# 07350100647/nvbio-gpl

Hardware: AMD Instinct MI355X
Metric: aligned reads/sec (150 bp single-end, 3 Gbp ref); GCUPS of the banded extend pass in `extend` (higher is better)
Workload: dtype u32 (FM-index coordinates) / i16x2 (band-31 DP, two alignments per 32-bit lane: 16-bit integer scores, held in binary16 lanes where every score is an integer of magnitude <= 2040 -- exact -- and in int16 lanes otherwise; bound-checked on the host)

## Files before the change

include/nvbio_amd.h:

```cpp
#ifndef NVBIO_AMD_H
#define NVBIO_AMD_H

#include <stdint.h>

#ifdef __cplusplus
extern "C" {
#endif

#define NVBIO_AMD_VERSION 100

typedef enum
{
    NVBIO_OK              = 0,
    NVBIO_ERR_INVALID     = 1,
    NVBIO_ERR_HIP         = 2,
    NVBIO_ERR_NOMEM       = 3,
    NVBIO_ERR_UNSUPPORTED = 4,
    NVBIO_ERR_NO_DEVICE   = 5
} nvbio_status;

int         nvbio_amd_version(void);
const char* nvbio_amd_last_error(void);
nvbio_status nvbio_amd_device_count(int* count);
nvbio_status nvbio_amd_device_arch(int device, char* name, uint32_t name_len);
// ... 125 lines not shown
                                           nvbio_uint2* hits_dev, void* stream);

nvbio_status nvbio_fm_filter_locate_diagonals(nvbio_fm_index_t index, const nvbio_uint2* ranges_dev, const uint64_t* slots_dev,
                                              const uint8_t* direct_dev, uint32_t n_queries, uint64_t begin, uint64_t end,
                                              uint32_t seeds_per_read, uint32_t seed_interval, uint32_t seed_len, uint32_t read_len,
                                              uint32_t strand, const uint32_t* query_ids_dev, uint64_t* keys_dev, void* stream);

enum { NVBIO_BACKTRACK_REFERENCE_QUIRKS = 1 };
nvbio_status nvbio_fm_hamming_backtrack(nvbio_fm_index_t index, const nvbio_string_set* queries, uint32_t seed_len, uint32_t mismatches, uint32_t flags,
                                        uint32_t* counts_dev, uint32_t* n_ranges_dev, nvbio_uint2* ranges_dev, uint32_t max_ranges, void* stream);

nvbio_status nvbio_fm_match_seed_diagonals_temp_bytes(const nvbio_string_set* seeds, uint64_t* bytes);
nvbio_status nvbio_fm_match_seed_diagonals(nvbio_fm_index_t index, const nvbio_string_set* seeds, uint32_t flags, uint32_t read_len,
                                           uint32_t strand, uint64_t* keys_dev, nvbio_uint2* residual_ranges_dev, uint32_t* residual_ids_dev,
                                           uint32_t* counts_dev, void* temp_dev, uint64_t temp_bytes, void* stream);

#define NVBIO_FM_INLINE_HITS(h) (((uint32_t)(h) & 15u) << 8)
#define NVBIO_FM_DEFER_HEAVY 64u
#define NVBIO_FM_NO_SEED_LOCUS 128u
#define NVBIO_FM_COUNT_LOCUS 4096u
#define NVBIO_FM_NO_FAST_RESOLVE 8192u
#define NVBIO_FM_COUNT_RESOLVE 16384u
nvbio_status nvbio_fm_match_seed_diagonals_both_temp_bytes(const nvbio_string_set* seeds, uint64_t* bytes);
nvbio_status nvbio_fm_match_seed_diagonals_both_keys_capacity(const nvbio_string_set* seeds, uint64_t* n_keys);
nvbio_status nvbio_fm_match_seed_diagonals_both(nvbio_fm_index_t index, const nvbio_string_set* seeds, uint32_t flags, uint32_t read_len,
                                                uint64_t* keys_dev, nvbio_uint2* residual_ranges_dev, uint32_t* residual_ids_dev,
                                                uint32_t residual_capacity, uint32_t* counts_dev, void* temp_dev, uint64_t temp_bytes,
                                                void* stream);
nvbio_status nvbio_fm_seed_tiles(const nvbio_string_set* seeds, uint32_t* reads_per_tile, uint32_t* n_tiles);
nvbio_status nvbio_fm_match_seed_diagonals_both_tiled(nvbio_fm_index_t index, const nvbio_string_set* seeds, uint32_t flags, uint32_t read_len,
                                                      uint64_t* keys_dev, nvbio_uint2* residual_ranges_dev, uint32_t* residual_ids_dev,
                                                      uint32_t residual_capacity, uint32_t* counts_dev, uint32_t* tile_offsets_dev,
                                                      void* temp_dev, uint64_t temp_bytes, void* stream);
int nvbio_fm_index_is_canonical(nvbio_fm_index_t index);

nvbio_status nvbio_fm_locate_init(nvbio_fm_index_t index, const uint32_t* rows_dev, uint32_t n,
                                  nvbio_uint2* jt_dev, void* stream);
nvbio_status nvbio_fm_locate_lookup(nvbio_fm_index_t index, const nvbio_uint2* jt_dev, uint32_t n,
                                    uint32_t* pos_dev, void* stream);

nvbio_status nvbio_fm_filter_rank(nvbio_fm_index_t index, const nvbio_string_set* queries, uint32_t flags,
                                  nvbio_uint2* ranges_dev, uint64_t* slots_dev, uint64_t* n_hits, void* stream);
nvbio_status nvbio_fm_filter_scan(nvbio_fm_index_t index, const nvbio_uint2* ranges_dev, uint32_t n_queries,
                                  uint64_t* slots_dev, uint64_t* n_hits, void* stream);
nvbio_status nvbio_fm_filter_locate(nvbio_fm_index_t index, const nvbio_uint2* ranges_dev, const uint64_t* slots_dev,
                                    uint32_t n_queries, uint64_t begin, uint64_t end,
                                    nvbio_uint2* hits_dev, void* stream);


typedef struct { uint32_t x, y, string_id, span; } nvbio_mem_range;
typedef struct { uint32_t pos, string_id, span_begin, span_end; } nvbio_mem_hit;
typedef struct { uint32_t min_intv, max_intv, min_span, split_len, split_width; } nvbio_mem_params;

nvbio_status nvbio_mem_filter_temp_bytes(const nvbio_string_set* reads, const nvbio_mem_params* params, uint64_t* bytes, void* stream);
nvbio_status nvbio_mem_filter_rank(nvbio_fm_index_t f_index, nvbio_fm_index_t r_index, const nvbio_string_set* reads,
                                   const nvbio_mem_params* params, nvbio_mem_range* ranges_dev, uint32_t max_ranges,
                                   uint32_t* first_range_dev, uint64_t* slots_dev, void* temp_dev, uint64_t temp_bytes,
                                   uint32_t* n_ranges, uint64_t* n_mems, uint64_t* records, void* stream);
nvbio_status nvbio_mem_filter_locate(nvbio_fm_index_t f_index, const nvbio_mem_range* ranges_dev, const uint64_t* slots_dev,
                                     uint32_t n_ranges, uint64_t begin, uint64_t end, nvbio_mem_hit* hits_dev, void* stream);

typedef struct nvbio_qgram_index_s* nvbio_qgram_index_t;

typedef struct
{
    uint32_t        q, symbol_size, qlut;
// ... 317 lines not shown
    const void*     text_dev;
    uint32_t        text_bits;
    const uint32_t* win_begin_dev;
    const uint32_t* win_end_dev;
    uint32_t        n;
    uint32_t        max_read_len;
    uint32_t        algo_flags;
    const void*     text_planes_dev;
} nvbio_alignment_batch;


enum
{
    NVBIO_ALN_NO_UNGAPPED_SCORE     = 1,
    NVBIO_ALN_NO_THIRD_CHANCE       = 2,
    NVBIO_ALN_NO_PACKED_DP          = 4,
    NVBIO_ALN_FORCE_PACKED_DP       = 8,
    NVBIO_ALN_NO_UNGAPPED_TRACEBACK = 16,
    NVBIO_ALN_PK_THREE_WAVES        = 32,
    NVBIO_ALN_NO_SECOND_CHANCE      = 128,
    NVBIO_ALN_NO_NARROW_SCORE       = 512,
    NVBIO_ALN_NO_BAND_ROUTE         = 1024,
    NVBIO_ALN_PK_STRIPE8            = 256,
    NVBIO_ALN_RAGGED_READS          = 4096,
    NVBIO_ALN_NO_LENGTH_SORT        = 8192,
    NVBIO_ALN_NO_QUALITY_SHORTCUT   = 2048,
    NVBIO_ALN_NO_GAP_CHANCE         = 65536,
    NVBIO_ALN_NO_COOPERATIVE_DP     = 32768,
    NVBIO_ALN_NO_F16_DP             = 16384,
    NVBIO_ALN_SPLIT_CHANCES         = 131072,
    NVBIO_ALN_NO_PAIRED_GAP_CHANCE  = 262144,
    NVBIO_ALN_NO_NARROW_DP          = 524288,
    NVBIO_ALN_NO_TEXT_PLANES        = 1048576,
    NVBIO_ALN_NO_NARROW_TRACEBACK   = 64
};

enum { NVBIO_READ_REVERSE = 1, NVBIO_READ_COMPLEMENT = 2 };

nvbio_status nvbio_best_candidate_reduce(int device, const uint64_t* keys_dev, const int32_t* scores_dev, const nvbio_uint2* sinks_dev,
                                         const uint32_t* win_begin_dev, uint64_t n, uint64_t* best_dev, void* stream);

nvbio_status nvbio_best_candidate_unpack(int device, const uint64_t* best_dev, uint32_t n_reads, int32_t* scores_dev,
                                         int64_t* end_pos_dev, uint8_t* rc_dev, void* stream);

nvbio_status nvbio_best_candidate_windows(int device, const uint64_t* keys_dev, const int32_t* scores_dev, const nvbio_uint2* sinks_dev,
                                          const uint32_t* win_begin_dev, uint64_t n, const uint64_t* best_dev, int64_t* best_wb_dev,
                                          int64_t* best_locus_dev, void* stream);

nvbio_status nvbio_traceback_best_batch(int device, const uint64_t* best_dev, const int64_t* best_wb_dev, uint32_t n_reads, uint32_t read_len,
                                        uint32_t band, uint32_t genome_len, int32_t min_score, uint8_t* flags_dev, uint32_t* win_begin_dev,
                                        uint32_t* win_end_dev, int32_t* scores_dev, nvbio_uint2* sinks_dev, void* stream);

nvbio_status nvbio_second_candidate_reduce(int device, const uint64_t* keys_dev, const int32_t* scores_dev, const nvbio_uint2* sinks_dev,
                                           const uint32_t* win_begin_dev, uint64_t n, const uint64_t* best_dev,
                                           uint32_t distinct_dist, int32_t worst_score, uint64_t* second_dev, void* stream);

typedef struct
{
    int32_t version;
    int32_t monotone;
    int32_t perfect_score;
    int32_t min_score;
} nvbio_mapq_params;
nvbio_status nvbio_mapq(int device, const uint64_t* best_dev, const uint64_t* second_dev, uint32_t n_reads,
                        const nvbio_mapq_params* params, int32_t* second_scores_dev, uint8_t* mapq_dev, void* stream);

nvbio_status nvbio_finish_reads_tiles_per_group(uint32_t reads_per_tile, uint32_t* tiles_per_group);
nvbio_status nvbio_finish_reads(int device, const uint64_t* keys_dev, const int32_t* scores_dev, const nvbio_uint2* sinks_dev,
                                const uint32_t* win_begin_dev, uint64_t n, const uint32_t* tile_offsets_dev, uint32_t n_tiles,
                                uint32_t reads_per_tile, uint32_t n_reads, uint32_t distinct_dist, int32_t worst_score,
                                const nvbio_mapq_params* params, int32_t match, const uint32_t* read_offsets_dev, const int32_t* min_scores_dev,
                                uint64_t* best_dev, uint64_t* second_dev, int32_t* scores_out_dev, int64_t* end_pos_dev, uint8_t* rc_dev,
                                uint8_t* mapq_dev, int32_t* second_scores_dev, uint32_t* status_dev, void* stream);

enum { NVBIO_PE_POLICY_FF = 0, NVBIO_PE_POLICY_FR = 1, NVBIO_PE_POLICY_RF = 2, NVBIO_PE_POLICY_RR = 3 };
nvbio_status nvbio_opposite_mate_windows(int device, const uint32_t* g_pos_dev, const uint8_t* anchor_rc_dev, uint32_t n,
                                         uint32_t anchor_len, uint32_t opposite_gapped_len, uint32_t anchor, uint32_t policy,
                                         uint32_t min_frag_len, uint32_t max_frag_len, uint32_t overlap, uint32_t genome_len,
                                         uint32_t* win_begin_dev, uint32_t* win_end_dev, uint8_t* flags_dev, uint8_t* valid_dev,
                                         void* stream);

#define NVBIO_GAP_PAIR_MAX_SHIFT 5
nvbio_status nvbio_banded_gap_pairs(int device, const nvbio_alignment_batch* batch, uint32_t* partner_dev, void* stream);

nvbio_status nvbio_banded_gotoh_score(int device, uint32_t band, nvbio_alignment_type type,
                                      const nvbio_gotoh_scheme* scheme, const nvbio_alignment_batch* batch,
                                      int32_t* scores_dev, nvbio_uint2* sinks_dev, void* stream);

nvbio_status nvbio_banded_gotoh_score_routes(int device, uint32_t band, nvbio_alignment_type type,
                                             const nvbio_gotoh_scheme* scheme, const nvbio_alignment_batch* batch,
                                             int32_t* scores_dev, nvbio_uint2* sinks_dev, uint8_t* routes_dev, void* stream);

nvbio_status nvbio_banded_gotoh_score_staged(int device, uint32_t band, nvbio_alignment_type type,
                                             const nvbio_gotoh_scheme* scheme, const nvbio_alignment_batch* batch,
                                             const int32_t* min_scores_dev, int32_t min_score,
                                             int32_t* scores_dev, nvbio_uint2* sinks_dev, void* stream);

enum { NVBIO_TRACEBACK_SINKS_GIVEN = 1 };
nvbio_status nvbio_banded_gotoh_traceback_temp_bytes(const nvbio_alignment_batch* batch_host_sizes, uint32_t band, uint64_t* bytes);
nvbio_status nvbio_banded_gotoh_traceback(int device, uint32_t band, nvbio_alignment_type type,
                                          const nvbio_gotoh_scheme* scheme, const nvbio_alignment_batch* batch,
                                          int32_t* scores_dev, nvbio_uint2* sources_dev, nvbio_uint2* sinks_dev,
                                          uint16_t* cigars_dev, uint32_t cigar_stride, uint32_t* cigar_lens_dev,
                                          uint32_t flags, void* temp_dev, uint64_t temp_bytes, void* stream);

nvbio_status nvbio_banded_gotoh_traceback_routes(int device, uint32_t band, nvbio_alignment_type type,
                                                 const nvbio_gotoh_scheme* scheme, const nvbio_alignment_batch* batch,
                                                 int32_t* scores_dev, nvbio_uint2* sources_dev, nvbio_uint2* sinks_dev,
                                                 uint16_t* cigars_dev, uint32_t cigar_stride, uint32_t* cigar_lens_dev,
                                                 uint32_t flags, void* temp_dev, uint64_t temp_bytes,
                                                 uint8_t* routes_dev, uint8_t* band_off_dev, void* stream);

nvbio_status nvbio_banded_sw_traceback(int device, uint32_t band, nvbio_alignment_type type,
                                       const nvbio_sw_scheme* scheme, const nvbio_alignment_batch* batch,
                                       int32_t* scores_dev, nvbio_uint2* sources_dev, nvbio_uint2* sinks_dev,
                                       uint16_t* cigars_dev, uint32_t cigar_stride, uint32_t* cigar_lens_dev,
                                       uint32_t flags, void* temp_dev, uint64_t temp_bytes, void* stream);

nvbio_status nvbio_full_gotoh_traceback_temp_bytes(const nvbio_alignment_batch* batch_host_sizes, uint32_t max_pattern_len,
                                                   uint32_t max_text_len, uint64_t* bytes);
nvbio_status nvbio_full_gotoh_traceback(int device, nvbio_alignment_type type, const nvbio_gotoh_scheme* scheme,
                                        const nvbio_alignment_batch* batch, uint32_t max_pattern_len, uint32_t max_text_len,
                                        const int32_t* min_scores_dev,
                                        int32_t* scores_dev, nvbio_uint2* sources_dev, nvbio_uint2* sinks_dev,
// ... 231 lines not shown
```

nvbio-gpl_amd/__init__.py:

```python
import ctypes
import os

import numpy as np

from .abi import bind

_HERE = os.path.dirname(os.path.abspath(__file__))
LIB_PATH = os.path.join(_HERE, "lib", "libnvbio_amd.so")
HEADER_PATH = os.path.join(os.path.dirname(_HERE), "include", "nvbio_amd.h")
HOST_HEADER_PATH = os.path.join(os.path.dirname(_HERE), "include", "nvbio_amd_host.h")

GLOBAL, LOCAL, SEMI_GLOBAL = 0, 1, 2
SCORE_MIN = -(1 << 30)
FM_SCAN_FORWARD, FM_COMPLEMENT, FM_NO_KMER_TABLE, FM_NO_VERIFY, FM_COUNT_SECTORS, FM_NO_PIPELINE, FM_DEFER_HEAVY = 1, 2, 4, 8, 16, 32, 64
FM_TABLE_NO_DIRECT, FM_TABLE_NO_CONTEXT, FM_TABLE_NO_GROUPS, FM_TABLE_CANONICAL, FM_TABLE_CANONICAL_WIDE = 1, 2, 4, 8, 16
FM_TABLE_NO_TEXT_PLANES = 32
FM_TABLE_NO_SEED_LOCUS = 64
FM_NO_SEED_LOCUS, FM_COUNT_LOCUS = 128, 4096
FM_NO_FAST_RESOLVE, FM_COUNT_RESOLVE = 8192, 16384
READ_REVERSE, READ_COMPLEMENT = 1, 2
MAX_SEED_OFFSET = 1024
TRACEBACK_SINKS_GIVEN = 1
ALN_NO_UNGAPPED_SCORE, ALN_NO_THIRD_CHANCE, ALN_NO_PACKED_DP, ALN_FORCE_PACKED_DP, ALN_NO_UNGAPPED_TRACEBACK, ALN_PK_THREE_WAVES = 1, 2, 4, 8, 16, 32
ALN_NO_NARROW_TRACEBACK, ALN_NO_SECOND_CHANCE, ALN_PK_STRIPE8, ALN_NO_NARROW_SCORE, ALN_NO_BAND_ROUTE = 64, 128, 256, 512, 1024
ALN_NO_QUALITY_SHORTCUT, ALN_RAGGED_READS, ALN_NO_LENGTH_SORT, ALN_NO_F16_DP, ALN_NO_COOPERATIVE_DP, ALN_NO_GAP_CHANCE = 2048, 4096, 8192, 16384, 32768, 65536
ALN_SPLIT_CHANCES, ALN_NO_PAIRED_GAP_CHANCE = 131072, 262144
ALN_NO_NARROW_DP = 524288
ALN_NO_TEXT_PLANES = 1048576
SEED_NO_LOCUS = 2097152
SEED_NO_FAST_RESOLVE = 4194304
ROUTE_SETTLED, ROUTE_FULL_BAND, ROUTE_CLASS_A, ROUTE_CLASS_B, ROUTE_REDONE = 0, 1, 2, 3, 8
DEFAULT_ALGO_FLAGS = 0
BACKTRACK_REFERENCE_QUIRKS = 1

_STATUS = {0: "OK", 1: "INVALID", 2: "HIP", 3: "NOMEM", 4: "UNSUPPORTED", 5: "NO_DEVICE"}


class NvbioError(RuntimeError):
    def __init__(self, status, msg):
        super().__init__("nvbio_amd: %s: %s" % (_STATUS.get(status, status), msg))
        self.status = status


class _View(ctypes.Structure):
    _fields_ = [("length", ctypes.c_uint32), ("primary", ctypes.c_uint32), ("L2", ctypes.c_uint32 * 5),
                ("bwt_occ_dev", ctypes.c_void_p), ("bwt_occ_words", ctypes.c_uint64),
                ("ssa_dev", ctypes.c_void_p), ("ssa_words", ctypes.c_uint64), ("sa_int", ctypes.c_uint32)]


class _BuildOptions(ctypes.Structure):
    _fields_ = [("kmer_len", ctypes.c_uint32), ("sa_int", ctypes.c_uint32), ("max_lcp", ctypes.c_uint32),
                ("verify", ctypes.c_uint32), ("table_flags", ctypes.c_uint32), ("bucket_symbols", ctypes.c_uint32)]


class _StringSet(ctypes.Structure):
    _fields_ = [("symbols_dev", ctypes.c_void_p), ("symbol_bits", ctypes.c_uint32),
                ("offsets_dev", ctypes.c_void_p), ("offsets_are_ranges", ctypes.c_uint32),
                ("fixed_len", ctypes.c_uint32), ("stride", ctypes.c_uint32), ("n", ctypes.c_uint32),
                ("seeds_per_string", ctypes.c_uint32), ("seed_interval", ctypes.c_uint32),
                ("seed_intervals_dev", ctypes.c_void_p)]


class _Scheme(ctypes.Structure):
    _fields_ = [("match", ctypes.c_int32), ("mm_min", ctypes.c_int32), ("mm_max", ctypes.c_int32),
# ... 292 lines not shown
        _check(lib().nvbio_fm_hamming_backtrack(self._h, ctypes.byref(qs), seed_len, mismatches, BACKTRACK_REFERENCE_QUIRKS if quirks else 0,
                                                _ptr(counts), _ptr(nr), _ptr(rg), max_ranges, _stream_ptr(self.device)))
        return counts, nr, rg

    def match_seed_diagonals(self, seeds, flags, read_len, strand, buffers=None, grid_blocks=0):
        torch = _torch()
        n = seeds.n
        if buffers is None:
            buffers = {}
        qs = seeds.c_struct()
        if buffers.get("n") != n or buffers.get("spr") != seeds.seeds_per_string:
            buffers["n"], buffers["spr"] = n, seeds.seeds_per_string
            buffers["keys"] = torch.empty(n, dtype=torch.int64, device=self.device)
            buffers["ranges"] = torch.empty((n, 2), dtype=torch.int32, device=self.device)
            buffers["ids"] = torch.empty(n, dtype=torch.int32, device=self.device)
            buffers["counts"] = torch.empty(4, dtype=torch.int32, device=self.device)
            nb = ctypes.c_uint64(0)
            _check(lib().nvbio_fm_match_seed_diagonals_temp_bytes(ctypes.byref(qs), ctypes.byref(nb)))
            buffers["temp"] = torch.empty(nb.value, dtype=torch.uint8, device=self.device)
        assert grid_blocks % 64 == 0 and grid_blocks < (1 << 22)
        _check(lib().nvbio_fm_match_seed_diagonals(self._h, ctypes.byref(qs), flags | ((grid_blocks // 64) << 16), read_len, strand,
                                                   _ptr(buffers["keys"]), _ptr(buffers["ranges"]), _ptr(buffers["ids"]), _ptr(buffers["counts"]),
                                                   _ptr(buffers["temp"]), buffers["temp"].numel(), _stream_ptr(self.device)))
        return buffers

    @property
    def canonical_kmer(self):
        return lib().nvbio_fm_index_is_canonical(self._h)

    @property
    def canonical(self):
        return self.canonical_kmer != 0

    def match_seed_diagonals_both(self, seeds, read_len, buffers=None, flags=0, grid_blocks=0, inline_hits=0, defer_heavy=False):
        torch = _torch()
        n = seeds.n
        if buffers is None:
            buffers = {}
        qs = seeds.c_struct()
        if buffers.get("n") != n or buffers.get("spr") != seeds.seeds_per_string:
            buffers["n"], buffers["spr"] = n, seeds.seeds_per_string
            cap = ctypes.c_uint64(0)
            _check(lib().nvbio_fm_match_seed_diagonals_both_keys_capacity(ctypes.byref(qs), ctypes.byref(cap)))
            buffers["keys"] = torch.empty(max(int(cap.value), 1), dtype=torch.int64, device=self.device)
            buffers["ranges"] = torch.empty((2 * n, 2), dtype=torch.int32, device=self.device)
            buffers["ids"] = torch.empty(2 * n, dtype=torch.int32, device=self.device)
            buffers["counts"] = torch.zeros(12, dtype=torch.int32, device=self.device)
            nb = ctypes.c_uint64(0)
            _check(lib().nvbio_fm_match_seed_diagonals_both_temp_bytes(ctypes.byref(qs), ctypes.byref(nb)))
            buffers["temp"] = torch.empty(nb.value, dtype=torch.uint8, device=self.device)
            rpt, nt = ctypes.c_uint32(0), ctypes.c_uint32(0)
            _check(lib().nvbio_fm_seed_tiles(ctypes.byref(qs), ctypes.byref(rpt), ctypes.byref(nt)))
            buffers["reads_per_tile"], buffers["n_tiles"] = int(rpt.value), int(nt.value)
            buffers["tile_offsets"] = torch.zeros(int(nt.value) + 1, dtype=torch.int32, device=self.device)
        assert grid_blocks % 64 == 0 and grid_blocks < (1 << 22)
        _check(lib().nvbio_fm_match_seed_diagonals_both_tiled(
            self._h, ctypes.byref(qs), flags | (FM_DEFER_HEAVY if defer_heavy else 0) | ((int(inline_hits) & 15) << 8) | ((grid_blocks // 64) << 16),
            read_len, _ptr(buffers["keys"]), _ptr(buffers["ranges"]), _ptr(buffers["ids"]), n, _ptr(buffers["counts"]), _ptr(buffers["tile_offsets"]),
            _ptr(buffers["temp"]), buffers["temp"].numel(), _stream_ptr(self.device)))
        return buffers

    def residual_diagonals(self, ranges, ids, cap, seeds_per_read, seed_interval, seed_len, read_len, read_offsets=None, seed_intervals=None):
        torch = _torch()
        n = int(ids.numel())
        keys = torch.empty(max(n * int(cap), 1), dtype=torch.int64, device=self.device)
        n_keys = torch.zeros(1, dtype=torch.int32, device=self.device)
        _check(lib().nvbio_fm_residual_diagonals(
            self._h, _ptr(ranges), _ptr(ids), n, int(cap), seeds_per_read, seed_interval, seed_len, read_len, _ptr(read_offsets),
            _ptr(seed_intervals), _ptr(keys), _ptr(n_keys), _stream_ptr(self.device)))
        return keys, n_keys

    def rank(self, rows, syms):
        torch = _torch()
        rows = _dev_tensor(rows, torch.int32, self.device)
        syms = _dev_tensor(syms, torch.uint8, self.device)
        out = torch.empty(rows.numel(), dtype=torch.int32, device=self.device)
        _check(lib().nvbio_fm_rank(self._h, _ptr(rows), _ptr(syms), rows.numel(), _ptr(out), _stream_ptr(self.device)))
        return out

    def rank4(self, rows):
        torch = _torch()
        rows = _dev_tensor(rows, torch.int32, self.device)
        out = torch.empty((rows.numel(), 4), dtype=torch.int32, device=self.device)
        _check(lib().nvbio_fm_rank4(self._h, _ptr(rows), rows.numel(), _ptr(out), _stream_ptr(self.device)))
        return out

    def basic_inv_psi(self, rows):
        torch = _torch()
        rows = _dev_tensor(rows, torch.int32, self.device)
        out = torch.empty(rows.numel(), dtype=torch.int32, device=self.device)
        _check(lib().nvbio_fm_basic_inv_psi(self._h, _ptr(rows), rows.numel(), _ptr(out), _stream_ptr(self.device)))
        return out
# ... 513 lines not shown
        self.c = _SWScheme(match, mismatch, deletion, insertion)


class SmithWatermanAligner:

    def __init__(self, type, scheme):
        self.type, self.sw = type, scheme
        c = scheme.c
        self.scheme = (GotohScheme(c.match, -c.mismatch, -c.mismatch, c.deletion, c.deletion, c.deletion, c.deletion)
                       if c.deletion == c.insertion else None)


def make_smith_waterman_aligner(type, scheme):
    return SmithWatermanAligner(type, scheme)


def make_edit_distance_aligner(type):
    return SmithWatermanAligner(type, SimpleSmithWatermanScheme(0, -1, -1, -1))


class GotohAligner:

    def __init__(self, type, scheme):
        self.type, self.scheme = type, scheme


def make_gotoh_aligner(type, scheme):
    return GotohAligner(type, scheme)


class AlignmentBatch:

    def __init__(self, reads, read_bits, read_offsets, text, text_bits, win_begin, win_end, quals=None, read_id=None,
                 flags=None, device="cuda:0", max_read_len=0, algo_flags=None, text_planes=None):
        torch = _torch()
        self.device = device
        self.text_planes = text_planes
        self.algo_flags = DEFAULT_ALGO_FLAGS if algo_flags is None else int(algo_flags)
        self.read_bits, self.text_bits = int(read_bits), int(text_bits)
        self.reads = _dev_tensor(reads, torch.uint8 if read_bits == 8 else torch.int32, device)
        self.read_offsets = _dev_tensor(read_offsets, torch.int32, device)
        self.text = _dev_tensor(text, torch.uint8 if text_bits == 8 else torch.int32, device)
        self.win_begin = _dev_tensor(win_begin, torch.int32, device)
        self.win_end = _dev_tensor(win_end, torch.int32, device)
        self.quals = _dev_tensor(quals, torch.uint8, device)
        self.read_id = _dev_tensor(read_id, torch.int32, device)
        self.flags = _dev_tensor(flags, torch.uint8, device)
        self.n = int(self.win_begin.numel())
        self.max_read_len = int(max_read_len)

    def size(self):
        return self.n

    def c_struct(self):
        return _Batch(_ptr(self.reads), self.read_bits, _ptr(self.read_offsets), _ptr(self.quals), _ptr(self.read_id),
                      _ptr(self.flags), _ptr(self.text), self.text_bits, _ptr(self.win_begin), _ptr(self.win_end),
                      self.n, self.max_read_len, self.algo_flags,
                      ctypes.c_void_p(self.text_planes.data_ptr() if hasattr(self.text_planes, "data_ptr") else self.text_planes))


def seed_locus_bytes(length):
    b = ctypes.c_uint64()
    _check(lib().nvbio_seed_locus_bytes(length, ctypes.byref(b)))
    return b.value


def text_planes_bytes(length):
    b = ctypes.c_uint64()
    _check(lib().nvbio_text_planes_bytes(length, ctypes.byref(b)))
    return b.value
# ... 13 lines not shown


class BatchedBandedAlignmentScore:

    def __init__(self, band_len, aligner, scheduler=DEVICE_THREAD_SCHEDULER):
        self.band_len, self.aligner, self.scheduler = int(band_len), aligner, scheduler
        if scheduler not in (DEVICE_THREAD_SCHEDULER, DEVICE_STAGED_THREAD_SCHEDULER):
            raise NvbioError(1, "unknown scheduler %r" % (scheduler,))

    def min_temp_storage(self, max_pattern_len, max_text_len, stream_size):
        return 0

    max_temp_storage = min_temp_storage

    def enact(self, batch, scores=None, sinks=None, min_scores=None):
        torch = _torch()
        if scores is None:
            scores = torch.empty(batch.n, dtype=torch.int32, device=batch.device)
        if sinks is None:
            sinks = torch.empty((batch.n, 2), dtype=torch.int32, device=batch.device)
        bs = batch.c_struct()
        sw = getattr(self.aligner, "sw", None)
        if self.scheduler == DEVICE_STAGED_THREAD_SCHEDULER:
            if sw is not None:
                raise NvbioError(4, "the staged scheduler is instantiated for Gotoh aligners")
            per_job = min_scores is not None and not isinstance(min_scores, int)
            if per_job and (min_scores.dtype != torch.int32 or min_scores.numel() != batch.n):
                raise NvbioError(1, "min_scores: int32 per job")
            _check(lib().nvbio_banded_gotoh_score_staged(
                FMIndex._dev_index(batch.device), self.band_len, self.aligner.type, ctypes.byref(self.aligner.scheme.c), ctypes.byref(bs),
                _ptr(min_scores) if per_job else None, SCORE_MIN if min_scores is None else (0 if per_job else int(min_scores)), _ptr(scores),
                _ptr(sinks), _stream_ptr(batch.device)))
            return scores, sinks
        fn = lib().nvbio_banded_sw_score if sw is not None else lib().nvbio_banded_gotoh_score
        _check(fn(FMIndex._dev_index(batch.device), self.band_len, self.aligner.type, ctypes.byref(sw.c if sw is not None else self.aligner.scheme.c),
                  ctypes.byref(bs), _ptr(scores), _ptr(sinks), _stream_ptr(batch.device)))
        return scores, sinks


def batch_banded_alignment_score(band_len, aligner, batch):
    return BatchedBandedAlignmentScore(band_len, aligner).enact(batch)


def banded_gotoh_score_routes(band_len, aligner, batch):
    torch = _torch()
    scores = torch.empty(batch.n, dtype=torch.int32, device=batch.device)
    sinks = torch.empty((batch.n, 2), dtype=torch.int32, device=batch.device)
    routes = torch.empty(batch.n, dtype=torch.uint8, device=batch.device)
    bs = batch.c_struct()
    _check(lib().nvbio_banded_gotoh_score_routes(FMIndex._dev_index(batch.device), int(band_len), aligner.type, ctypes.byref(aligner.scheme.c),
                                                 ctypes.byref(bs), _ptr(scores), _ptr(sinks), _ptr(routes), _stream_ptr(batch.device)))
    return scores, sinks, routes


TB_ROUTE_SETTLED, TB_ROUTE_FULL_BAND, TB_ROUTE_BAND15, TB_ROUTE_BAND7 = 0, 1, 2, 3


def banded_gotoh_traceback_routes(band_len, aligner, batch, cigar_stride=64, temp=None, scores=None, sinks=None):
    torch = _torch()
    n, dev = batch.n, batch.device
    given = scores is not None and sinks is not None
    if not given:
        scores = torch.empty(n, dtype=torch.int32, device=dev)
        sinks = torch.empty((n, 2), dtype=torch.int32, device=dev)
    sources = torch.empty((n, 2), dtype=torch.int32, device=dev)
    cigars = torch.zeros((n, cigar_stride), dtype=torch.int16, device=dev)
    lens = torch.empty(n, dtype=torch.int32, device=dev)
    routes = torch.empty(n, dtype=torch.uint8, device=dev)
    band_off = torch.empty(n, dtype=torch.uint8, device=dev)
    bs = batch.c_struct()
    _check(lib().nvbio_banded_gotoh_traceback_routes(
        FMIndex._dev_index(dev), int(band_len), aligner.type, ctypes.byref(aligner.scheme.c), ctypes.byref(bs), _ptr(scores), _ptr(sources),
        _ptr(sinks), _ptr(cigars), cigar_stride, _ptr(lens), TRACEBACK_SINKS_GIVEN if given else 0, _ptr(temp),
        0 if temp is None else temp.numel() * temp.element_size(), _ptr(routes), _ptr(band_off), _stream_ptr(dev)))
    return scores, sources, sinks, cigars, lens, routes, band_off


FULL_TB_ROUTE_SETTLED, FULL_TB_ROUTE_ALL_ROWS, FULL_TB_ROUTE_RESTRICTED, FULL_TB_ROUTE_BAND15 = 0, 1, 2, 3


def full_gotoh_traceback_routes(aligner, batch, max_pattern_len, max_text_len, min_scores=None, cigar_stride=64, temp=None, scores=None, sinks=None):
    torch = _torch()
# ... 1227 lines not shown
```

nvbio-gpl_amd/csrc/band31_first_pass.hip:

```cpp
#include "band31_ungapped_inl.h"

namespace nvbio_amd {

template <int RBITS, int MODE, bool QUAL = false>
__global__ void __launch_bounds__(256) __attribute__((amdgpu_waves_per_eu((MODE == 0 && !QUAL) ? 7 : 1)))
ungapped_e2e31_kernel(const BatchDev b, const int32_t P, const int32_t G, const int32_t gap_open, const int32_t gap_ext,
                      int32_t* __restrict__ scores, uint2* __restrict__ sinks, uint8_t* __restrict__ need_dp,
                      const uint32_t* __restrict__ job_list, const uint32_t* __restrict__ job_count,
                      const SchemeDev sc, const JobLists out, const uint32_t third_mask, const NarrowRule nr)
{
    constexpr bool LIST = MODE != 0;
    constexpr int  NL   = LIST ? 1 : 6;
    __shared__ int32_t s_pen[QUAL ? 64 : 1];
    __shared__ typename JobAppend<NL>::Lds s_lists;
    const uint32_t n    = LIST ? *job_count : b.n;
    const uint32_t slot0 = blockIdx.x * (256u * JOB_LIST_CHUNKS);
    if (slot0 >= n) return;
    if (QUAL)
    {
        if (threadIdx.x < 64) s_pen[threadIdx.x] = -mismatch_score( sc, threadIdx.x );
        __syncthreads();
    }
    JobAppend<NL> app;
    auto job_of = [&](const int k) -> uint32_t { const uint32_t slot = slot0 + 256u * k + threadIdx.x; return LIST ? job_list[slot] : slot; };
    const bool pairing = ((third_mask >> 4) & 1u) && !(b.algo & (NVBIO_ALN_NO_PAIRED_GAP_CHANCE | NVBIO_ALN_RAGGED_READS));
    #pragma unroll 1
    for (int k = 0; k < JOB_LIST_CHUNKS; ++k)
    {
        int which = -1;
        uint32_t flag = 0;
        if (slot0 + 256u * k + threadIdx.x < n)
        {
            const uint32_t job  = job_of( k );
            flag = ungapped_e2e31_job<RBITS,MODE,QUAL>( b, P, G, gap_open, gap_ext, scores, sinks, job, s_pen, nr );
            const uint32_t cls = flag >> 8;
            flag &= 255u;
            need_dp[job] = (uint8_t)flag;
            if (flag) which = LIST ? JOB_DP : (flag == 3u ? JOB_SECOND : (((third_mask >> flag) & 1u) ? JOB_THIRD : (cls ? JOB_CLASS_B - 1 + (int)cls : JOB_DP)));
        }
        if (MODE == 0 && !QUAL && pairing && __any( flag == 4u ))
        {
            const uint32_t slot = slot0 + 256u * k + threadIdx.x;
            const int role = gap_pair_role( b, slot, slot < n );
            const uint32_t flag_up = __shfl_down( flag, 1 ), flag_dn = __shfl_up( flag, 1 );
            if (role > 0 && flag == 4u && flag_up == 4u) which = JOB_PAIRS;
            if (role < 0 && flag == 4u && flag_dn == 4u) which = -1;
        }
        app.note( s_lists, k, which );
    }
    app.flush( s_lists, out, job_of );
}

nvbio_status launch_ungapped_e2e31(const uint32_t rbits, const int mode, const bool by_quality, const BatchDev& b, const SchemeDev& sc, const int32_t P,
                                   const int32_t G, int32_t* scores, uint2* sinks, uint8_t* need_dp, const JobLists& out, const uint32_t third_mask,
                                   const NarrowRule nr, hipStream_t s)
{
    const dim3 grid( job_list_grid( b.n ) ), block( 256 );
    const uint32_t* job_list  = mode == 1 ? out.second : (mode == 2 ? out.third : nullptr);
    const uint32_t* job_count = mode == 1 ? out.count( JOB_SECOND ) : (mode == 2 ? out.count( JOB_THIRD ) : nullptr);
    auto miss = [&] { set_error( "band-31 first pass: read_bits %u, mode %d not instantiated", rbits, mode ); return NVBIO_ERR_UNSUPPORTED; };
    return with_value( ReadBits31(), (int)rbits, [&](auto RB)
    {
        if (by_quality && mode == 0)
            return NVB_LAUNCH( (ungapped_e2e31_kernel<RB,0,true>), grid, block, s, b, P, G, sc.pat_go, sc.pat_ge, scores, sinks, need_dp, job_list, job_count,
                               sc, out, third_mask, nr );
        return with_value( Values<0, 1, 2>(), by_quality ? -1 : mode, [&](auto MODE)
        {
            return NVB_LAUNCH( (ungapped_e2e31_kernel<RB,MODE>), grid, block, s, b, P, G, sc.pat_go, sc.pat_ge, scores, sinks, need_dp, job_list, job_count,
                               MODE == 0 ? sc : SchemeDev{}, out, MODE == 0 ? third_mask : 0u, MODE == 0 ? nr : NarrowRule{ 1, 1, 0u } );
        }, miss );
    }, miss );
}

}
```

nvbio-gpl_amd/csrc/band31_jobs.h:

```cpp
#pragma once
#include "gotoh_common.h"
#include "bitplanes.h"

namespace nvbio_amd {

constexpr int GAP_CHANCE_GA = 5;
__host__ __device__ __forceinline__ int32_t gap_chance_unknown_cost(const int32_t P, const int32_t go, const int32_t ge)
{
    auto cg = [&](const int g) -> int32_t { return -(go + (g - 1) * ge); };
    int32_t c = cg( 1 ) + 3 * P;
    const int32_t others[] = { cg( GAP_CHANCE_GA + 1 ), 3 * cg( 1 ), 2 * cg( 1 ) + P, cg( 1 ) + cg( 3 ), 2 * cg( 2 ) };
    #pragma unroll
    for (int k = 0; k < 5; ++k) c = others[k] < c ? others[k] : c;
    return c;
}
struct GapLadder { int32_t c_unk_u, c_unk_n; };
constexpr int NARROW_A_HALF = 6, NARROW_B_HALF = 8;
struct NarrowJobs { const uint32_t *list_b, *count_b, *list_a, *count_a; uint32_t *redo, *redo_count; };
struct NarrowRule { int32_t thr_a, thr_b; uint32_t cnt_max; };
__device__ __forceinline__ uint32_t narrow_class(const NarrowRule nr, const int64_t U, const uint32_t best_d, const int32_t gap_ext)
{
    const int64_t o = best_d > 15u ? best_d - 15u : 15u - best_d;
    if (o <= NARROW_A_HALF && U >= (int64_t)nr.thr_a - o * gap_ext) return 2u;
    if (o <= NARROW_B_HALF && U >= (int64_t)nr.thr_b - o * gap_ext) return 1u;
    return 0u;
}

enum JobList : uint32_t
{
    JOB_DP,
    JOB_SECOND,
    JOB_THIRD,
    JOB_PAIRS,
    JOB_CLASS_B, JOB_CLASS_A,
    JOB_REDO,
    JOB_LIST_COUNT
};
static_assert( JOB_CLASS_A == JOB_CLASS_B + 1, "narrow_class() 1, 2 = class B, class A, in this order" );
constexpr uint32_t JOB_COUNT_STRIDE = 32u;
#ifndef NVB_JOB_LIST_CHUNKS
#define NVB_JOB_LIST_CHUNKS 1
#endif
constexpr int JOB_LIST_CHUNKS = NVB_JOB_LIST_CHUNKS;
static inline uint32_t job_list_grid(const uint32_t n) { return (n + 256u * JOB_LIST_CHUNKS - 1u) / (256u * JOB_LIST_CHUNKS); }

struct JobLists
{
    uint32_t *dp, *second, *third, *pairs; uint32_t* counts; uint32_t *class_b, *class_a, *redo;
    static __host__ __device__ constexpr uint32_t count_at(const uint32_t list) { return JOB_COUNT_STRIDE * list; }
    __host__ __device__ __forceinline__ uint32_t* count(const uint32_t list) const { return counts + count_at( list ); }
};

template <int NL>
struct JobAppend
{
    static_assert( NL >= 1 && NL <= 6 && JOB_LIST_CHUNKS >= 1 && JOB_LIST_CHUNKS <= 4, "JobAppend: up to 6 lists, up to 4 chunks" );
    struct Lds { uint32_t cnt[NL][4 * JOB_LIST_CHUNKS]; uint32_t base[NL]; };
    static constexpr int SLOT = NL <= 3 ? 8 : 16;
    typedef typename std::conditional<NL <= 3, uint32_t, uint64_t>::type Mine;
    Mine mine = 0;
    __device__ __forceinline__ void note(Lds& lds, const int k, const int which)
    {
        const uint32_t lane = threadIdx.x & 63u, wave = threadIdx.x >> 6;
        #pragma unroll
        for (int l = 0; l < NL; ++l)
        {
            const uint64_t m = __ballot( which == l );
            if (lane == 0) lds.cnt[l][4 * k + wave] = (uint32_t)__popcll( m );
            if (which == l) mine |= (Mine)(((uint32_t)(l + 1) << 6) | (uint32_t)__popcll( m & ((1ull << lane) - 1ull) )) << (SLOT * k);
        }
    }
    template <typename JobOf>
    __device__ __forceinline__ void flush(Lds& lds, const JobLists& out, JobOf job_of)
    {
        __syncthreads();
        if (threadIdx.x < (uint32_t)NL)
        {
            uint32_t tot = 0;
            for (int i = 0; i < 4 * JOB_LIST_CHUNKS; ++i) { const uint32_t c = lds.cnt[threadIdx.x][i]; lds.cnt[threadIdx.x][i] = tot; tot += c; }
            lds.base[threadIdx.x] = tot ? atomicAdd( out.count( threadIdx.x ), (unsigned int)tot ) : 0u;
        }
        __syncthreads();
        const uint32_t wave = threadIdx.x >> 6;
        #pragma unroll
        for (int k = 0; k < JOB_LIST_CHUNKS; ++k)
        {
            const uint32_t e = (uint32_t)(mine >> (SLOT * k)) & ((1u << SLOT) - 1u);
            if (e)
            {
                const uint32_t l = (e >> 6) - 1u;
                uint32_t* const list = l == JOB_DP ? out.dp : (l == JOB_SECOND ? out.second : (l == JOB_THIRD ? out.third : (l == JOB_PAIRS ? out.pairs : (l == JOB_CLASS_B ? out.class_b : out.class_a))));
                list[lds.base[l] + lds.cnt[l][4 * k + wave] + (e & 63u)] = job_of( k );
            }
        }
    }
};

struct JobAppendTwo
{
    struct Lds { uint32_t cnt[2 * 4 * JOB_LIST_CHUNKS]; uint32_t base; };
    uint64_t mine = 0;
    __device__ __forceinline__ void note(Lds& lds, const int k, const bool first, const bool second)
    {
        const uint32_t lane = threadIdx.x & 63u, wave = threadIdx.x >> 6;
        #pragma unroll
        for (int r = 0; r < 2; ++r)
        {
            const bool on = r ? second : first;
            const uint64_t m = __ballot( on );
            if (lane == 0) lds.cnt[4 * (2 * k + r) + wave] = (uint32_t)__popcll( m );
            if (on) mine |= (uint64_t)(64u | (uint32_t)__popcll( m & ((1ull << lane) - 1ull) )) << (16 * k + 8 * r);
        }
    }
    template <typename JobOf>
    __device__ __forceinline__ void flush(Lds& lds, const JobLists& out, JobOf job_of)
    {
        __syncthreads();
        if (threadIdx.x == 0)
        {
            uint32_t tot = 0;
            for (int i = 0; i < 2 * 4 * JOB_LIST_CHUNKS; ++i) { const uint32_t c = lds.cnt[i]; lds.cnt[i] = tot; tot += c; }
            lds.base = tot ? atomicAdd( out.count( JOB_DP ), (unsigned int)tot ) : 0u;
        }
        __syncthreads();
        const uint32_t wave = threadIdx.x >> 6;
        #pragma unroll
        for (int k = 0; k < JOB_LIST_CHUNKS; ++k)
            #pragma unroll
            for (int r = 0; r < 2; ++r)
            {
                const uint32_t e = (uint32_t)(mine >> (16 * k + 8 * r)) & 255u;
                if (e) out.dp[lds.base + lds.cnt[4 * (2 * k + r) + wave] + (e & 63u)] = job_of( k, r );
            }
    }
};

constexpr uint32_t PAIR_MAX_SHIFT = NVBIO_GAP_PAIR_MAX_SHIFT;

__device__ __forceinline__ int gap_pair_role(const BatchDev& b, const uint32_t job, const bool live)
{
    uint32_t rid = 0, fl = 0, tb = 0, whole = 0;
    if (live)
    {
        rid = b.read_id ? b.read_id[job] : job;
        const uint32_t M = b.read_offsets[rid + 1] - b.read_offsets[rid];
        fl = b.flags ? b.flags[job] : 0u;
        tb = b.win_begin[job];
        whole = (M >= 1u && M <= PLANE_MAX_READ && b.win_end[job] - tb == M + 31u) ? 1u : 0u;
    }
    const uint32_t lane = threadIdx.x & 63u;
    const uint32_t rid_n = __shfl_down( rid, 1 ), fl_n = __shfl_down( fl, 1 ), tb_n = __shfl_down( tb, 1 ), whole_n = __shfl_down( whole, 1 );
    const uint32_t shift = tb_n > tb ? tb_n - tb : tb - tb_n;
    const bool link = lane < 63u && whole && whole_n && rid_n == rid && fl_n == fl && shift >= 1u && shift <= PAIR_MAX_SHIFT;
    const uint64_t links = __ballot( link );
    const uint32_t run = lane ? (uint32_t)__clzll( (long long)~(links << (64u - lane)) ) : 0u;
    const bool lower = link && !(run & 1u);
    const uint64_t lowers = __ballot( lower );
    if (lower) return 1;
    return (lane && ((lowers >> (lane - 1u)) & 1ull)) ? -1 : 0;
}

bool packed_ok(const int type, const SchemeDev& sc, const uint32_t max_read_len);
bool pk_binary16_ok(const int type, const BatchDev& b, const SchemeDev& sc);
nvbio_status launch_pk_kernel(const int type, const uint32_t rbits, const BatchDev& b, const SchemeDev& sc, const uint32_t pairs, int32_t* scores, uint2* sinks,
                              const uint32_t* job_list, const uint32_t* job_count, hipStream_t s, const NarrowJobs* narrow = nullptr);
nvbio_status launch_ungapped_e2e31(const uint32_t rbits, const int mode, const bool by_quality, const BatchDev& b, const SchemeDev& sc, const int32_t P,
                                   const int32_t G, int32_t* scores, uint2* sinks, uint8_t* need_dp, const JobLists& out, const uint32_t third_mask,
                                   const NarrowRule nr, hipStream_t s);
nvbio_status launch_gap_chance_e2e31(const uint32_t rbits, const bool with_second, const BatchDev& b, const SchemeDev& sc, const int32_t P, const int32_t G,
                                     const GapLadder lad, int32_t* scores, uint2* sinks, uint8_t* need_dp, const JobLists& out, hipStream_t s);
nvbio_status launch_gap_pairs(const BatchDev& b, uint32_t* partner, hipStream_t s);
nvbio_status launch_pk(const int type, const uint32_t rbits, const BatchDev& b, const SchemeDev& sc, int32_t* scores, uint2* sinks, hipStream_t s, uint8_t* routes);

using ReadBits31 = Values<2, 4>;

}
```

nvbio-gpl_amd/csrc/band31_stage.hip:

```cpp
#include "band31_jobs.h"
#include <hipcub/hipcub.hpp>

namespace nvbio_amd {

static bool ungapped_ok(const SchemeDev& sc, const BatchDev& b, int32_t* P, bool* by_quality)
{
    if (sc.match != 0) return false;
    if (sc.mm_min < 0 || sc.mm_max < 0) return false;
    if (sc.mm_min == 0) return false;
    *by_quality = b.quals != nullptr && sc.mm_min != sc.mm_max;
    if (*by_quality && (sc.mm_min <= 0 || sc.mm_max < sc.mm_min || (b.algo & NVBIO_ALN_NO_QUALITY_SHORTCUT))) return false;
    if (sc.pat_go >= 0 || sc.txt_go >= 0 || sc.pat_ge > 0 || sc.txt_ge > 0) return false;
    *P = sc.mm_min;
    return true;
}

static NarrowRule narrow_rule(const bool on, const int32_t P, const int32_t go, const int32_t ge)
{
    NarrowRule r = { 1, 1, 0u };
    if (!on || ge >= 0 || P <= 0) return r;
    const int64_t a = (int64_t)go + (int64_t)NARROW_A_HALF * ge + 1, bb = (int64_t)go + (int64_t)NARROW_B_HALF * ge + 1;
    if (bb < -2000) return r;
    r.thr_a = (int32_t)a; r.thr_b = (int32_t)bb;
    r.cnt_max = (uint32_t)((-bb) / P);
// ... 29 lines not shown
    }
}

static nvbio_status sort_jobs_by_length(const BatchDev& b, const uint32_t* job_list, const uint32_t* job_count, const uint32_t** list_out,
                                        const uint32_t** count_out, ScratchBlock* aux, hipStream_t s)
{
    size_t sort_bytes = 0;
    const int bits = 16;
    NVB_HIP( hipcub::DeviceRadixSort::SortPairs( nullptr, sort_bytes, (const uint16_t*)nullptr, (uint16_t*)nullptr, (const uint32_t*)nullptr, (uint32_t*)nullptr,
                                                 (int)b.n, 0, bits, s ) );
    uint16_t *k_in, *k_out; uint32_t *l_all, *l_out, *c_all; void* tmp;
    NVB_CHECK( aux->alloc_layout( "banded_length_sort", s, "banded score: out of device memory for the length-sorted job list", [&](ScratchLayout& c)
    {
        k_in  = c.take<uint16_t>( b.n ); k_out = c.take<uint16_t>( b.n );
        l_all = c.take<uint32_t>( b.n ); l_out = c.take<uint32_t>( b.n );
        c_all = c.take<uint32_t>( 1 );
        tmp   = c.take<uint8_t>( sort_bytes );
    } ) );
    NVB_CHECK( NVB_LAUNCH( job_length_keys_kernel, dim3( (b.n + 255u) / 256u < 65536u ? (b.n + 255u) / 256u : 65536u ), dim3( 256 ), s, b, job_list, job_count, k_in, l_all, c_all ) );
    const hipError_t e = hipcub::DeviceRadixSort::SortPairs( tmp, sort_bytes, (const uint16_t*)k_in, k_out, job_list ? job_list : (const uint32_t*)l_all, l_out, (int)b.n, 0, bits, s );
    if (e != hipSuccess) { set_error( "job sort failed: %s", hipGetErrorString( e ) ); return NVBIO_ERR_HIP; }
    *list_out = l_out; *count_out = job_list ? job_count : c_all;
    return NVBIO_OK;
}

template <bool REDO>
__global__ void __launch_bounds__(256)
job_routes_kernel(const JobLists l, const uint32_t n, const bool classes, uint8_t* __restrict__ routes)
{
    const uint32_t n_dp = REDO ? 0u : *l.count( JOB_DP ), n_b = (REDO || !classes) ? 0u : *l.count( JOB_CLASS_B ), n_a = (REDO || !classes) ? 0u : *l.count( JOB_CLASS_A );
    const uint32_t n_r = (REDO && classes) ? *l.count( JOB_REDO ) : 0u;
    for (uint32_t i = blockIdx.x * blockDim.x + threadIdx.x; i < n; i += gridDim.x * blockDim.x)
    {
        if (i < n_dp) routes[l.dp[i]] = 1u;
        if (i < n_b)  routes[l.class_b[i]] = 3u;
        if (i < n_a)  routes[l.class_a[i]] = 2u;
        if (i < n_r)  routes[l.redo[i]] |= 8u;
    }
}

nvbio_status launch_pk(const int type, const uint32_t rbits, const BatchDev& b, const SchemeDev& sc, int32_t* scores, uint2* sinks, hipStream_t s, uint8_t* routes)
{
    const uint32_t pairs = (b.n + 1u) / 2u;
    int32_t P = 0; bool by_quality = false;
    const bool sorted_lengths = type == NVBIO_SEMI_GLOBAL && sc.match == 0 && (b.algo & NVBIO_ALN_RAGGED_READS) && !(b.algo & NVBIO_ALN_NO_LENGTH_SORT);
    if (type == NVBIO_SEMI_GLOBAL && ungapped_ok( sc, b, &P, &by_quality ) && !(b.algo & NVBIO_ALN_NO_UNGAPPED_SCORE))
    {
        const int32_t G = sc.pat_go > sc.txt_go ? sc.pat_go : sc.txt_go;
        const bool third = !(b.algo & NVBIO_ALN_NO_THIRD_CHANCE);
        uint8_t* need_dp; JobLists out;
        const NarrowRule nr = narrow_rule( b.quals == nullptr && !(b.algo & (NVBIO_ALN_NO_NARROW_DP | NVBIO_ALN_RAGGED_READS)) && pk_binary16_ok( type, b, sc ),
                                           P, sc.pat_go, sc.pat_ge );
        const bool classes = nr.thr_b != 1;
        ScratchBlock aux;
        NVB_CHECK( aux.alloc_layout( "banded_job_list", s, "banded score: out of device memory for the job list", [&](ScratchLayout& c)
        {
            need_dp     = c.take<uint8_t>( b.n );
            out.dp      = c.take<uint32_t>( b.n );
            out.second  = c.take<uint32_t>( b.n );
            out.third   = c.take<uint32_t>( b.n );
            out.pairs   = c.take<uint32_t>( (b.n + 1u) / 2u );
            out.counts  = c.take<uint32_t>( JobLists::count_at( JOB_LIST_COUNT ) );
            out.class_b = c.take<uint32_t>( classes ? b.n : 1u );
            out.class_a = c.take<uint32_t>( classes ? b.n : 1u );
            out.redo    = c.take<uint32_t>( classes ? b.n : 1u );
        } ) );
        const bool gapc = !by_quality && !(b.algo & NVBIO_ALN_NO_GAP_CHANCE);
        const uint32_t third_mask = gapc ? ((third ? 1u << 2 : 0u) | 1u << 4) : (third ? 1u << 2 : 0u);
        const bool fused = gapc && third && !(b.algo & (NVBIO_ALN_NO_SECOND_CHANCE | NVBIO_ALN_SPLIT_CHANCES));
        const GapLadder lad = gap_ladder( P, G, sc.pat_go, sc.pat_ge );
        NVB_HIP( hipMemsetAsync( out.counts, 0, JobLists::count_at( JOB_LIST_COUNT ) * sizeof(uint32_t), s ) );
        NVB_CHECK( launch_ungapped_e2e31( rbits, 0, by_quality, b, sc, P, G, scores, sinks, need_dp, out, third_mask, nr, s ) );
        if (!fused)     NVB_CHECK( launch_ungapped_e2e31( rbits, 1, false, b, sc, P, G, scores, sinks, need_dp, out, 0u, nr, s ) );
        if (gapc)       NVB_CHECK( launch_gap_chance_e2e31( rbits, fused, b, sc, P, G, lad, scores, sinks, need_dp, out, s ) );
        else if (third) NVB_CHECK( launch_ungapped_e2e31( rbits, 2, false, b, sc, P, G, scores, sinks, need_dp, out, 0u, nr, s ) );
        const uint32_t* jl = out.dp; const uint32_t* jc = out.count( JOB_DP ); ScratchBlock sorted;
        if (sorted_lengths) NVB_CHECK( sort_jobs_by_length( b, out.dp, out.count( JOB_DP ), &jl, &jc, &sorted, s ) );
        if (classes)
        {
            const NarrowJobs nj = { out.class_b, out.count( JOB_CLASS_B ), out.class_a, out.count( JOB_CLASS_A ), out.redo, out.count( JOB_REDO ) };
            NVB_CHECK( launch_pk_kernel( type, rbits, b, sc, pairs, scores, sinks, jl, jc, s, &nj ) );
            NVB_CHECK( launch_pk_kernel( type, rbits, b, sc, pairs, scores, sinks, out.redo, out.count( JOB_REDO ), s ) );
        }
        else
            NVB_CHECK( launch_pk_kernel( type, rbits, b, sc, pairs, scores, sinks, jl, jc, s ) );
        if (routes)
        {
            const dim3 rgrid( (b.n + 255u) / 256u < 4096u ? (b.n + 255u) / 256u : 4096u ), block( 256 );
            NVB_HIP( hipMemsetAsync( routes, 0, b.n, s ) );
            NVB_CHECK( NVB_LAUNCH( job_routes_kernel<false>, rgrid, block, s, out, b.n, classes, routes ) );
            NVB_CHECK( NVB_LAUNCH( job_routes_kernel<true>,  rgrid, block, s, out, b.n, classes, routes ) );
        }
        return NVBIO_OK;
    }
    if (sorted_lengths && b.n > 1u)
    {
        const uint32_t* jl = nullptr; const uint32_t* jc = nullptr; ScratchBlock sorted;
        NVB_CHECK( sort_jobs_by_length( b, nullptr, nullptr, &jl, &jc, &sorted, s ) );
        return launch_pk_kernel( type, rbits, b, sc, pairs, scores, sinks, jl, jc, s );
    }
    return launch_pk_kernel( type, rbits, b, sc, pairs, scores, sinks, nullptr, nullptr, s );
}

}
```

nvbio-gpl_amd/csrc/band31_ungapped_inl.h:

```cpp
#pragma once
#include "band31_jobs.h"

namespace nvbio_amd {


struct PlaneWords
{
    uint32_t pl[6], ph[6], pn[6], pm[6], ql[7], qh[7];

    __device__ __forceinline__ void set(const uint64_t (&rlo)[3], const uint64_t (&rhi)[3], const uint64_t (&rn)[3],
                                        const uint64_t (&tlo)[4], const uint64_t (&thi)[4], const uint32_t M)
    {
        #pragma unroll
        for (int k = 0; k < 3; ++k)
        {
            pattern_plane_words( k, rlo, rhi, rn, M, pl, ph, pn, pm );
            ql[2*k] = (uint32_t)tlo[k]; ql[2*k+1] = (uint32_t)(tlo[k] >> 32);
            qh[2*k] = (uint32_t)thi[k]; qh[2*k+1] = (uint32_t)(thi[k] >> 32);
        }
        ql[6] = (uint32_t)tlo[3]; qh[6] = (uint32_t)thi[3];
    }
    __device__ __forceinline__ uint32_t mmw(const int k, const uint32_t x) const
    {
        const uint32_t tl = __builtin_amdgcn_alignbit( ql[k + 1], ql[k], x ), th = __builtin_amdgcn_alignbit( qh[k + 1], qh[k], x );
        return (((pl[k] ^ tl) | (ph[k] ^ th)) & pm[k]) | pn[k];
    }
};

template <int RBITS, int MODE, bool QUAL>
__device__ __forceinline__ uint32_t
ungapped_e2e31_job(const BatchDev& b, const int32_t P, const int32_t G, const int32_t gap_open, const int32_t gap_ext,
                   int32_t* __restrict__ scores, uint2* __restrict__ sinks, const uint32_t job, const int32_t* s_pen,
                   const NarrowRule nr = NarrowRule{ 1, 1, 0u })
{
    constexpr bool LIST = MODE != 0;
    const AlnJob   J = load_job( b, job );
    const uint32_t first = J.first, M = J.M, tb = J.tb, N = scored_text_len( b, J );
    const bool     rev = J.rev, comp = J.comp;

    if (N < M)
    {
        scores[job] = NVBIO_SCORE_MIN; sinks[job] = make_uint2( 0xFFFFFFFFu, 0xFFFFFFFFu );
        return 0u;
    }
    if (M == 0u || M > 161u) return 1u;

    uint64_t rlo[3], rhi[3], rn[3], tlo[4], thi[4];
    {
        ReadWords<RBITS> rw; TextUnits<4> tu;
        load_read_words<RBITS>( b.reads, first, M, rw );
        if (b.text_planes) load_text_units<4,0,3>( b.text_planes, tb, tu );
        else               load_text_words<13>( b.text, tb, N < 192u ? N : 192u, tu );
        read_planes192<RBITS>( rw, first, M, rev, comp, rlo, rhi, rn );
        if (b.text_planes)
        {
            load_text_units<4,3,4>( b.text_planes, tb, tu );
            text_planes_units<4>( tu, tb, tlo, thi );
        }
        else text_planes_words<13>( tu, tb, tlo, thi );
    }
    const uint32_t mb = M + 30u;
    const uint32_t m  = (mb < N ? mb : N) - (M - 1u);
    PlaneWords pw;
    pw.set( rlo, rhi, rn, tlo, thi, M );
    const uint32_t (&pl)[6] = pw.pl, (&ph)[6] = pw.ph, (&pn)[6] = pw.pn, (&pm)[6] = pw.pm, (&ql0)[7] = pw.ql, (&qh0)[7] = pw.qh;
    uint32_t ql[7], qh[7];

    uint32_t best_cnt = 0xFFFFFFFFu, best_d = 0;
    int64_t U = 0;
    if (LIST)
    {
        U      = scores[job];
        best_d = sinks[job].x - M;
    }
    else
    {
        const int64_t floor_u = 3 * (int64_t)(G < gap_open ? G : gap_open) - P;
        const uint32_t cap = P > 0 ? (uint32_t)((-floor_u - 1) / (int64_t)P) : 0xFFFFFFFEu;
        const uint32_t cap_x = (!QUAL && nr.cnt_max > cap && N >= M + 30u) ? nr.cnt_max : cap;
        uint32_t cnt_d[QUAL ? 31 : 1];
        #pragma unroll
        for (uint32_t d = 0; d < 31u; ++d)
        {
            const bool on = (d == 0u || d < m);
            uint32_t cnt = (uint32_t)__popc( pw.mmw( 0, d ) );
            const uint32_t thr = QUAL ? cap : (best_cnt < cap_x ? best_cnt : cap_x);
            if (__any( on && cnt <= thr ))
            {
                #pragma unroll
                for (int k = 1; k < 6; ++k) cnt += (uint32_t)__popc( pw.mmw( k, d ) );
            }
            else cnt = 0xFFFFFFFFu;
            if (QUAL) cnt_d[d] = on ? cnt : 0xFFFFFFFFu;
            if (on && cnt <= best_cnt) { best_cnt = cnt; best_d = d; }
        }
        if (best_cnt > cap)
        {
            if (!QUAL && best_cnt <= cap_x)
            {
                const uint32_t cls = narrow_class( nr, -(int64_t)P * (int64_t)best_cnt, best_d, gap_ext );
                if (cls) { scores[job] = -P * (int32_t)best_cnt; sinks[job] = make_uint2( M + best_d, M ); return 1u | (cls << 8); }
            }
            const bool gap_chance = !QUAL && P > 0 && N >= M + 30u && gap_ext < 0 && gap_open <= gap_ext && !(b.algo & NVBIO_ALN_NO_GAP_CHANCE);
            return gap_chance ? 4u : 1u;
        }
        U = -(int64_t)P * (int64_t)best_cnt;
        if (QUAL)
        {
            if (U <= 3 * (int64_t)G - P) return 1u;
            const uint32_t pmax  = (uint32_t)s_pen[63];
            const uint64_t bound = (uint64_t)pmax * best_cnt;
            uint32_t cand = 0;
            #pragma unroll
            for (uint32_t d = 0; d < 31u; ++d)
                if (cnt_d[d] != 0xFFFFFFFFu && (uint64_t)(uint32_t)P * cnt_d[d] <= bound) cand |= 1u << d;
            uint32_t best_w = 0xFFFFFFFFu;
            while (cand)
            {
                const uint32_t d = (uint32_t)__builtin_ctz( cand );
                cand &= cand - 1u;
                uint32_t w = 0;
                #pragma unroll
                for (int k = 0; k < 6; ++k)
                {
                    uint32_t mm = pw.mmw( k, d );
                    while (mm)
                    {
                        const uint32_t row = 32u * k + (uint32_t)__builtin_ctz( mm );
                        mm &= mm - 1u;
                        const uint32_t qq = b.quals[rev ? first + M - 1u - row : first + row];
                        w += (uint32_t)s_pen[qq < 63u ? qq : 63u];
                    }
                }
                if (w <= best_w) { best_w = w; best_d = d; }
            }
            U = -(int64_t)best_w;
        }
    }
    bool settled = U > (int64_t)G;
    auto stash = [&]() { scores[job] = (int32_t)U; sinks[job] = make_uint2( M + best_d, M ); };
    const bool second_applies = !settled && (int64_t)G - P < U && 2 * (int64_t)G < U && N >= M + 30u && !(b.algo & NVBIO_ALN_NO_SECOND_CHANCE);
    if (MODE == 0 && second_applies)
    {
        int32_t gmax = 0;
        while (gmax < 5 && (int64_t)gap_open + (int64_t)gmax * gap_ext >= U) ++gmax;
        if (gmax >= 1 && gmax <= 4) { stash(); return 3u; }
    }
    if (MODE == 1 && second_applies)
    {
        int32_t gmax = 0;
        while (gmax < 5 && (int64_t)gap_open + (int64_t)gmax * gap_ext >= U) ++gmax;
        if (gmax >= 1 && gmax <= 4)
        {
            #pragma unroll
            for (int k = 0; k < 7; ++k) { ql[k] = ql0[k]; qh[k] = qh0[k]; }
            uint32_t lead_prev[4] = { 0, 0, 0, 0 }, tail_prev[4] = { 0, 0, 0, 0 };
            bool gapped = false;
            for (uint32_t d = 0; d < 31u && !gapped; ++d)
            {
                uint32_t first = M, last = 0xFFFFFFFFu;
                #pragma unroll
                for (int k = 0; k < 6; ++k)
                    if (first == M)
                    {
                        const uint32_t mm = (((pl[k] ^ ql[k]) | (ph[k] ^ qh[k])) & pm[k]) | pn[k];
                        if (mm) first = 32u * k + (uint32_t)__builtin_ctz( mm );
                    }
                #pragma unroll
                for (int k = 5; k >= 0; --k)
                    if (last == 0xFFFFFFFFu)
                    {
                        const uint32_t mm = (((pl[k] ^ ql[k]) | (ph[k] ^ qh[k])) & pm[k]) | pn[k];
                        if (mm) last = 32u * k + 31u - (uint32_t)__builtin_clz( mm );
                    }
                const uint32_t lead = first;
                const uint32_t tail = (last == 0xFFFFFFFFu) ? M : M - 1u - last;
                #pragma unroll
                for (int g = 1; g <= 4; ++g)
                    if (g <= gmax && d >= (uint32_t)g)
                    {
                        if (lead_prev[g - 1] + tail >= M) gapped = true;
                        if (lead + tail_prev[g - 1] + (uint32_t)g >= M) gapped = true;
                    }
                #pragma unroll
                for (int k = 3; k > 0; --k) { lead_prev[k] = lead_prev[k - 1]; tail_prev[k] = tail_prev[k - 1]; }
                lead_prev[0] = lead; tail_prev[0] = tail;
                #pragma unroll
                for (int k = 0; k < 6; ++k)
                {
                    ql[k] = __builtin_amdgcn_alignbit( ql[k + 1], ql[k], 1u );
                    qh[k] = __builtin_amdgcn_alignbit( qh[k + 1], qh[k], 1u );
                }
                ql[6] >>= 1; qh[6] >>= 1;
            }
            settled = !gapped;
        }
    }
    const int64_t go = gap_open, ge = gap_ext;
    int32_t gmax0 = 0, gmax1 = 0;
    while (gmax0 < 5 && go + (int64_t)gmax0 * ge >= U) ++gmax0;
    while (gmax1 < 5 && go + (int64_t)gmax1 * ge - P >= U) ++gmax1;
    const bool two11  = 2 * go >= U;
    const bool beyond = gmax0 > 4 || gmax1 > 4 || go - 2 * (int64_t)P >= U || 2 * go + ge >= U || 2 * go - P >= U || 3 * go >= U || ge < go;
    const bool third_applies = !settled && N >= M + 30u && !beyond && gmax0 >= 1 && (gmax1 >= 1 || two11);
    if (MODE == 0 && third_applies)
    {
        stash();
        return 2u;
    }
    if (MODE != 0 && third_applies)
    {
        #pragma unroll
        for (int k = 0; k < 7; ++k) { ql[k] = ql0[k]; qh[k] = qh0[k]; }
        uint32_t lead0_p[4] = { 0, 0, 0, 0 }, lead1_p[4] = { 0, 0, 0, 0 }, tail0_p[4] = { 0, 0, 0, 0 }, tail1_p[4] = { 0, 0, 0, 0 };
        bool gapped = false;
        uint32_t mwp[6] = { 0, 0, 0, 0, 0, 0 };
        for (uint32_t d = 0; d <= 31u && !gapped; ++d)
        {
            const bool have = d < 31u;
            uint32_t first = M, second = M, last = 0xFFFFFFFFu, last2 = 0xFFFFFFFFu;
            #pragma unroll
            for (int k = 0; k < 6; ++k)
                if (have && __any( second == M ))
                {
                    uint32_t w = (second == M) ? ((((pl[k] ^ ql[k]) | (ph[k] ^ qh[k])) & pm[k]) | pn[k]) : 0u;
                    if (first == M && w) { first = 32u * k + (uint32_t)__builtin_ctz( w ); w &= w - 1u; }
                    if (first != M && second == M && w) second = 32u * k + (uint32_t)__builtin_ctz( w );
                }
            #pragma unroll
            for (int k = 5; k >= 0; --k)
                if (have && __any( last2 == 0xFFFFFFFFu ))
                {
                    uint32_t w = (last2 == 0xFFFFFFFFu) ? ((((pl[k] ^ ql[k]) | (ph[k] ^ qh[k])) & pm[k]) | pn[k]) : 0u;
                    if (last == 0xFFFFFFFFu && w) { const uint32_t t = 31u - (uint32_t)__builtin_clz( w ); last = 32u * k + t; w &= ~(1u << t); }
                    if (last != 0xFFFFFFFFu && last2 == 0xFFFFFFFFu && w) last2 = 32u * k + 31u - (uint32_t)__builtin_clz( w );
                }
            const uint32_t lead0 = first, lead1 = second;
            const uint32_t tail0 = (last  == 0xFFFFFFFFu) ? M : M - 1u - last;
            const uint32_t tail1 = (last2 == 0xFFFFFFFFu) ? M : M - 1u - last2;
            if (have)
            {
                #pragma unroll
// ... 51 lines not shown
                                {
                                    const uint32_t hi_m = (a1 >= 32) ? 0xFFFFFFFFu : ((1u << a1) - 1u);
                                    const uint32_t lo_m = (1u << a0) - 1u;
                                    any = any || ((mwp[k] & hi_m & ~lo_m) != 0u);
                                }
                            }
                        }
                        if (!any) gapped = true;
                    }
            }
            #pragma unroll
            for (int k = 3; k > 0; --k) { lead0_p[k] = lead0_p[k - 1]; lead1_p[k] = lead1_p[k - 1]; tail0_p[k] = tail0_p[k - 1]; tail1_p[k] = tail1_p[k - 1]; }
            lead0_p[0] = lead0; lead1_p[0] = lead1; tail0_p[0] = tail0; tail1_p[0] = tail1;
            if (two11 && have)
            {
                #pragma unroll
                for (int k = 0; k < 6; ++k) mwp[k] = (((pl[k] ^ ql[k]) | (ph[k] ^ qh[k])) & pm[k]) | pn[k];
            }
            #pragma unroll
            for (int k = 0; k < 6; ++k)
            {
                ql[k] = __builtin_amdgcn_alignbit( ql[k + 1], ql[k], 1u );
                qh[k] = __builtin_amdgcn_alignbit( qh[k + 1], qh[k], 1u );
            }
            ql[6] >>= 1; qh[6] >>= 1;
        }
        settled = !gapped;
    }
    if (settled)
    {
        scores[job] = (int32_t)U; sinks[job] = make_uint2( M + best_d, M );
        return 0u;
    }
    if (MODE == 0 && !QUAL && N >= M + 30u)
    {
        const uint32_t cls = narrow_class( nr, U, best_d, gap_ext );
        if (cls) { stash(); return 1u | (cls << 8); }
    }
    return 1u;
}

}
```

nvbio-gpl_amd/csrc/bitplanes.h:

```cpp
#pragma once
#include "common.h"

namespace nvbio_amd {

constexpr uint32_t PLANE_MAX_READ = 161u;

template <int RBITS> struct ReadWords { static constexpr int N = (161 + 15) * RBITS / 32 + 2; uint32_t w[N]; };

template <int RBITS>
__device__ __forceinline__ void load_read_words(const void* reads, const uint32_t first, const uint32_t M, ReadWords<RBITS>& out)
{
    constexpr uint32_t RPW = 32u / RBITS;
    const uint32_t* __restrict__ rwords = (const uint32_t*)reads;
    const uint32_t rw0 = (first & ~(RPW - 1u)) / RPW, rw_last = (first + M - 1u) / RPW;
    #pragma unroll
    for (int j = 0; j < ReadWords<RBITS>::N; ++j) { const uint32_t widx = rw0 + (uint32_t)j; out.w[j] = rwords[widx < rw_last ? widx : rw_last]; }
}

template <int WORDS, typename W>
__device__ __forceinline__ void load_text_words(const void* text, const uint32_t tb, const uint32_t T, W& out)
{
    const uint32_t* __restrict__ twords = (const uint32_t*)text;
    const uint32_t tw0 = (tb & ~15u) >> 4, tw_last = (tb + T - 1u) >> 4;
    #pragma unroll
// ... 138 lines not shown
    #pragma unroll
    for (int k = 0; k < 4; ++k)
    {
        tlo[k] = (uint64_t)__builtin_amdgcn_alignbit( a[2*k+1], a[2*k], s ) | ((uint64_t)__builtin_amdgcn_alignbit( a[2*k+2], a[2*k+1], s ) << 32);
        thi[k] = (uint64_t)__builtin_amdgcn_alignbit( c[2*k+1], c[2*k], s ) | ((uint64_t)__builtin_amdgcn_alignbit( c[2*k+2], c[2*k+1], s ) << 32);
    }
}

constexpr uint32_t SEED_LOCUS_LINE_BYTES = 128u;
constexpr uint32_t SEED_LOCUS_UNITS      = 5u;
constexpr uint32_t SEED_LOCUS_MAX_READ   = 193u;
inline __host__ __device__ uint64_t seed_locus_lines(const uint32_t n) { return ((uint64_t)n >> 7) + 1u; }

struct LocusWords { uint32_t lo0, lo1, hi0, hi1, u; };

__device__ __forceinline__ void load_locus_words(const void* __restrict__ lines, const uint32_t base, const uint32_t x, LocusWords& out)
{
    static_assert( 127u + SEED_LOCUS_MAX_READ - 1u <= 64u * SEED_LOCUS_UNITS - 1u, "the last symbol of a read lies in the line its first symbol lies in" );
    static_assert( 24u * SEED_LOCUS_UNITS <= SEED_LOCUS_LINE_BYTES, "a line holds its units" );
    const uint32_t line = base >> 7, off = x - (line << 7), unit = off >> 6, w = (off >> 5) & 1u;
    const uint32_t* __restrict__ p = (const uint32_t*)lines + ((size_t)line * 32u + 6u * unit);
    const uint32_t w1 = w ? (unit + 1u < SEED_LOCUS_UNITS ? 6u : 0u) : 1u;
    out.lo0 = p[w]; out.lo1 = p[w1]; out.hi0 = p[2u + w]; out.hi1 = p[2u + w1]; out.u = p[4u + w];
}

__device__ __forceinline__ bool locus_answers(const LocusWords& lw, const uint32_t x, const uint32_t len, const uint32_t tlo, const uint32_t thi)
{
    const uint32_t s = x & 31u;
    const uint32_t lo = __builtin_amdgcn_alignbit( lw.lo1, lw.lo0, s ), hi = __builtin_amdgcn_alignbit( lw.hi1, lw.hi0, s );
    const uint32_t mask = len >= 32u ? 0xFFFFFFFFu : (1u << len) - 1u;
    return ((((lo ^ tlo) | (hi ^ thi)) & mask) == 0u) && ((lw.u >> s) & 1u);
}

}
```

nvbio-gpl_amd/csrc/fm_canon_inl.h:

```cpp
constexpr uint32_t CTAB_FLANK    = 7u;
constexpr uint32_t CTAB_ROWS_MAX = 8u;
constexpr uint32_t CTAB_INLINE   = 4u;

__device__ __forceinline__ uint64_t canon_revcomp(const uint64_t key, const uint32_t k)
{
    return reverse_symbols( key, k ) ^ ((1ull << (2u * k)) - 1ull);
}
__device__ __forceinline__ uint64_t canon_index(const uint64_t ckey, const uint32_t k)
{
    return ((ckey >> (k + 1u)) << k) | (ckey & ((1ull << k) - 1ull));
}
__device__ __forceinline__ uint64_t canon_key(const uint64_t idx, const uint32_t k)
{
    return ((idx >> k) << (k + 1u)) | (idx & ((1ull << k) - 1ull));
}
__device__ __forceinline__ uint32_t text_symbol(const uint32_t* __restrict__ text, const uint32_t i)
{
    return (text[i >> 4] >> (30u - 2u * (i & 15u))) & 3u;
}

__device__ __forceinline__ uint2 canon_range(const DevIndex& f, const uint64_t key)
{
    const uint2 r = f.ktab[key >> 2];
    uint32_t x = r.x, y = r.y, nb = 0;
// ... 212 lines not shown
seed_locus_kernel(const DevIndex f, const uint32_t len, const uint32_t wide, const uint64_t n_units, const uint64_t n_lines, uint64_t* __restrict__ lines)
{
    const uint32_t lane = threadIdx.x & 63u, n = f.length;
    for (uint64_t unit = (uint64_t)blockIdx.x * 4u + (threadIdx.x >> 6); unit < n_units; unit += (uint64_t)gridDim.x * 4u)
    {
        const uint64_t x64 = unit * 64u + lane;
        const uint32_t sym = x64 < n ? text_symbol( f.text, (uint32_t)x64 ) : 0u;
        bool uq = false;
        if (x64 + len <= n)
        {
            const uint32_t x = (uint32_t)x64;
            uint64_t V; uint32_t qo; CanonHits h;
            (void)seed_bits_from_words<2>( load_seed_words<2>( f.text, x, len ), x, len, false, false, V );
            uint4 e = canon_entry( f, V, len, wide != 0u, qo );
            uq = canon_lookup( f, V, len, qo, e, h ) && h.nf == 1u && h.nr == 0u && h.vf == x;
            if (uq)
            {
                const uint64_t R = canon_revcomp( V, len );
                e  = canon_entry( f, R, len, wide != 0u, qo );
                uq = canon_lookup( f, R, len, qo, e, h ) && h.nf == 0u && h.nr == 1u && h.vr == x;
            }
        }
        const uint64_t ub = __ballot( uq ), lo = __ballot( (sym & 1u) != 0u ), hi = __ballot( (sym & 2u) != 0u );
        if (lane < 3u && (unit >> 1) >= lane)
        {
            const uint64_t L = (unit >> 1) - lane, slot = unit - 2u * L;
            if (L < n_lines && slot < SEED_LOCUS_UNITS) { uint64_t* p = lines + L * 16u + 3u * slot; p[0] = lo; p[1] = hi; p[2] = ub; }
        }
    }
}

enum : uint32_t { LS_SEED = 1u, LS_OK = 2u, LS_ASKED = 4u, LS_USABLE = 8u, LS_STRAND = 16u,
                  LS_SETTLED = 32u,
                  LS_BEGIN = 256u };
template <int BITS, bool COUNT, bool WIDE, bool RAGGED, typename Geom, typename Entry, typename Resolve>
__device__ __forceinline__ void fm_seed_locus_loop(const DevIndex& f, const StringSetDev& q, const SeedTiles& tl, const uint32_t read_len, const void* __restrict__ locus,
                                                   unsigned long long* __restrict__ sectors_out, unsigned int* __restrict__ routes, const uint32_t tile0,
                                                   const uint32_t lane, const uint32_t lr, const uint32_t j, const bool lane_ok,
                                                   const Geom& seed_geom, const Entry& entry_of, const Resolve& resolve_tile)
{
    const uint32_t n_waves = gridDim.x * 4u;
    const uint32_t k = f.ckmer, len = q.fixed_len, n = f.length;
    const uint32_t anchor = lane - j;
    const bool     first = j == 0u;
    const uint32_t u_pfw = j * q.interval;
    const uint4 none = make_uint4( 1u, 0u, 0u, 0u );
    auto qo_of = [&](const uint64_t V) -> uint32_t { return (uint32_t)(V >> (2u * (len - k) + k)) & 1u; };
    auto pfw_of  = [&](const uint32_t v) -> uint32_t { return RAGGED ? v : u_pfw; };
    auto rlen_of = [&](const uint32_t v) -> uint32_t { return RAGGED ? v : read_len; };
    auto add = [&](unsigned int* word, const bool on) {
        const uint32_t c = (uint32_t)__popcll( __ballot( on ) );
        if (lane == 0 && c) atomicAdd( word, c );
    };
    SeedWords W = { 0, 0, 0, 0, 0 }; uint32_t w_pfw = 0, w_rlen = 0, w_fl = 0;
    uint64_t aV = 0; uint4 ae = none; uint32_t a_fl = 0, a_pfw = 0, a_rlen = 0;
    uint64_t lV = 0; uint32_t l_fl = 0, l_pfw = 0, l_rlen = 0;
    uint32_t l_x = 0; LocusWords LW = { none.x, none.y, none.z, none.w, 0 };
    uint64_t cV = 0; uint4 ce = none; uint32_t c_fl = 0, c_pfw = 0, c_rlen = 0;
    for (uint32_t step = 0; ; ++step)
    {
        const uint64_t t4 = (uint64_t)tile0 + (uint64_t)step * n_waves;
        if (step >= 4u && t4 - 4ull * n_waves >= tl.n_tiles) break;
        uint32_t settled = 0;
        if (l_fl & LS_ASKED)
        {
            const uint32_t strand = (l_fl / LS_STRAND) & 1u;
            const uint32_t vl = (uint32_t)lV, vh = (uint32_t)(lV >> 32);
            uint32_t plo = squeeze2( vl ) | (squeeze2( vh ) << 16), phi = squeeze2( vl >> 1 ) | (squeeze2( vh >> 1 ) << 16);
            if (strand) { plo = ~(__brev( plo ) >> (32u - len)); phi = ~(__brev( phi ) >> (32u - len)); }
            if (locus_answers( LW, l_x, len, plo, phi )) settled = 1u + strand;
        }
        if (COUNT && routes)
        {
            add( routes + 1, settled != 0u );
            add( routes + 2, (l_fl & LS_SEED) && !first && (l_fl & LS_USABLE) && !settled );
            add( routes + 3, (l_fl & LS_SEED) && !first && !(l_fl & LS_USABLE) );
        }
        uint32_t a_hit = 0xFFFFFFFFu, a_strand = 0;
        if (first && (a_fl & LS_OK))
        {
            CanonHits h;
            if (canon_lookup( f, aV, len, qo_of( aV ), ae, h ) && h.nf + h.nr == 1u) { a_strand = h.nr; a_hit = h.nr ? h.vr : h.vf; }
        }
        const uint32_t r_hit = (uint32_t)__shfl( (int)a_hit, (int)anchor ), r_strand = (uint32_t)__shfl( (int)a_strand, (int)anchor );
        const bool usable = r_hit != 0xFFFFFFFFu;
        bool ask = false; uint32_t x = 0, base = 0;
        if (usable && !first && (a_fl & LS_OK) && rlen_of( a_rlen ) <= SEED_LOCUS_MAX_READ)
        {
            const uint32_t p = pfw_of( a_pfw );
            if (r_strand == 0u) { base = r_hit; x = r_hit + p; ask = (uint64_t)r_hit + p + len <= n; }
            else
            {
                const uint32_t span = rlen_of( a_rlen ) - len;
                base = r_hit >= span ? r_hit - span : 0u; x = r_hit - p; ask = r_hit >= p;
            }
        }
        if (COUNT)
        {
            if (routes) add( routes, first && usable );
            const uint64_t asked = __ballot( ask );
            const uint64_t mine = (q.spr >= 64u ? ~0ull : ((1ull << q.spr) - 1ull)) << anchor;
            const uint32_t c = (uint32_t)__popcll( __ballot( first && (asked & mine) != 0ull ) );
            if (lane == 0 && c) atomicAdd( sectors_out, (unsigned long long)c );
        }
        uint64_t nV = 0; uint32_t n_fl = w_fl;
        if (w_fl & LS_SEED) n_fl |= seed_bits_from_words<BITS>( W, (w_fl / LS_BEGIN) & 15u, len, false, false, nV ) ? LS_OK : 0u;
        const uint32_t n_pfw = w_pfw, n_rlen = w_rlen;
        const bool c_ok = (c_fl & LS_OK) != 0u;
        const bool is_one   = c_ok && ce.y >= DTAB_MARK && ce.x < DTAB_MARK;
        const bool is_group = c_ok && ce.y >= DTAB_MARK && ce.x >= DTAB_MARK;
        const bool is_heavy = c_ok && ce.y < DTAB_MARK && ce.x <= ce.y;
        uint4 q0 = make_uint4( 0, 0, 0, 0 ), q1 = q0, q2 = q0, q3 = q0;
        if (is_group)
        {
            const uint4* g4 = (const uint4*)(f.cside + 4ull * (ce.x - DTAB_MARK));
            q0 = g4[0]; q1 = g4[1];
            if (ce.y - DTAB_MARK > 4u) { q2 = g4[2]; q3 = g4[3]; }
        }
        uint4 got = none;
        if (first ? (n_fl & LS_OK) != 0u : ((l_fl & LS_OK) && !settled)) { uint32_t qo; got = entry_of( first ? nV : lV, qo ); }
        const uint4 fe = first ? make_uint4( LW.lo0, LW.lo1, LW.hi0, LW.hi1 ) : got;
        LocusWords nLW = { ae.x, ae.y, ae.z, ae.w, 0 };
        if (ask) load_locus_words( locus, base, x, nLW );
        {
            const uint64_t rid4 = t4 * tl.rpt + lr;
            uint32_t w_begin = 0;
            bool ws = t4 < tl.n_tiles && lane_ok && rid4 < tl.reads;
            if (RAGGED) { if (ws) ws = seed_geom( (uint32_t)rid4, w_begin, w_pfw, w_rlen ); }
            else if (ws) w_begin = (q.offsets ? q.offsets[rid4] : (uint32_t)rid4 * q.stride) + u_pfw;
            if (ws) W = load_seed_words<BITS>( q.symbols, w_begin, len );
            w_fl = ws ? LS_SEED | ((w_begin & 15u) * LS_BEGIN) : 0u;
        }
        if (step >= 4u)
        {
            const uint32_t tile = (uint32_t)(t4 - 4ull * n_waves), rid = tile * tl.rpt + lr;
            resolve_tile( tile, rid, (c_fl & LS_SEED) != 0u, cV, ce, c_ok, qo_of( cV ), pfw_of( c_pfw ), rlen_of( c_rlen ), is_one, is_group, is_heavy,
                          q0, q1, q2, q3, (c_fl / LS_SETTLED) & 3u, (uint32_t)cV );
        }
        cV = settled ? (uint64_t)l_x : lV; ce = fe; c_fl = l_fl | (settled * LS_SETTLED); c_pfw = l_pfw; c_rlen = l_rlen;
        lV = aV; l_pfw = a_pfw; l_rlen = a_rlen; l_x = x; LW = nLW;
        l_fl = (a_fl & (LS_SEED | LS_OK)) | (ask ? LS_ASKED : 0u) | (usable ? LS_USABLE : 0u) | (r_strand ? LS_STRAND : 0u);
        aV = nV; ae = got; a_fl = n_fl; a_pfw = n_pfw; a_rlen = n_rlen;
    }
}

constexpr uint32_t SEED_RESOLVE_GENERAL = 16u;
template <int BITS, bool COUNT, bool WIDE, bool DEFER, bool LOCUS, bool RAGGED = false>
__global__ void __launch_bounds__(256)
fm_seed_both_kernel(const DevIndex f, const StringSetDev q, const SeedTiles tl, const uint32_t read_len, const uint32_t resolve_opts,
                    uint64_t* __restrict__ tile_keys, uint32_t* __restrict__ tile_counts, uint2* __restrict__ res_ranges,
                    uint32_t* __restrict__ res_ids, const uint32_t res_cap, unsigned int* __restrict__ counts, unsigned long long* __restrict__ sectors_out,
                    uint32_t* __restrict__ tile_defer, uint32_t* __restrict__ defer_counts, const void* __restrict__ locus, unsigned int* __restrict__ routes,
                    unsigned int* __restrict__ paths)
{
    const uint32_t lane = threadIdx.x & 63u;
    const uint32_t inline_max = resolve_opts & 15u;
    constexpr bool FAST_FORM = BITS == 4 && WIDE && (COUNT || DEFER);
    const bool fast_ok = FAST_FORM && !(resolve_opts & SEED_RESOLVE_GENERAL) && inline_max >= 1u && f.length >= q.fixed_len;
    const uint32_t n_waves = gridDim.x * 4u;
    const uint32_t k = f.ckmer, len = q.fixed_len, r = len - k;
    const uint32_t lr = lane / q.spr, j = lane - lr * q.spr;
    const bool lane_ok = lr < tl.rpt;
    const bool ragged = LOCUS ? RAGGED : (q.intervals != nullptr);
    const uint32_t rmask = (1u << (2u * r)) - 1u;
    const uint32_t fshift = 2u * (CTAB_FLANK - r);
    DevIndex fplain = f; fplain.dtab = nullptr; fplain.dkmer = 0;

    auto seed_geom = [&](const uint32_t rid, uint32_t& begin, uint32_t& p_fw, uint32_t& rlen) -> bool {
        const uint32_t base = q.offsets ? q.offsets[rid] : rid * q.stride;
        p_fw  = j * (ragged ? q.intervals[rid] : q.interval);
        rlen  = ragged ? q.offsets[rid + 1] - base : read_len;
        begin = base + p_fw;
        return !ragged || p_fw + len <= rlen;
    };
    auto entry_of = [&](const uint64_t V, uint32_t& qo) -> uint4 {
        const uint64_t key = V >> (2u * r);
        qo = (uint32_t)(key >> k) & 1u;
        const uint64_t idx = canon_index( qo ? canon_revcomp( key, k ) : key, k );
        if (WIDE)
        {
            typedef unsigned int u4v __attribute__((ext_vector_type(4)));
            const u4v v = __builtin_nontemporal_load( (const u4v*)f.ctab + idx );
            return make_uint4( v.x, v.y, v.z, v.w );
        }
        const uint2 e = load_table_entry( f.ctab, idx, true );
        return make_uint4( e.x, e.y, 0u, 0u );
    };

    auto resolve_tile = [&](const uint32_t tile, const uint32_t rid, const bool valid, const uint64_t V, const uint4 e, const bool e_valid, const uint32_t qo,
                            const uint32_t c_pfw, const uint32_t c_rlen, const bool is_one, const bool is_group, const bool is_heavy,
                            const uint4 q0, const uint4 q1, const uint4 q2, const uint4 q3, const uint32_t settled, const uint32_t settled_x)
    {
        const uint32_t m = e.y - DTAB_MARK;
        const uint32_t rest = (uint32_t)V & rmask;
        const uint32_t want = qo ? (~rest & rmask) : rest;
        const uint32_t i = rid * q.spr + j;
        uint32_t sectors = (e_valid && !(LOCUS && settled)) ? (is_group ? 2u : 1u) : 0u;
        bool common = false;
        if (fast_ok)
        {
            const uint32_t fsel = (qo ? 0u : 14u) + fshift;
            const uint32_t plim = f.length - len + 1u;
            uint32_t cnt = 0, hit_rev = 0, hit_p = 0;
            auto crow = [&](const bool on, const uint32_t P, const uint32_t C) {
                const uint32_t rev = ((C >> 28) ^ qo) & 1u;
                const bool fits = rev ? P < plim : P >= r;
                const bool hit = on & (__builtin_amdgcn_ubfe( C, fsel, 2u * r ) == want) & fits;
                cnt += hit ? 1u : 0u; hit_rev = hit ? rev : hit_rev; hit_p = hit ? P : hit_p;
            };
            crow( is_one, e.x, e.y );
            if (WIDE) crow( is_one & (e.w >= DTAB_MARK), e.z, e.w );
            if (__ballot( is_group ))
            {
                const uint32_t gm = is_group ? m : 0u;
                crow( 0u < gm, q0.x, q0.y ); crow( 1u < gm, q0.z, q0.w ); crow( 2u < gm, q1.x, q1.y ); crow( 3u < gm, q1.z, q1.w );
                if (__ballot( gm > 4u ))
                {
                    crow( 4u < gm, q2.x, q2.y ); crow( 5u < gm, q2.z, q2.w ); crow( 6u < gm, q3.x, q3.y ); crow( 7u < gm, q3.z, q3.w );
                }
            }
            uint32_t v = hit_rev ? hit_p : hit_p - r;
            if (LOCUS && settled) { cnt = 1u; hit_rev = settled - 1u; v = settled_x; }
            const bool live = valid && e_valid;
            common = __ballot( live && (is_heavy || cnt > 1u) ) == 0ull;
            if (common)
            {
                const bool     has = live && cnt == 1u;
                const uint32_t s = hit_rev;
                const uint32_t p = s ? c_rlen - c_pfw - len : c_pfw;
                const uint64_t diag = (uint64_t)v + 1024u - p;
                const uint64_t key = ((uint64_t)rid << 34) | ((uint64_t)s << 33) | diag;
                const uint64_t below = (1ull << lane) - 1ull;
                const uint64_t m0 = __ballot( has && s == 0u ), m1 = __ballot( has && s != 0u );
                const uint64_t prev_mask = (s ? m1 : m0) & below;
                const int      prev_lane = prev_mask ? 63 - __clzll( (long long)prev_mask ) : 0;
                const uint32_t prev_diag = (uint32_t)__shfl( (int)(uint32_t)diag, prev_lane );
                const bool     dup = prev_mask != 0ull && (uint32_t)prev_lane >= lane - j && prev_diag == (uint32_t)diag;
                const bool     keep = has && !dup;
                const uint64_t k0 = __ballot( keep && s == 0u ), k1 = __ballot( keep && s != 0u );
                const uint32_t n0 = (uint32_t)__popcll( k0 ), n1 = (uint32_t)__popcll( k1 );
                if (keep) tile_keys[(uint64_t)tile * 128u + (s ? n0 + (uint32_t)__popcll( k1 & below ) : (uint32_t)__popcll( k0 & below ))] = key;
                if (lane == 0) { tile_counts[tile] = n0 + n1; if (DEFER) defer_counts[tile] = 0u; }
            }
        }
        if (COUNT && paths && lane == 0) atomicAdd( paths + (common ? 0 : 1), 1u );
        if (!common)
        {
        uint32_t hits[2] = { 0, 0 }, pos[2][CTAB_INLINE] = { { 0, 0, 0, 0 }, { 0, 0, 0, 0 } };
        auto row = [&](const uint32_t P, const uint32_t C) {
            bool rev; uint32_t v;
            if (!canon_row_hit( P, C, qo, want, fshift, r, len, f.length, rev, v )) return;
            #pragma unroll
            for (int s = 0; s < 2; ++s)
                if ((s == 1) == rev)
                {
                    #pragma unroll
                    for (uint32_t t = 0; t < CTAB_INLINE; ++t) pos[s][t] = (hits[s] == t) ? v : pos[s][t];
                    ++hits[s];
                }
        };
        if (is_one) { row( e.x, e.y ); if (WIDE && e.w >= DTAB_MARK) row( e.z, e.w ); }
        else if (is_group)
        {
#define NVB_CROW(jj, P, C) if ((jj) < m) row( (P), (C) );
            NVB_CROW( 0u, q0.x, q0.y ) NVB_CROW( 1u, q0.z, q0.w ) NVB_CROW( 2u, q1.x, q1.y ) NVB_CROW( 3u, q1.z, q1.w )
            NVB_CROW( 4u, q2.x, q2.y ) NVB_CROW( 5u, q2.z, q2.w ) NVB_CROW( 6u, q3.x, q3.y ) NVB_CROW( 7u, q3.z, q3.w )
#undef NVB_CROW
        }
        if (LOCUS && settled)
        {
            hits[0] = settled == 1u; hits[1] = settled == 2u;
            pos[0][0] = pos[1][0] = settled_x;
        }
        uint32_t tile_fill = 0;
        uint32_t defer_fill = 0;
        #pragma unroll
        for (int s = 0; s < 2; ++s)
        {
            uint32_t cnt = (valid && e_valid && !is_heavy && hits[s] <= inline_max) ? hits[s] : 0u;
            uint32_t rx = 1u, ry = 0u;
            bool searched = false, deferred = false;
            const uint32_t sflags = s ? (NVBIO_FM_SCAN_FORWARD | NVBIO_FM_COMPLEMENT) : 0u;
            auto plain_search = [&]() -> bool {
                uint32_t nblk, sec = 0; bool single = false;
                match_one<BITS,false,true,true>( fplain, q, sflags, f.ktab != nullptr, false, i, rx, ry, nblk, single, &sec );
                sectors += sec; searched = true;
                return single;
            };
            if (valid && e_valid && (is_heavy || hits[s] > inline_max))
            {
                cnt = 0u;
                if (DEFER) deferred = true;
                else if (plain_search()) { pos[s][0] = rx; cnt = 1u; }
                else if (rx <= ry && ry - rx < inline_max)
                {
                    cnt = ry - rx + 1u;
                    #pragma unroll
                    for (uint32_t t = 0; t < CTAB_INLINE; ++t)
                        if (t < cnt) { const uint32_t sv = f.ssa[rx + t]; pos[s][t] = (sv == 0xFFFFFFFFu) ? f.length : sv; }
                    sectors += cnt;
                }
            }
            if (__ballot( cnt >= 2u ))
            {
                uint32_t total = (uint32_t)__popcll( __ballot( cnt == 1u ) );
                #pragma unroll
// ... 7 lines not shown
            }
            uint64_t* slots = tile_keys + (uint64_t)tile * 128u + tile_fill;
            uint32_t n_out = 0; uint64_t last = ~0ull;
            const uint32_t x1 = cnt == 1u ? pos[s][0] : (cnt == 0u ? rx : 1u), y1 = cnt == 1u ? pos[s][0] : (cnt == 0u ? ry : 0u);
            emit_seed_results( c_pfw, len, c_rlen, (uint32_t)s, lane, valid, cnt == 1u, x1, y1, rid, i, slots, n_out, last,
                               res_ranges + (s ? res_cap : 0u), res_ids + (s ? res_cap : 0u), counts + s );
            if (__ballot( cnt >= 2u ))
            {
                uint32_t pq = c_pfw;
                if (s) pq = c_rlen - pq - len;
                #pragma unroll
                for (uint32_t t = 0; t < CTAB_INLINE; ++t)
                {
                    const bool on = cnt >= 2u && t < cnt;
                    const uint64_t mk = __ballot( on );
                    if (on) slots[n_out + (uint32_t)__popcll( mk & ((1ull << lane) - 1ull) )] =
                                ((uint64_t)rid << 34) | ((uint64_t)s << 33) | ((uint64_t)pos[s][t] + 1024u - pq);
                    n_out += (uint32_t)__popcll( mk );
                }
            }
            tile_fill += n_out;
            if (DEFER)
            {
                const uint64_t md = __ballot( deferred );
                if (md)
                {
                    if (deferred) tile_defer[(uint64_t)tile * 128u + defer_fill + (uint32_t)__popcll( md & ((1ull << lane) - 1ull) )] = i | ((uint32_t)s << 31);
                    defer_fill += (uint32_t)__popcll( md );
                }
            }
        }
        if (lane == 0) { tile_counts[tile] = tile_fill; if (DEFER) defer_counts[tile] = defer_fill; }
        }
        if (COUNT)
        {
            uint32_t tot = valid ? sectors : 0u;
            #pragma unroll
            for (int d = 32; d > 0; d >>= 1) tot += (uint32_t)__shfl_xor( (int)tot, d );
            if (lane == 0 && tot) atomicAdd( sectors_out, (unsigned long long)tot );
        }
    };

    uint32_t tile = blockIdx.x * 4u + (threadIdx.x >> 6);
    if (tile >= tl.n_tiles) return;
    if constexpr (LOCUS)
    {
        tile = (uint32_t)__builtin_amdgcn_readfirstlane( (int)tile );
        fm_seed_locus_loop<BITS,COUNT,WIDE,RAGGED>( f, q, tl, read_len, locus, sectors_out, routes, tile, lane, lr, j, lane_ok, seed_geom, entry_of, resolve_tile );
        return;
    }
    SeedWords W = { 0, 0, 0, 0, 0 }; uint32_t w_begin = 0, w_pfw = 0, w_rlen = 0; bool w_valid = false;
    uint64_t V = 0; uint4 e = make_uint4( 1u, 0u, 0u, 0u ); bool e_valid = false; uint32_t qo = 0, c_pfw = 0, c_rlen = 0; bool c_seed = false;
    {
        const uint32_t rid = tile * tl.rpt + lr;
        if (lane_ok && rid < tl.reads)
        {
            uint32_t b0;
            c_seed = seed_geom( rid, b0, c_pfw, c_rlen );
            if (c_seed)
            {
                const SeedWords W0 = load_seed_words<BITS>( q.symbols, b0, len );
                e_valid = seed_bits_from_words<BITS>( W0, b0, len, false, false, V );
                if (e_valid) e = entry_of( V, qo );
            }
        }
        const uint32_t t1 = tile + n_waves, rid1 = t1 * tl.rpt + lr;
        if (t1 < tl.n_tiles && lane_ok && rid1 < tl.reads)
        {
            w_valid = seed_geom( rid1, w_begin, w_pfw, w_rlen );
            if (w_valid) W = load_seed_words<BITS>( q.symbols, w_begin, len );
        }
    }
    for (; tile < tl.n_tiles; tile += n_waves)
    {
        const uint32_t rid = tile * tl.rpt + lr;
        const bool valid = lane_ok && rid < tl.reads && c_seed;
        const bool is_one   = e_valid && e.y >= DTAB_MARK && e.x < DTAB_MARK;
        const bool is_group = e_valid && e.y >= DTAB_MARK && e.x >= DTAB_MARK;
        const bool is_heavy = e_valid && e.y < DTAB_MARK && e.x <= e.y;
        uint4 q0 = make_uint4( 0, 0, 0, 0 ), q1 = q0, q2 = q0, q3 = q0;
        const uint32_t m = e.y - DTAB_MARK;
        if (is_group)
        {
            const uint4* g4 = (const uint4*)(f.cside + 4ull * (e.x - DTAB_MARK));
            q0 = g4[0]; q1 = g4[1];
            if (m > 4u) { q2 = g4[2]; q3 = g4[3]; }
        }
        uint64_t Vn = 0; uint4 en = make_uint4( 1u, 0u, 0u, 0u ); bool en_valid = false; uint32_t qon = 0;
        const uint32_t n_pfw = w_pfw, n_rlen = w_rlen; const bool n_seed = w_valid;
        if (w_valid)
        {
            en_valid = seed_bits_from_words<BITS>( W, w_begin, len, false, false, Vn );
            if (en_valid) en = entry_of( Vn, qon );
        }
        {
            const uint32_t t2 = tile + 2u * n_waves, rid2 = t2 * tl.rpt + lr;
            w_valid = t2 < tl.n_tiles && lane_ok && rid2 < tl.reads;
            if (w_valid) w_valid = seed_geom( rid2, w_begin, w_pfw, w_rlen );
            if (w_valid) W = load_seed_words<BITS>( q.symbols, w_begin, len );
        }
        resolve_tile( tile, rid, valid, V, e, e_valid, qo, c_pfw, c_rlen, is_one, is_group, is_heavy, q0, q1, q2, q3, 0u, 0u );
        V = Vn; e = en; e_valid = en_valid; qo = qon; c_pfw = n_pfw; c_rlen = n_rlen; c_seed = n_seed;
    }
}

constexpr uint32_t HEAVY_PER_LANE = 4u;
template <int BITS>
__global__ void __launch_bounds__(256)
fm_seed_heavy_kernel(const DevIndex f, const StringSetDev q, const uint32_t read_len, const uint32_t* __restrict__ list, const uint32_t* __restrict__ n_list,
                     uint64_t* __restrict__ keys_out, uint2* __restrict__ res_ranges, uint32_t* __restrict__ res_ids, const uint32_t res_cap,
                     unsigned int* __restrict__ counts)
{
    __shared__ uint32_t s_cnt[4][3], s_base[3];
    const uint32_t n = *n_list;
    const uint32_t lane = threadIdx.x & 63u, wave = threadIdx.x >> 6;
    const uint32_t len = q.fixed_len;
    const bool ragged = q.intervals != nullptr;
    DevIndex fplain = f; fplain.dtab = nullptr; fplain.dkmer = 0;
    const uint32_t chunk = 256u * HEAVY_PER_LANE;
    for (uint32_t c0 = blockIdx.x * chunk; c0 < n; c0 += gridDim.x * chunk)
    {
        uint32_t kind[HEAVY_PER_LANE], vx[HEAVY_PER_LANE], vy[HEAVY_PER_LANE], ent[HEAVY_PER_LANE];
        uint32_t nk = 0, nr0 = 0, nr1 = 0;
        #pragma unroll
        for (uint32_t u = 0; u < HEAVY_PER_LANE; ++u)
        {
            const uint32_t t = c0 + u * 256u + threadIdx.x;
            kind[u] = 0u; vx[u] = 1u; vy[u] = 0u; ent[u] = 0u;
            if (t < n)
            {
                ent[u] = list[t];
                const uint32_t i = ent[u] & 0x7FFFFFFFu, s = ent[u] >> 31;
                uint32_t rx, ry, nblk; bool single;
                match_one<BITS,false,true,true>( fplain, q, s ? (NVBIO_FM_SCAN_FORWARD | NVBIO_FM_COMPLEMENT) : 0u, f.ktab != nullptr, false, i, rx, ry, nblk, single );
// ... 54 lines not shown
```

nvbio-gpl_amd/csrc/fm_index.hip:

```cpp
#include "fm_device.h"
#include "fm_seed_device.h"
#include "seed_hits_device.h"
#include "bitplanes.h"
#include <hipcub/hipcub.hpp>
#include <new>
#include <stdlib.h>

namespace nvbio_amd {

struct FMIndexImpl
{
    int                  device;
    nvbio_fm_index_view  view;
    uint2*               ktab;
    uint32_t             kmer;
    uint2*               dtab;
    uint32_t             dkmer;
    uint2*               side;
    uint32_t             dmark, dctx;
    uint2*               ctab;
    uint2*               cside;
    uint32_t             ckmer;
    uint32_t             cwide;
    uint32_t             table_flags;
    bool                 owns_arrays;
    uint64_t             owned_bytes;
    uint32_t*            isa;
    uint32_t*            text;
    void*                planes;
    void*                locus;
    uint32_t             locus_len;

    DevIndex dev() const
    {
        DevIndex d;
        d.length = view.length; d.primary = view.primary;
// ... 1576 lines not shown
{
    return index != nullptr && ((FMIndexImpl*)index)->ctab != nullptr ? (int)((FMIndexImpl*)index)->ckmer : 0;
}

nvbio_status nvbio_fm_match_seed_diagonals_both_temp_bytes(const nvbio_string_set* seeds, uint64_t* bytes)
{
    NVB_REQUIRE( bytes != nullptr, "bytes is NULL" );
    SeedScratch L; NVB_CHECK( seed_scratch_layout( seeds, true, &L ) );
    ScratchLayout c( nullptr, scratch_check_enabled() ); L.carve( c ); *bytes = c.bytes();
    return NVBIO_OK;
}

nvbio_status nvbio_fm_match_seed_diagonals_both_keys_capacity(const nvbio_string_set* seeds, uint64_t* n_keys)
{
    NVB_REQUIRE( n_keys != nullptr, "n_keys is NULL" );
    SeedScratch L; NVB_CHECK( seed_scratch_layout( seeds, true, &L ) );
    *n_keys = 256ull * L.tl.n_tiles;
    return NVBIO_OK;
}

nvbio_status nvbio_fm_seed_tiles(const nvbio_string_set* seeds, uint32_t* reads_per_tile, uint32_t* n_tiles)
{
    NVB_REQUIRE( reads_per_tile && n_tiles, "NULL output pointer" );
    SeedScratch L; NVB_CHECK( seed_scratch_layout( seeds, true, &L ) );
    *reads_per_tile = L.tl.rpt; *n_tiles = L.tl.n_tiles;
    return NVBIO_OK;
}

nvbio_status nvbio_fm_match_seed_diagonals_both(nvbio_fm_index_t index, const nvbio_string_set* seeds, uint32_t flags, uint32_t read_len,
                                                uint64_t* keys_dev, nvbio_uint2* residual_ranges_dev, uint32_t* residual_ids_dev,
                                                uint32_t residual_capacity, uint32_t* counts_dev, void* temp_dev, uint64_t temp_bytes,
                                                void* stream)
{
    return nvbio_fm_match_seed_diagonals_both_tiled( index, seeds, flags, read_len, keys_dev, residual_ranges_dev, residual_ids_dev, residual_capacity,
                                                     counts_dev, nullptr, temp_dev, temp_bytes, stream );
}

nvbio_status nvbio_fm_match_seed_diagonals_both_tiled(nvbio_fm_index_t index, const nvbio_string_set* seeds, uint32_t flags, uint32_t read_len,
                                                      uint64_t* keys_dev, nvbio_uint2* residual_ranges_dev, uint32_t* residual_ids_dev,
                                                      uint32_t residual_capacity, uint32_t* counts_dev, uint32_t* tile_offsets_dev,
                                                      void* temp_dev, uint64_t temp_bytes, void* stream)
{
    NVB_REQUIRE( index != nullptr, "index is NULL" );
    FMIndexImpl* idx = (FMIndexImpl*)index;
    StringSetDev q; NVB_CHECK( make_set( seeds, &q ) );
    NVB_REQUIRE( counts_dev != nullptr, "counts_dev is NULL" );
    if (idx->ctab == nullptr)
    {
        set_error( "nvbio_fm_match_seed_diagonals_both needs the canonical table: build the index with NVBIO_FM_TABLE_CANONICAL" );
        return NVBIO_ERR_UNSUPPORTED;
    }
    NVB_REQUIRE( q.spr > 0 && q.spr <= 64u, "the string set must enumerate 1..64 seeds per read (seeds_per_string)" );
    NVB_REQUIRE( seeds->symbol_bits == 2 || seeds->symbol_bits == 4, "packed seeds (2 or 4 bits per symbol)" );
    NVB_REQUIRE( q.fixed_len >= idx->ckmer && q.fixed_len - idx->ckmer <= CTAB_FLANK, "seed length outside [kmer_len, kmer_len + 7]" );
    NVB_REQUIRE( q.intervals != nullptr || (uint64_t)(q.spr - 1u) * q.interval + q.fixed_len <= read_len, "seeds do not fit the read" );
    NVB_REQUIRE( q.intervals != nullptr || read_len - q.fixed_len <= NVBIO_MAX_SEED_OFFSET, NVB_SEED_OFFSET_MSG );
    NVB_REQUIRE( residual_capacity >= q.n, "residual_capacity must be at least the number of seeds" );
    NVB_REQUIRE( q.n < (1u << 31), "at most 2^31 - 1 seeds per call (bit 31 of a seed id carries the strand)" );
    DeviceGuard g( idx->device ); if (!g.ok) return NVBIO_ERR_NO_DEVICE;
    hipStream_t s = (hipStream_t)stream;
    const bool count = (flags & NVBIO_FM_COUNT_SECTORS) != 0;
    const bool defer = (flags & NVBIO_FM_DEFER_HEAVY) != 0 && !count;
    const bool routes = (flags & NVBIO_FM_COUNT_LOCUS) != 0;
    NVB_REQUIRE( !routes || count, "NVBIO_FM_COUNT_LOCUS goes with NVBIO_FM_COUNT_SECTORS" );
    const bool paths = (flags & NVBIO_FM_COUNT_RESOLVE) != 0;
    NVB_REQUIRE( !paths || routes, "NVBIO_FM_COUNT_RESOLVE goes with NVBIO_FM_COUNT_LOCUS" );
    NVB_REQUIRE( !count || ((uintptr_t)counts_dev & 7u) == 0, "counts_dev must be 8-byte aligned with NVBIO_FM_COUNT_SECTORS" );
    NVB_HIP( hipMemsetAsync( counts_dev, 0, (paths ? 12 : (routes ? 10 : (count ? 6 : 4))) * sizeof(uint32_t), s ) );
    const bool use_locus = idx->locus && idx->locus_len == q.fixed_len && !(flags & NVBIO_FM_NO_SEED_LOCUS) &&
                           (q.intervals != nullptr || read_len <= SEED_LOCUS_MAX_READ);
    if (q.n == 0) return NVBIO_OK;
    NVB_REQUIRE( keys_dev && residual_ranges_dev && residual_ids_dev, "NULL device pointer" );
    SeedScratch L; NVB_CHECK( seed_scratch_layout( seeds, true, &L ) );
    ScratchBlock temp;
    NVB_CHECK( temp.alloc_layout( "fm_seed_pass_both", s, "seed pass: out of device memory for %llu bytes of scratch", [&](ScratchLayout& c) { L.carve( c ); },
                                  temp_dev, temp_bytes, "nvbio_fm_match_seed_diagonals_both_temp_bytes" ) );
    uint64_t* tile_keys = L.tile_keys; uint32_t* tile_counts = L.tile_counts; uint32_t* tile_defer = L.tile_defer; uint32_t* defer_counts = L.defer_counts;
    uint32_t* tile_offsets = tile_offsets_dev ? tile_offsets_dev : L.tile_offsets;
    const DevIndex f = idx->dev();
    unsigned blocks = (L.tl.n_tiles + 3u) / 4u;
    const unsigned cap = (flags >> 16) ? (flags >> 16) * 64u : 256u * 64u;
    if (blocks > cap) blocks = cap;
    const dim3 grid( blocks ), block( 256 );
    uint32_t inline_max = (flags >> 8) & 15u;
    inline_max = inline_max < 1u ? 1u : (inline_max > CTAB_INLINE ? CTAB_INLINE : inline_max);
    const uint32_t resolve_opts = inline_max | (((flags & NVBIO_FM_NO_FAST_RESOLVE) || !(flags & NVBIO_FM_DEFER_HEAVY)) ? SEED_RESOLVE_GENERAL : 0u);
    NVB_CHECK( with_value( Values<2, 4>(), seeds->symbol_bits, [&](auto BITS)
    {
        const auto launch = [&](auto CNT, auto W, auto D, auto LC)
        {
            const auto form = [&](auto RG)
            {
                return NVB_LAUNCH( (fm_seed_both_kernel<BITS,CNT,W,D,LC,RG>), grid, block, s, f, q, L.tl, read_len, resolve_opts, tile_keys, tile_counts,
                                   (uint2*)residual_ranges_dev, residual_ids_dev, residual_capacity, (unsigned int*)counts_dev,
                                   CNT ? (unsigned long long*)(counts_dev + 4) : (unsigned long long*)nullptr, tile_defer, defer_counts,
                                   (const void*)(LC ? idx->locus : nullptr), routes ? (unsigned int*)counts_dev + 6 : (unsigned int*)nullptr,
                                   paths ? (unsigned int*)counts_dev + 10 : (unsigned int*)nullptr );
            };
            if constexpr (LC) { if (q.intervals != nullptr) return form( std::true_type() ); }
            return form( std::false_type() );
        };
        const auto kind = [&](auto W, auto LC)
        {
            if (count) return launch( std::true_type(),  W, std::false_type(), LC );
            if (defer) return launch( std::false_type(), W, std::true_type(),  LC );
            return            launch( std::false_type(), W, std::false_type(), LC );
        };
        const auto wide = [&](auto W) { return use_locus ? kind( W, std::true_type() ) : kind( W, std::false_type() ); };
        return idx->cwide ? wide( std::true_type() ) : wide( std::false_type() );
    }, bad_symbol_bits ) );
    size_t scan_bytes = L.scan_bytes;
    hipError_t e = hipcub::DeviceScan::ExclusiveSum( L.scan_temp, scan_bytes, (const uint32_t*)tile_counts, tile_offsets, (int)L.tl.n_tiles, s );
    if (e == hipSuccess)
        NVB_CHECK( NVB_LAUNCH( fm_seed_compact_kernel, dim3( grid_for( 4ull * L.tl.n_tiles ) ), block, s, (const uint64_t*)tile_keys, (const uint32_t*)tile_counts,
                               (const uint32_t*)tile_offsets, L.tl.n_tiles, 128u, keys_dev, (unsigned int*)counts_dev, (unsigned int*)counts_dev + 3,
                               tile_offsets_dev ? tile_offsets_dev + L.tl.n_tiles : (uint32_t*)nullptr ) );
    if (e == hipSuccess && defer)
    {
        scan_bytes = L.scan_bytes;
        e = hipcub::DeviceScan::ExclusiveSum( L.scan_temp, scan_bytes, (const uint32_t*)defer_counts, L.defer_offsets, (int)L.tl.n_tiles, s );
        if (e == hipSuccess)
        {
            NVB_CHECK( NVB_LAUNCH( fm_seed_defer_compact_kernel, dim3( grid_for( L.tl.n_tiles ) ), block, s, (const uint32_t*)tile_defer, (const uint32_t*)defer_counts,
                                   (const uint32_t*)L.defer_offsets, L.tl.n_tiles, L.defer_list, L.defer_n ) );
            const uint64_t max_chunks = (128ull * L.tl.n_tiles + 256u * HEAVY_PER_LANE - 1u) / (256u * HEAVY_PER_LANE);
            const dim3 hgrid( (unsigned)(max_chunks < 4096u ? (max_chunks ? max_chunks : 1u) : 4096u) );
            if (seeds->symbol_bits == 2)
                NVB_CHECK( NVB_LAUNCH( (fm_seed_heavy_kernel<2>), hgrid, block, s, f, q, read_len, (const uint32_t*)L.defer_list, (const uint32_t*)L.defer_n, keys_dev,
                                       (uint2*)residual_ranges_dev, residual_ids_dev, residual_capacity, (unsigned int*)counts_dev ) );
            else
// ... 137 lines not shown
```

nvbio-gpl_amd/csrc/fm_seed_device.h:

```cpp
#pragma once
#include "fm_device.h"

namespace nvbio_amd {

constexpr uint32_t DTAB_MARK      = 0xC0000000u;
constexpr uint32_t DTAB_CTX       = 15u;
constexpr uint32_t DTAB_SIDE_MAX  = 7u;

__device__ __forceinline__ uint32_t left_context(const uint32_t* __restrict__ text, const uint32_t p)
{
    uint32_t ctx = 0;
    const uint32_t nsym = p < DTAB_CTX ? p : DTAB_CTX;
    if (nsym == 0) return 0;
    const uint32_t lo = p - nsym, w0 = lo >> 4, w1 = (p - 1u) >> 4;
    const uint32_t a = text[w0], b = (w1 != w0) ? text[w1] : 0u;
    const uint64_t two = ((uint64_t)a << 32) | b;
    #pragma unroll
    for (uint32_t t = 0; t < DTAB_CTX; ++t)
        if (t < nsym)
        {
            const uint32_t k = (p - 1u - t) - (w0 << 4);
            ctx |= (uint32_t)((two >> (62u - 2u * k)) & 3u) << (2u * (DTAB_CTX - 1u - t));
        }
    return ctx;
// ... 3 lines not shown
{
    x &= 0x3333333333333333ull;
    x = (x | (x >> 2)) & 0x0F0F0F0F0F0F0F0Full;
    x = (x | (x >> 4)) & 0x00FF00FF00FF00FFull;
    x = (x | (x >> 8)) & 0x0000FFFF0000FFFFull;
    x = (x | (x >> 16)) & 0x00000000FFFFFFFFull;
    return x;
}

__device__ __forceinline__ uint64_t reverse_symbols(uint64_t v, const uint32_t len)
{
    v = __brevll( v );
    v = ((v & 0x5555555555555555ull) << 1) | ((v >> 1) & 0x5555555555555555ull);
    return v >> (64u - 2u * len);
}

struct SeedWords { uint32_t w0, w1, w2, w3, w4; };

template <int BITS>
__device__ __forceinline__ SeedWords load_seed_words(const void* __restrict__ symbols, const uint32_t begin, const uint32_t len)
{
    constexpr uint32_t LOG = (BITS == 4) ? 3u : 4u;
    const uint32_t* w = (const uint32_t*)symbols + (begin >> LOG);
    const uint32_t nw = ((begin + len - 1u) >> LOG) - (begin >> LOG) + 1u;
    SeedWords W;
    W.w0 = w[0];
    W.w1 = nw > 1u ? w[1] : 0u;
    W.w2 = nw > 2u ? w[2] : 0u;
    W.w3 = (BITS == 4 && nw > 3u) ? w[3] : 0u;
    W.w4 = (BITS == 4 && nw > 4u) ? w[4] : 0u;
    return W;
}

template <int BITS>
__device__ __forceinline__ bool seed_bits_from_words(const SeedWords& W, const uint32_t begin, const uint32_t len, const bool fwd, const bool comp, uint64_t& V)
{
    uint64_t P; bool clean = true;
    if (BITS == 4)
    {
        const uint32_t sh = (begin & 7u) * 4u;
        const uint64_t A = ((uint64_t)W.w0 << 32) | W.w1, B = ((uint64_t)W.w2 << 32) | W.w3, C = (uint64_t)W.w4 << 32;
        const uint64_t X = sh ? (A << sh) | (B >> (64u - sh)) : A;
        const uint64_t Y = sh ? (B << sh) | (C >> (64u - sh)) : B;
        const uint64_t mx = len >= 16u ? ~0ull : ~0ull << (64u - 4u * len);
        const uint64_t my = len <= 16u ? 0ull : (len >= 32u ? ~0ull : ~0ull << (64u - 4u * (len - 16u)));
        clean = (((X & mx) | (Y & my)) & 0xCCCCCCCCCCCCCCCCull) == 0ull;
        P = ((squeeze_nibbles( X ) << 32) | squeeze_nibbles( Y )) >> (64u - 2u * len);
    }
    else
    {
        const uint32_t sh = (begin & 15u) * 2u;
        const uint64_t A = ((uint64_t)W.w0 << 32) | W.w1, C = (uint64_t)W.w2 << 32;
        P = (sh ? (A << sh) | (C >> (64u - sh)) : A) >> (64u - 2u * len);
    }
    V = fwd ? P : reverse_symbols( P, len );
    if (comp) V ^= (len >= 32u) ? ~0ull : ((1ull << (2u * len)) - 1ull);
    return clean;
}

template <int BITS>
__device__ __forceinline__ bool seed_bits(const void* __restrict__ symbols, const uint32_t begin, const uint32_t len, const bool fwd, const bool comp,
                                          uint64_t& V)
{
    if (BITS == 8)
    {
        uint64_t P = 0; bool clean = true;
// ... 23 lines not shown
```

nvbio-gpl_amd/csrc/gotoh_banded.hip:

```cpp
#include "band31_jobs.h"

namespace nvbio_amd {

template <int BAND, int TYPE, int RBITS, int TBITS, bool BEST2 = false, bool STAGED = false>
__global__ void __launch_bounds__(128)
banded_gotoh_kernel(const BatchDev b, const SchemeDev sc, int32_t* __restrict__ scores, uint2* __restrict__ sinks,
                    const uint32_t distinct_dist, int32_t* __restrict__ scores2, uint2* __restrict__ sinks2,
                    const int32_t* __restrict__ min_scores, const int32_t min_score_all)
{
    __shared__ int32_t s_mm[64];
    fill_mismatch_table( s_mm, sc );

    const uint32_t job = blockIdx.x * blockDim.x + threadIdx.x;
    if (job >= b.n) return;

    const uint32_t rid   = b.read_id ? b.read_id[job] : job;
    const uint32_t first = b.read_offsets[rid];
    const uint32_t M     = b.read_offsets[rid + 1] - first;
    const uint32_t fl    = b.flags ? b.flags[job] : 0u;
    const uint32_t tb    = b.win_begin[job];
    const uint32_t N     = (b.max_read_len && M > b.max_read_len) ? 0u : b.win_end[job] - tb;
    const AlnJob   J{ first, M, tb, N, fl, (fl & NVBIO_READ_REVERSE) != 0, (fl & NVBIO_READ_COMPLEMENT) != 0 };

    int32_t  best   = NVBIO_SCORE_MIN;
// ... 112 lines not shown

        if (TYPE == NVBIO_LOCAL && !BEST2)
        {
            const int32_t h = row_key >> 5;
            if (h >= best) { best = h; best_x = i + (uint32_t)(row_key & 31) + 1u; best_y = i + 1u; }
        }
    }

    if (STAGED && stopped) {  }
    else if (TYPE == NVBIO_GLOBAL)
    {
        if (BEST2) report2( H[BAND - 1], M + BAND - 1, M );
        else if (best <= H[BAND - 1]) { best = H[BAND - 1]; best_x = M + BAND - 1; best_y = M; }
    }
    else if (TYPE == NVBIO_SEMI_GLOBAL)
    {
        const uint32_t mb = M + (uint32_t)(BAND - 1);
        const uint32_t m  = (mb < N ? mb : N) - (M - 1u);
        #pragma unroll
        for (int j = 0; j < BAND; ++j)
            if (j == 0 || (uint32_t)j < m)
            {
                if (BEST2) report2( H[j], M + j, M );
                else if (best <= H[j]) { best = H[j]; best_x = M + j; best_y = M; }
            }
    }
    scores[job] = best;
    sinks[job]  = make_uint2( best_x, best_y );
    if (BEST2) { scores2[job] = sec; sinks2[job] = make_uint2( sec_x, sec_y ); }
}

template <int BAND>
static nvbio_status launch_score(int type, const BatchDev& b, const SchemeDev& sc, uint32_t rbits, uint32_t tbits,
                                 int32_t* scores, uint2* sinks, hipStream_t s, uint8_t* routes)
{
    return with_value( AlnTypes(), type, [&](auto TYPE)
    {
        if (BAND == 31 && plain_gotoh( sc ) && packed_ok( TYPE, sc, b.max_read_len ) && !(b.algo & NVBIO_ALN_NO_PACKED_DP) &&
            tbits == 2 && (rbits == 4 || rbits == 2))
            return launch_pk( TYPE, rbits, b, sc, scores, sinks, s, routes );
        const dim3 grid( (b.n + 127u) / 128u ), block( 128 );
        return with_bits( BitsAll(), rbits, tbits, [&](auto P)
        {
            return NVB_LAUNCH( (banded_gotoh_kernel<BAND,TYPE,P.r,P.t>), grid, block, s, b, sc, scores, sinks, 0u, nullptr, nullptr, nullptr, 0 );
        }, [&] { return invalid_bits( rbits, tbits ); } );
    }, [&] { return invalid_type( type ); } );
}

template <int BAND>
static nvbio_status launch_staged(int type, const BatchDev& b, const SchemeDev& sc, uint32_t rbits, uint32_t tbits,
                                  const int32_t* min_scores, int32_t min_score, int32_t* scores, uint2* sinks, hipStream_t s)
{
    const dim3 grid( (b.n + 127u) / 128u ), block( 128 );
    return with_value( AlnTypes(), type, [&](auto TYPE)
    {
        return with_bits( BitsStaged(), rbits, tbits, [&](auto P)
        {
            return NVB_LAUNCH( (banded_gotoh_kernel<BAND,TYPE,P.r,P.t,false,true>), grid, block, s, b, sc, scores, sinks,
                               0u, (int32_t*)nullptr, (uint2*)nullptr, min_scores, min_score );
        }, [&] { set_error( "staged scoring: read_bits/text_bits %u/%u not instantiated (4/2, 2/2, 8/8)", rbits, tbits ); return NVBIO_ERR_UNSUPPORTED; } );
    }, [&] { return invalid_type( type ); } );
}

nvbio_status make_batch(const nvbio_alignment_batch* in, BatchDev* b)
{
    NVB_REQUIRE( in != nullptr, "batch is NULL" );
    NVB_REQUIRE( in->read_bits == 2 || in->read_bits == 4 || in->read_bits == 8, "read_bits must be 2, 4 or 8" );
    NVB_REQUIRE( in->text_bits == 2 || in->text_bits == 8, "text_bits must be 2 or 8" );
    NVB_REQUIRE( in->n < (1u << 31), "at most 2^31 - 1 jobs per batch (the job lists are compacted with 32-bit signed counts)" );
    if (in->n)
    {
        NVB_REQUIRE( in->reads_dev && in->read_offsets_dev && in->text_dev && in->win_begin_dev && in->win_end_dev,
                     "NULL device pointer in batch" );
// ... 16 lines not shown
                                 int32_t* scores, uint2* sinks, int32_t* scores2, uint2* sinks2, hipStream_t s)
{
    const dim3 grid( (b.n + 127u) / 128u ), block( 128 );
    return with_value( AlnTypes(), type, [&](auto TYPE)
    {
        return with_bits( BitsBest2(), rbits, tbits, [&](auto P)
        {
            return NVB_LAUNCH( (banded_gotoh_kernel<BAND,TYPE,P.r,P.t,true>), grid, block, s, b, sc, scores, sinks, dist, scores2, sinks2, nullptr, 0 );
        }, [&] { set_error( "Best2Sink scoring: read_bits/text_bits %u/%u not instantiated (4/2, 2/2, 8/2, 8/8)", rbits, tbits ); return NVBIO_ERR_UNSUPPORTED; } );
    }, [&] { return invalid_type( type ); } );
}

extern "C" nvbio_status nvbio_banded_gotoh_score_best2(int device, uint32_t band, nvbio_alignment_type type,
                                                       const nvbio_gotoh_scheme* scheme, const nvbio_alignment_batch* batch, uint32_t distinct_dist,
                                                       int32_t* scores_dev, nvbio_uint2* sinks_dev, int32_t* scores2_dev, nvbio_uint2* sinks2_dev,
                                                       void* stream)
{
    NVB_REQUIRE( scheme != nullptr, "scheme is NULL" );
    BatchDev b; NVB_CHECK( make_batch( batch, &b ) );
    NVB_CHECK( check_band( band, NVBIO_ERR_UNSUPPORTED ) );
    if (b.n == 0) return NVBIO_OK;
    NVB_REQUIRE( scores_dev && sinks_dev && scores2_dev && sinks2_dev, "NULL output pointer" );
    DeviceGuard g( device ); if (!g.ok) return NVBIO_ERR_NO_DEVICE;
    const SchemeDev sc = scheme_dev( scheme );
    hipStream_t s = (hipStream_t)stream;
    return with_value( Bands(), band, [&](auto BAND)
    {
        return launch_best2<BAND>( type, b, sc, batch->read_bits, batch->text_bits, distinct_dist, scores_dev, (uint2*)sinks_dev, scores2_dev,
                                   (uint2*)sinks2_dev, s );
    }, [] { return NVBIO_ERR_UNSUPPORTED; } );
}

static nvbio_status banded_score(int device, uint32_t band, int type, const SchemeDev sc, const BatchDev& b, const nvbio_alignment_batch* batch,
                                 int32_t* scores_dev, nvbio_uint2* sinks_dev, void* stream, uint8_t* routes_dev = nullptr)
{
    DeviceGuard g( device ); if (!g.ok) return NVBIO_ERR_NO_DEVICE;
    hipStream_t s = (hipStream_t)stream;
    if (routes_dev) NVB_HIP( hipMemsetAsync( routes_dev, 1, b.n, s ) );
    return with_value( Bands(), band, [&](auto BAND)
    {
        return launch_score<BAND>( type, b, sc, batch->read_bits, batch->text_bits, scores_dev, (uint2*)sinks_dev, s, routes_dev );
    }, [] { return NVBIO_ERR_UNSUPPORTED; } );
}

extern "C" nvbio_status nvbio_banded_gotoh_score_routes(int device, uint32_t band, nvbio_alignment_type type,
                                                        const nvbio_gotoh_scheme* scheme, const nvbio_alignment_batch* batch,
                                                        int32_t* scores_dev, nvbio_uint2* sinks_dev, uint8_t* routes_dev, void* stream)
{
    NVB_REQUIRE( scheme != nullptr, "scheme is NULL" );
    BatchDev b; NVB_CHECK( make_batch( batch, &b ) );
    NVB_CHECK( check_band( band, NVBIO_ERR_UNSUPPORTED ) );
    if (b.n == 0) return NVBIO_OK;
    NVB_REQUIRE( scores_dev && sinks_dev && routes_dev, "NULL output pointer" );
    return banded_score( device, band, type, scheme_dev( scheme ), b, batch, scores_dev, sinks_dev, stream, routes_dev );
}

extern "C" nvbio_status nvbio_banded_gotoh_score(int device, uint32_t band, nvbio_alignment_type type,
                                                 const nvbio_gotoh_scheme* scheme, const nvbio_alignment_batch* batch,
                                                 int32_t* scores_dev, nvbio_uint2* sinks_dev, void* stream)
{
    NVB_REQUIRE( scheme != nullptr, "scheme is NULL" );
    BatchDev b; NVB_CHECK( make_batch( batch, &b ) );
    NVB_CHECK( check_band( band, NVBIO_ERR_UNSUPPORTED ) );
    if (b.n == 0) return NVBIO_OK;
    NVB_REQUIRE( scores_dev && sinks_dev, "NULL output pointer" );
    return banded_score( device, band, type, scheme_dev( scheme ), b, batch, scores_dev, sinks_dev, stream );
}

extern "C" nvbio_status nvbio_banded_gap_pairs(int device, const nvbio_alignment_batch* batch, uint32_t* partner_dev, void* stream)
{
    BatchDev b; NVB_CHECK( make_batch( batch, &b ) );
    if (b.n == 0) return NVBIO_OK;
    NVB_REQUIRE( partner_dev != nullptr, "NULL output pointer" );
    DeviceGuard g( device ); if (!g.ok) return NVBIO_ERR_NO_DEVICE;
    return launch_gap_pairs( b, partner_dev, (hipStream_t)stream );
}

extern "C" nvbio_status nvbio_banded_gotoh_score_staged(int device, uint32_t band, nvbio_alignment_type type,
                                                        const nvbio_gotoh_scheme* scheme, const nvbio_alignment_batch* batch,
                                                        const int32_t* min_scores_dev, int32_t min_score,
                                                        int32_t* scores_dev, nvbio_uint2* sinks_dev, void* stream)
{
    NVB_REQUIRE( scheme != nullptr, "scheme is NULL" );
    BatchDev b; NVB_CHECK( make_batch( batch, &b ) );
    NVB_CHECK( check_band( band, NVBIO_ERR_UNSUPPORTED ) );
    if (b.n == 0) return NVBIO_OK;
    NVB_REQUIRE( scores_dev && sinks_dev, "NULL output pointer" );
// ... 23 lines not shown
```

nvbio-gpl_amd/pipeline.py:

```python
import ctypes
import math
import os

import numpy as np

from .abi import bind
from . import (_MIRRORS, HOST_HEADER_PATH, ALN_RAGGED_READS, FM_COMPLEMENT, FM_NO_FAST_RESOLVE, FM_NO_SEED_LOCUS, FM_SCAN_FORWARD, LOCAL, MAX_SEED_OFFSET, READ_COMPLEMENT, READ_REVERSE, SCORE_MIN, SEMI_GLOBAL, AlignmentBatch,
               BatchedBandedAlignmentScore, FMIndexFilter, GotohAligner, GotohScheme, HitQueues, PackedStringSet, RaggedSeedLayout, SeedHitsParams,
               best_approx_init_ragged, read_queue_begin_ragged, score_reduce_effort, score_reduce_effort_ragged, score_stream_flatten, score_stream_output,
               seed_hits_loc, seed_hits_map, seed_hits_map_ragged, seed_hits_select, SEED_NO_FAST_RESOLVE, SEED_NO_LOCUS)


class SeedExtendParams:
    def __init__(self, seed_len=22, seed_interval=None, band=31, aln_type=LOCAL, scheme=None, min_score=None,
                 max_seed_hits=None):
        self.seed_len = seed_len
        self.seed_interval = seed_interval
        self.band = band
        self.aln_type = aln_type
        self.scheme = scheme or GotohScheme(2, 2, 6, -8, -3, -8, -3)
        self.min_score = min_score
        self.max_seed_hits = max_seed_hits
        self.direct = True
        self.fused_seed_pass = True
        self.mapq = False
        self.mapq_version = 2
        self.merge_strands = True
        self.algo_flags = 0
        self.defer_heavy = True
        self.fused_finish = True

    @classmethod
    def end_to_end(cls, constant_quality=True, **kw):
        scheme = GotohScheme(0, 6, 6, -8, -3, -8, -3) if constant_quality else GotohScheme(0, 2, 6, -8, -3, -8, -3)
        p = cls(aln_type=SEMI_GLOBAL, scheme=scheme, **kw)
        p.e2e = True
        return p

    def interval_for(self, read_len):
        return self.seed_interval or int(1 + 1.15 * math.sqrt(read_len))
# ... 23 lines not shown


def _batch_geometry(torch, fmi, reads, params):
    dev = fmi.device
    R, M, L = reads.n, reads.read_len, params.seed_len
    if M - L > MAX_SEED_OFFSET:
        raise ValueError("read_len - seed_len = %d exceeds %d (NVBIO_MAX_SEED_OFFSET): a diagonal could leave its key's field" % (M - L, MAX_SEED_OFFSET))
    S_int = params.interval_for(M)
    spr = (M - L) // S_int + 1
    ragged = reads.offsets is not None
    intervals = min_scores = None
    if ragged:
        cache = getattr(reads, "_ragged", None)
        if cache is None or cache[0] is not params:
            lens = (reads.offsets[1:] - reads.offsets[:-1]).to(torch.int64)
            itab = params.interval_table(M)
            it = torch.from_numpy(itab).to(dev)
            mt = torch.from_numpy(params.min_score_table(M)).to(dev)
            spr_max = max(((l - L) // int(itab[l]) + 1) if l >= L else 0 for l in range(M + 1))
            cache = reads._ragged = (params, it[lens].contiguous(), mt[lens].contiguous(), int(spr_max))
        _, intervals, min_scores, spr = cache
        qs = PackedStringSet(reads.reads4, 4, R * spr, offsets=reads.offsets, fixed_len=L, stride=0, device=dev, seeds_per_string=spr,
                             seed_intervals=intervals)
        read_off = reads.offsets
    else:
        qs = PackedStringSet(reads.reads4, 4, R * spr, fixed_len=L, stride=M, device=dev, seeds_per_string=spr,
                             seed_interval=S_int)
        read_off = getattr(reads, "_read_off", None)
        if read_off is None:
            read_off = reads._read_off = torch.arange(R + 1, device=dev, dtype=torch.int32) * M
    return dict(S_int=S_int, spr=spr, ragged=ragged, intervals=intervals, min_scores=min_scores, qs=qs, read_off=read_off)


def seed_pass_begin(fmi, reads, params, slot=0, timers=None, stream=None, after=None):
    import torch
    if stream is not None:
        if after is not None:
            stream.wait_event(after)
        with torch.cuda.stream(stream):
            return seed_pass_begin(fmi, reads, params, slot, timers)
    geo = _batch_geometry(torch, fmi, reads, params)
    bufs = getattr(fmi, "_seed_bufs2", None)
    if bufs is None:
        bufs = fmi._seed_bufs2 = {}
    b = bufs.setdefault(slot, {})
    ev_t = None
    if timers is not None:
        a, ev_t = torch.cuda.Event(enable_timing=True), torch.cuda.Event(enable_timing=True)
        timers.setdefault("match_both", []).append((a, ev_t))
        a.record()
    af = params.algo_flags or 0
    fmi.match_seed_diagonals_both(geo["qs"], reads.read_len, b, inline_hits=min(4, params.max_seed_hits or 4), defer_heavy=params.defer_heavy,
                                  grid_blocks=int(getattr(params, "seed_grid_blocks", 0) or 0),
                                  flags=(FM_NO_SEED_LOCUS if af & SEED_NO_LOCUS else 0) | (FM_NO_FAST_RESOLVE if af & SEED_NO_FAST_RESOLVE else 0))
    if ev_t is not None:
        ev_t.record()
    if "host" not in b:
        b["host"] = torch.empty(4, dtype=torch.int32, pin_memory=True)
    b["host"].copy_(b["counts"][:4], non_blocking=True)
    ev = torch.cuda.Event()
    ev.record()
    return dict(b=b, ev=ev, reads=reads)


SCORE_BIAS = 1 << 20


def pack_best_key(torch, scores, rc, pos):
    s = torch.clamp(scores.to(torch.int64) + SCORE_BIAS, min=0)
    return (s << 34) | (rc.to(torch.int64) << 33) | pos.to(torch.int64)


def seed_and_extend(fmi, genome2, genome_len, reads, params, timers=None, return_windows=False, extras=None, pre=None):
    import torch
    from . import (FinishStatus, best_candidate_reduce, best_candidate_unpack, best_candidate_windows, diagonals_to_windows, finish_reads, mapq,
                   second_candidate_reduce)
    dev = fmi.device
    R, M, L = reads.n, reads.read_len, params.seed_len
    geo = _batch_geometry(torch, fmi, reads, params)
    S_int, spr, ragged, intervals, min_scores, qs, read_off = (geo[k] for k in ("S_int", "spr", "ragged", "intervals", "min_scores", "qs", "read_off"))

    def tick(name):
        if timers is None:
            return None
        a, b = torch.cuda.Event(enable_timing=True), torch.cuda.Event(enable_timing=True)
        timers.setdefault(name, []).append((a, b))
        a.record()
        return b

    def tock(b):
        if b is not None:
            b.record()

    ext_flags = (params.algo_flags or 0) | (ALN_RAGGED_READS if ragged else 0)
    text_planes = fmi.text_planes_of(genome2, genome_len)
    aligner = GotohAligner(params.aln_type, params.scheme)
    top = None
    finish = None

    def extend(keys, tag):
        nonlocal top
        if finish is None and top is None:
            top = torch.zeros((R,), dtype=torch.int64, device=dev)
        e = tick("windows" + tag)
        rid, flags, wb, we = diagonals_to_windows(keys, params.band, M, genome_len, read_offsets=read_off if ragged else None)
        tock(e)
        e = tick("extend" + tag)
        batch = AlignmentBatch(reads.reads4, 4, read_off, genome2, 2, wb, we, quals=reads.quals, read_id=rid,
                               flags=flags, device=dev, max_read_len=M, algo_flags=ext_flags or None, text_planes=text_planes)
        scores, sinks = BatchedBandedAlignmentScore(params.band, aligner).enact(batch)
        tock(e)
        if finish is not None:
            scored.append((keys, scores, sinks, wb))
            return None
        e = tick("reduce")
        best_candidate_reduce(keys, scores, sinks, wb, top)
        tock(e)
        if params.mapq or return_windows:
            scored.append((keys, scores, sinks, wb))
        return None

    use_direct = params.direct and fmi.supports_direct()
    results, n_cand, scored = [], 0, []
    fused = use_direct and params.fused_seed_pass

    def residual_keys(ranges, ids, strand):
        if params.max_seed_hits is not None and params.max_seed_hits <= 64 and use_direct and ids.numel() * params.max_seed_hits < 2 ** 31 \
                and getattr(params, "one_call_residuals", True):
            if strand:
                ids = ids ^ -2 ** 31
            rk, nk = fmi.residual_diagonals(ranges.contiguous(), ids.contiguous(), params.max_seed_hits, spr, S_int, L, M,
                                            read_offsets=read_off if ragged else None, seed_intervals=intervals)
            return rk[:int(nk.item())]
        if params.max_seed_hits is not None:
            x = ranges[:, 0].to(torch.int64) & 0xFFFFFFFF
            y = ranges[:, 1].to(torch.int64) & 0xFFFFFFFF
            ycap = torch.minimum(y, x + (params.max_seed_hits - 1))
            ranges = torch.stack([ranges[:, 0], torch.where(ycap >= 2 ** 31, ycap - 2 ** 32, ycap).to(torch.int32)], dim=1).contiguous()
        flt = FMIndexFilter()
        n_hits = flt.rank_ranges(fmi, ranges.contiguous(), None)
        rkeys = flt.locate_diagonals(0, n_hits, spr, S_int, L, M, strand, query_ids=ids.contiguous(),
                                     read_offsets=read_off if ragged else None, seed_intervals=intervals)
        rkeys = torch.unique_consecutive(rkeys)
        if rkeys.numel() > 2 * R:
            rkeys = torch.unique(rkeys)
        return rkeys

    ck = fmi.canonical_kmer if fused else 0
    both = fused and ck and ck <= L <= ck + 7 and spr <= 64 and getattr(params, "two_strand_pass", True)
    if ragged and fused and not both:
        fused = False
    if both:
        if pre is None:
            pre = seed_pass_begin(fmi, reads, params, 0, timers)
        assert pre["reads"] is reads
        b = pre["b"]
        pre["ev"].synchronize()
        FinishStatus.of(dev).check()
        n_keys, n_rf, n_rr = int(b["host"][0]), int(b["host"][1]), int(b["host"][2])
        if params.mapq and getattr(params, "fused_finish", True) and n_keys and n_rf == 0 and n_rr == 0 and int(b["host"][3]) == n_keys:
            finish = (b["tile_offsets"], b["reads_per_tile"])
        parts = [b["keys"][:n_keys]]
        if n_rf or n_rr:
            e = tick("locate")
            parts.append(residual_keys(torch.cat([b["ranges"][:n_rf], b["ranges"][qs.n:qs.n + n_rr]]),
                                       torch.cat([b["ids"][:n_rf], b["ids"][qs.n:qs.n + n_rr] | -2 ** 31]), 0))
            tock(e)
        keys = parts[0] if len(parts) == 1 else torch.cat(parts)
        n_cand += keys.numel()
        if keys.numel():
            results.append(extend(keys, ""))
    elif fused:
        bufs = getattr(fmi, "_seed_bufs", None)
        if bufs is None:
            bufs = fmi._seed_bufs = ({}, {})
        pending = []
        for strand, flags in ((0, 0), (1, FM_SCAN_FORWARD | FM_COMPLEMENT)):
            b = bufs[strand]
            e = tick("match_fw" if strand == 0 else "match_rc")
            fmi.match_seed_diagonals(qs, flags, M, strand, b)
            tock(e)
            if "host" not in b:
                b["host"] = torch.empty(2, dtype=torch.int32, pin_memory=True)
            b["host"].copy_(b["counts"][:2], non_blocking=True)
            ev = torch.cuda.Event()
            ev.record()
            pending.append((strand, b, ev))
        merged = []
        for strand, b, ev in pending:
# ... 789 lines not shown
```

Measured before the change: 2.340 billion.

## Route band-31 extend jobs via seed-stage anchor records to settle without full DP

The seed matching pass now emits a per-read anchor record: the strand, the locus and bitmasks of clean or mismatching lanes around the seed. The band-31 packed extend path uses a new placed-route kernel that reads these records. When a job's window matches the anchor, it derives the mismatch count and an upper score bound directly and runs only the ungapped first-pass tail, skipping the generic first pass. Other jobs flow into a new JOB_FIRST list that the ungapped kernel then processes. This adds work and an extra output to the seed kernel and more cross-stage coupling, with correctness depending on the record encoding.

```diff
diff --git a/include/nvbio_amd.h b/include/nvbio_amd.h
--- a/include/nvbio_amd.h
+++ b/include/nvbio_amd.h
@@ -181,6 +181,10 @@
                                                       uint64_t* keys_dev, nvbio_uint2* residual_ranges_dev, uint32_t* residual_ids_dev,
                                                       uint32_t residual_capacity, uint32_t* counts_dev, uint32_t* tile_offsets_dev,
                                                       void* temp_dev, uint64_t temp_bytes, void* stream);
+nvbio_status nvbio_fm_match_seed_diagonals_both_anchored(nvbio_fm_index_t index, const nvbio_string_set* seeds, uint32_t flags, uint32_t read_len,
+                                                         uint64_t* keys_dev, nvbio_uint2* residual_ranges_dev, uint32_t* residual_ids_dev,
+                                                         uint32_t residual_capacity, uint32_t* counts_dev, uint32_t* tile_offsets_dev,
+                                                         nvbio_uint2* anchor_records_dev, void* temp_dev, uint64_t temp_bytes, void* stream);
 int nvbio_fm_index_is_canonical(nvbio_fm_index_t index);
 
 nvbio_status nvbio_fm_locate_init(nvbio_fm_index_t index, const uint32_t* rows_dev, uint32_t n,
@@ -564,6 +568,8 @@
     NVBIO_ALN_NO_PAIRED_GAP_CHANCE  = 262144,
     NVBIO_ALN_NO_NARROW_DP          = 524288,
     NVBIO_ALN_NO_TEXT_PLANES        = 1048576,
+    NVBIO_ALN_NO_ANCHOR_ROUTE       = 8388608,
+    NVBIO_ALN_ANCHOR_ROUTE_SETTLED_ONLY = 16777216,
     NVBIO_ALN_NO_NARROW_TRACEBACK   = 64
 };
 
@@ -619,9 +625,15 @@
                                       const nvbio_gotoh_scheme* scheme, const nvbio_alignment_batch* batch,
                                       int32_t* scores_dev, nvbio_uint2* sinks_dev, void* stream);
 
+#define NVBIO_ROUTE_PLACED 16u
 nvbio_status nvbio_banded_gotoh_score_routes(int device, uint32_t band, nvbio_alignment_type type,
                                              const nvbio_gotoh_scheme* scheme, const nvbio_alignment_batch* batch,
                                              int32_t* scores_dev, nvbio_uint2* sinks_dev, uint8_t* routes_dev, void* stream);
+
+nvbio_status nvbio_banded_gotoh_score_anchored(int device, uint32_t band, nvbio_alignment_type type,
+                                               const nvbio_gotoh_scheme* scheme, const nvbio_alignment_batch* batch,
+                                               const nvbio_uint2* anchor_records_dev, int32_t* scores_dev, nvbio_uint2* sinks_dev,
+                                               uint8_t* routes_dev, void* stream);
 
 nvbio_status nvbio_banded_gotoh_score_staged(int device, uint32_t band, nvbio_alignment_type type,
                                              const nvbio_gotoh_scheme* scheme, const nvbio_alignment_batch* batch,
diff --git a/nvbio-gpl_amd/__init__.py b/nvbio-gpl_amd/__init__.py
--- a/nvbio-gpl_amd/__init__.py
+++ b/nvbio-gpl_amd/__init__.py
@@ -29,7 +29,11 @@
 ALN_NO_TEXT_PLANES = 1048576
 SEED_NO_LOCUS = 2097152
 SEED_NO_FAST_RESOLVE = 4194304
+ALN_NO_ANCHOR_ROUTE = 8388608
+ALN_ANCHOR_ROUTE_SETTLED_ONLY = 16777216
 ROUTE_SETTLED, ROUTE_FULL_BAND, ROUTE_CLASS_A, ROUTE_CLASS_B, ROUTE_REDONE = 0, 1, 2, 3, 8
+ROUTE_PLACED = 16
+ANCHOR_REC_VALID, ANCHOR_REC_STRAND, ANCHOR_REC_APART2, ANCHOR_REC_LANES = 1 << 31, 1 << 30, 1 << 27, 9
 DEFAULT_ALGO_FLAGS = 0
 BACKTRACK_REFERENCE_QUIRKS = 1
 
@@ -388,7 +392,7 @@
     def canonical(self):
         return self.canonical_kmer != 0
 
-    def match_seed_diagonals_both(self, seeds, read_len, buffers=None, flags=0, grid_blocks=0, inline_hits=0, defer_heavy=False):
+    def match_seed_diagonals_both(self, seeds, read_len, buffers=None, flags=0, grid_blocks=0, inline_hits=0, defer_heavy=False, anchor_records=False):
         torch = _torch()
         n = seeds.n
         if buffers is None:
@@ -409,11 +413,14 @@
             _check(lib().nvbio_fm_seed_tiles(ctypes.byref(qs), ctypes.byref(rpt), ctypes.byref(nt)))
             buffers["reads_per_tile"], buffers["n_tiles"] = int(rpt.value), int(nt.value)
             buffers["tile_offsets"] = torch.zeros(int(nt.value) + 1, dtype=torch.int32, device=self.device)
+            buffers.pop("anchor_records", None)
+        if anchor_records and "anchor_records" not in buffers:
+            buffers["anchor_records"] = torch.empty((n // seeds.seeds_per_string, 2), dtype=torch.int32, device=self.device)
         assert grid_blocks % 64 == 0 and grid_blocks < (1 << 22)
-        _check(lib().nvbio_fm_match_seed_diagonals_both_tiled(
+        _check(lib().nvbio_fm_match_seed_diagonals_both_anchored(
             self._h, ctypes.byref(qs), flags | (FM_DEFER_HEAVY if defer_heavy else 0) | ((int(inline_hits) & 15) << 8) | ((grid_blocks // 64) << 16),
             read_len, _ptr(buffers["keys"]), _ptr(buffers["ranges"]), _ptr(buffers["ids"]), n, _ptr(buffers["counts"]), _ptr(buffers["tile_offsets"]),
-            _ptr(buffers["temp"]), buffers["temp"].numel(), _stream_ptr(self.device)))
+            _ptr(buffers["anchor_records"]) if anchor_records else None, _ptr(buffers["temp"]), buffers["temp"].numel(), _stream_ptr(self.device)))
         return buffers
 
     def residual_diagonals(self, ranges, ids, cap, seeds_per_read, seed_interval, seed_len, read_len, read_offsets=None, seed_intervals=None):
@@ -993,10 +1000,11 @@
 class AlignmentBatch:
 
     def __init__(self, reads, read_bits, read_offsets, text, text_bits, win_begin, win_end, quals=None, read_id=None,
-                 flags=None, device="cuda:0", max_read_len=0, algo_flags=None, text_planes=None):
+                 flags=None, device="cuda:0", max_read_len=0, algo_flags=None, text_planes=None, anchor_records=None):
         torch = _torch()
         self.device = device
         self.text_planes = text_planes
+        self.anchor_records = None if anchor_records is None else _dev_tensor(anchor_records, _torch().int32, device)
         self.algo_flags = DEFAULT_ALGO_FLAGS if algo_flags is None else int(algo_flags)
         self.read_bits, self.text_bits = int(read_bits), int(text_bits)
         self.reads = _dev_tensor(reads, torch.uint8 if read_bits == 8 else torch.int32, device)
@@ -1076,6 +1084,10 @@
                 _ptr(min_scores) if per_job else None, SCORE_MIN if min_scores is None else (0 if per_job else int(min_scores)), _ptr(scores),
                 _ptr(sinks), _stream_ptr(batch.device)))
             return scores, sinks
+        if sw is None and batch.anchor_records is not None:
+            _check(lib().nvbio_banded_gotoh_score_anchored(FMIndex._dev_index(batch.device), self.band_len, self.aligner.type, ctypes.byref(self.aligner.scheme.c),
+                                                           ctypes.byref(bs), _ptr(batch.anchor_records), _ptr(scores), _ptr(sinks), None, _stream_ptr(batch.device)))
+            return scores, sinks
         fn = lib().nvbio_banded_sw_score if sw is not None else lib().nvbio_banded_gotoh_score
         _check(fn(FMIndex._dev_index(batch.device), self.band_len, self.aligner.type, ctypes.byref(sw.c if sw is not None else self.aligner.scheme.c),
                   ctypes.byref(bs), _ptr(scores), _ptr(sinks), _stream_ptr(batch.device)))
@@ -1092,6 +1104,11 @@
     sinks = torch.empty((batch.n, 2), dtype=torch.int32, device=batch.device)
     routes = torch.empty(batch.n, dtype=torch.uint8, device=batch.device)
     bs = batch.c_struct()
+    if batch.anchor_records is not None:
+        _check(lib().nvbio_banded_gotoh_score_anchored(FMIndex._dev_index(batch.device), int(band_len), aligner.type, ctypes.byref(aligner.scheme.c),
+                                                       ctypes.byref(bs), _ptr(batch.anchor_records), _ptr(scores), _ptr(sinks), _ptr(routes),
+                                                       _stream_ptr(batch.device)))
+        return scores, sinks, routes
     _check(lib().nvbio_banded_gotoh_score_routes(FMIndex._dev_index(batch.device), int(band_len), aligner.type, ctypes.byref(aligner.scheme.c),
                                                  ctypes.byref(bs), _ptr(scores), _ptr(sinks), _ptr(routes), _stream_ptr(batch.device)))
     return scores, sinks, routes
diff --git a/nvbio-gpl_amd/csrc/anchor_record.h b/nvbio-gpl_amd/csrc/anchor_record.h
--- /dev/null
+++ b/nvbio-gpl_amd/csrc/anchor_record.h
@@ -0,0 +1,25 @@
+#pragma once
+#include <stdint.h>
+
+namespace nvbio_amd {
+
+constexpr uint32_t ANCHOR_REC_VALID = 1u << 31, ANCHOR_REC_STRAND = 1u << 30, ANCHOR_REC_APART2 = 1u << 27;
+constexpr uint32_t ANCHOR_REC_LANES = 9u;
+constexpr uint32_t ANCHOR_REC_LANE_MASK = (1u << ANCHOR_REC_LANES) - 1u;
+
+__host__ __device__ inline bool anchor_record_counts(const uint32_t y, uint32_t& c, uint32_t& m)
+{
+    const uint32_t clean = y & ANCHOR_REC_LANE_MASK, b0 = (y >> ANCHOR_REC_LANES) & ANCHOR_REC_LANE_MASK, b1 = (y >> (2u * ANCHOR_REC_LANES)) & ANCHOR_REC_LANE_MASK;
+    if (b0 & b1) return false;
+    uint32_t n0 = 0, n1 = 0, taken = 0;
+    const uint32_t apart = (y & ANCHOR_REC_APART2) ? 2u : 1u;
+    for (uint32_t j = 0, next = 0; j < ANCHOR_REC_LANES; ++j)
+    {
+        n0 += (b0 >> j) & 1u; n1 += (b1 >> j) & 1u;
+        if (((clean >> j) & 1u) && j >= next) { ++taken; next = j + apart; }
+    }
+    c = n0 + 2u * n1; m = taken;
+    return true;
+}
+
+}
diff --git a/nvbio-gpl_amd/csrc/band31_first_pass.hip b/nvbio-gpl_amd/csrc/band31_first_pass.hip
--- a/nvbio-gpl_amd/csrc/band31_first_pass.hip
+++ b/nvbio-gpl_amd/csrc/band31_first_pass.hip
@@ -2,15 +2,15 @@
 
 namespace nvbio_amd {
 
-template <int RBITS, int MODE, bool QUAL = false>
+template <int RBITS, int MODE, bool QUAL = false, bool FLIST = false>
 __global__ void __launch_bounds__(256) __attribute__((amdgpu_waves_per_eu((MODE == 0 && !QUAL) ? 7 : 1)))
 ungapped_e2e31_kernel(const BatchDev b, const int32_t P, const int32_t G, const int32_t gap_open, const int32_t gap_ext,
                       int32_t* __restrict__ scores, uint2* __restrict__ sinks, uint8_t* __restrict__ need_dp,
                       const uint32_t* __restrict__ job_list, const uint32_t* __restrict__ job_count,
                       const SchemeDev sc, const JobLists out, const uint32_t third_mask, const NarrowRule nr)
 {
-    constexpr bool LIST = MODE != 0;
-    constexpr int  NL   = LIST ? 1 : 6;
+    constexpr bool LIST = MODE != 0 || FLIST;
+    constexpr int  NL   = MODE != 0 ? 1 : 6;
     __shared__ int32_t s_pen[QUAL ? 64 : 1];
     __shared__ typename JobAppend<NL>::Lds s_lists;
     const uint32_t n    = LIST ? *job_count : b.n;
@@ -36,12 +36,12 @@
             const uint32_t cls = flag >> 8;
             flag &= 255u;
             need_dp[job] = (uint8_t)flag;
-            if (flag) which = LIST ? JOB_DP : (flag == 3u ? JOB_SECOND : (((third_mask >> flag) & 1u) ? JOB_THIRD : (cls ? JOB_CLASS_B - 1 + (int)cls : JOB_DP)));
+            if (flag) which = MODE != 0 ? (int)JOB_DP : job_list_of_flag( flag, cls, third_mask );
         }
         if (MODE == 0 && !QUAL && pairing && __any( flag == 4u ))
         {
             const uint32_t slot = slot0 + 256u * k + threadIdx.x;
-            const int role = gap_pair_role( b, slot, slot < n );
+            const int role = gap_pair_role<FLIST>( b, FLIST ? (slot < n ? job_of( k ) : 0u) : slot, slot < n );
             const uint32_t flag_up = __shfl_down( flag, 1 ), flag_dn = __shfl_up( flag, 1 );
             if (role > 0 && flag == 4u && flag_up == 4u) which = JOB_PAIRS;
             if (role < 0 && flag == 4u && flag_dn == 4u) which = -1;
@@ -51,18 +51,72 @@
     app.flush( s_lists, out, job_of );
 }
 
+__global__ void __launch_bounds__(256)
+route_placed_e2e31_kernel(const BatchDev b, const uint2* __restrict__ records, const int32_t P, const int32_t G, const int32_t gap_open, const int32_t gap_ext,
+                          int32_t* __restrict__ scores, uint2* __restrict__ sinks, uint8_t* __restrict__ need_dp, const JobLists out,
+                          const uint32_t third_mask, const NarrowRule nr, const bool settle_only, uint8_t* __restrict__ marks)
+{
+    typedef JobAppend<6, JOB_FIRST> Append;
+    __shared__ typename Append::Lds s_lists;
+    const uint32_t slot0 = blockIdx.x * (256u * JOB_LIST_CHUNKS);
+    const uint32_t cap = first_pass_cap( P, G, gap_open );
+    Append app;
+    auto job_of = [&](const int k) -> uint32_t { return slot0 + 256u * k + threadIdx.x; };
+    #pragma unroll 1
+    for (int k = 0; k < JOB_LIST_CHUNKS; ++k)
+    {
+        int which = -1;
+        const uint32_t job = job_of( k );
+        if (job < b.n)
+        {
+            which = JOB_PAIRS;
+            const AlnJob   J = load_job( b, job );
+            const uint32_t N = scored_text_len( b, J );
+            const uint2    rec = records[b.read_id ? b.read_id[job] : job];
+            const bool     plain = J.fl == 0u, rc = J.fl == (uint32_t)(NVBIO_READ_REVERSE | NVBIO_READ_COMPLEMENT);
+            uint32_t c = 0, m = 0;
+            if ((rec.y & ANCHOR_REC_VALID) && (plain || rc) && rc == ((rec.y & ANCHOR_REC_STRAND) != 0u) && J.M >= 1u && J.M <= 161u && N == J.M + 31u &&
+                J.tb + 15u + 1024u == rec.x && anchor_record_counts( rec.y, c, m ) && c <= cap && m >= c + 1u)
+            {
+                const int64_t U = -(int64_t)P * (int64_t)c;
+                if (!settle_only || U > (int64_t)G)
+                {
+                    const uint32_t flag = first_pass_tail<true>( b.algo, P, G, gap_open, gap_ext, scores, sinks, job, J.M, N, U, 15u, nr );
+                    need_dp[job] = (uint8_t)(flag & 255u);
+                    which = job_list_of_flag( flag & 255u, flag >> 8, third_mask );
+                    if (marks) marks[job] = (uint8_t)NVBIO_ROUTE_PLACED;
+                }
+            }
+        }
+        app.note( s_lists, k, which );
+    }
+    app.flush( s_lists, out, job_of );
+}
+
+nvbio_status launch_route_placed_e2e31(const BatchDev& b, const uint2* anchor_records, const SchemeDev& sc, const int32_t P, const int32_t G,
+                                       int32_t* scores, uint2* sinks, uint8_t* need_dp, const JobLists& out, const uint32_t third_mask,
+                                       const NarrowRule nr, const bool settle_only, uint8_t* marks, hipStream_t s)
+{
+    return NVB_LAUNCH( route_placed_e2e31_kernel, dim3( job_list_grid( b.n ) ), dim3( 256 ), s, b, anchor_records, P, G, sc.pat_go, sc.pat_ge, scores, sinks,
+                       need_dp, out, third_mask, nr, settle_only, marks );
+}
+
 nvbio_status launch_ungapped_e2e31(const uint32_t rbits, const int mode, const bool by_quality, const BatchDev& b, const SchemeDev& sc, const int32_t P,
                                    const int32_t G, int32_t* scores, uint2* sinks, uint8_t* need_dp, const JobLists& out, const uint32_t third_mask,
-                                   const NarrowRule nr, hipStream_t s)
+                                   const NarrowRule nr, hipStream_t s, const bool first_list)
 {
     const dim3 grid( job_list_grid( b.n ) ), block( 256 );
-    const uint32_t* job_list  = mode == 1 ? out.second : (mode == 2 ? out.third : nullptr);
-    const uint32_t* job_count = mode == 1 ? out.count( JOB_SECOND ) : (mode == 2 ? out.count( JOB_THIRD ) : nullptr);
+    const uint32_t* job_list  = mode == 1 ? out.second : (mode == 2 ? out.third : (first_list ? out.first : nullptr));
+    const uint32_t* job_count = mode == 1 ? out.count( JOB_SECOND ) : (mode == 2 ? out.count( JOB_THIRD ) : (first_list ? out.count( JOB_FIRST ) : nullptr));
+    if (first_list && (mode != 0 || by_quality)) { set_error( "band-31 first pass: only the pass over every job without qualities has a list form" ); return NVBIO_ERR_INVALID; }
     auto miss = [&] { set_error( "band-31 first pass: read_bits %u, mode %d not instantiated", rbits, mode ); return NVBIO_ERR_UNSUPPORTED; };
     return with_value( ReadBits31(), (int)rbits, [&](auto RB)
     {
         if (by_quality && mode == 0)
             return NVB_LAUNCH( (ungapped_e2e31_kernel<RB,0,true>), grid, block, s, b, P, G, sc.pat_go, sc.pat_ge, scores, sinks, need_dp, job_list, job_count,
+                               sc, out, third_mask, nr );
+        if (first_list)
+            return NVB_LAUNCH( (ungapped_e2e31_kernel<RB,0,false,true>), grid, block, s, b, P, G, sc.pat_go, sc.pat_ge, scores, sinks, need_dp, job_list, job_count,
                                sc, out, third_mask, nr );
         return with_value( Values<0, 1, 2>(), by_quality ? -1 : mode, [&](auto MODE)
         {
diff --git a/nvbio-gpl_amd/csrc/band31_jobs.h b/nvbio-gpl_amd/csrc/band31_jobs.h
--- a/nvbio-gpl_amd/csrc/band31_jobs.h
+++ b/nvbio-gpl_amd/csrc/band31_jobs.h
@@ -1,6 +1,7 @@
 #pragma once
 #include "gotoh_common.h"
 #include "bitplanes.h"
+#include "anchor_record.h"
 
 namespace nvbio_amd {
 
@@ -34,6 +35,7 @@
     JOB_PAIRS,
     JOB_CLASS_B, JOB_CLASS_A,
     JOB_REDO,
+    JOB_FIRST,
     JOB_LIST_COUNT
 };
 static_assert( JOB_CLASS_A == JOB_CLASS_B + 1, "narrow_class() 1, 2 = class B, class A, in this order" );
@@ -47,11 +49,12 @@
 struct JobLists
 {
     uint32_t *dp, *second, *third, *pairs; uint32_t* counts; uint32_t *class_b, *class_a, *redo;
+    uint32_t *first;
     static __host__ __device__ constexpr uint32_t count_at(const uint32_t list) { return JOB_COUNT_STRIDE * list; }
     __host__ __device__ __forceinline__ uint32_t* count(const uint32_t list) const { return counts + count_at( list ); }
 };
 
-template <int NL>
+template <int NL, uint32_t SLOT3 = JOB_PAIRS>
 struct JobAppend
 {
     static_assert( NL >= 1 && NL <= 6 && JOB_LIST_CHUNKS >= 1 && JOB_LIST_CHUNKS <= 4, "JobAppend: up to 6 lists, up to 4 chunks" );
@@ -78,7 +81,7 @@
         {
             uint32_t tot = 0;
             for (int i = 0; i < 4 * JOB_LIST_CHUNKS; ++i) { const uint32_t c = lds.cnt[threadIdx.x][i]; lds.cnt[threadIdx.x][i] = tot; tot += c; }
-            lds.base[threadIdx.x] = tot ? atomicAdd( out.count( threadIdx.x ), (unsigned int)tot ) : 0u;
+            lds.base[threadIdx.x] = tot ? atomicAdd( out.count( threadIdx.x == JOB_PAIRS ? SLOT3 : threadIdx.x ), (unsigned int)tot ) : 0u;
         }
         __syncthreads();
         const uint32_t wave = threadIdx.x >> 6;
@@ -89,7 +92,7 @@
             if (e)
             {
                 const uint32_t l = (e >> 6) - 1u;
-                uint32_t* const list = l == JOB_DP ? out.dp : (l == JOB_SECOND ? out.second : (l == JOB_THIRD ? out.third : (l == JOB_PAIRS ? out.pairs : (l == JOB_CLASS_B ? out.class_b : out.class_a))));
+                uint32_t* const list = l == JOB_DP ? out.dp : (l == JOB_SECOND ? out.second : (l == JOB_THIRD ? out.third : (l == JOB_PAIRS ? (SLOT3 == JOB_FIRST ? out.first : out.pairs) : (l == JOB_CLASS_B ? out.class_b : out.class_a))));
                 list[lds.base[l] + lds.cnt[l][4 * k + wave] + (e & 63u)] = job_of( k );
             }
         }
@@ -135,8 +138,15 @@
     }
 };
 
+__device__ __forceinline__ int job_list_of_flag(const uint32_t flag, const uint32_t cls, const uint32_t third_mask)
+{
+    if (!flag) return -1;
+    return flag == 3u ? (int)JOB_SECOND : (((third_mask >> flag) & 1u) ? (int)JOB_THIRD : (cls ? (int)JOB_CLASS_B - 1 + (int)cls : (int)JOB_DP));
+}
+
 constexpr uint32_t PAIR_MAX_SHIFT = NVBIO_GAP_PAIR_MAX_SHIFT;
 
+template <bool BY_ID = false>
 __device__ __forceinline__ int gap_pair_role(const BatchDev& b, const uint32_t job, const bool live)
 {
     uint32_t rid = 0, fl = 0, tb = 0, whole = 0;
@@ -151,7 +161,8 @@
     const uint32_t lane = threadIdx.x & 63u;
     const uint32_t rid_n = __shfl_down( rid, 1 ), fl_n = __shfl_down( fl, 1 ), tb_n = __shfl_down( tb, 1 ), whole_n = __shfl_down( whole, 1 );
     const uint32_t shift = tb_n > tb ? tb_n - tb : tb - tb_n;
-    const bool link = lane < 63u && whole && whole_n && rid_n == rid && fl_n == fl && shift >= 1u && shift <= PAIR_MAX_SHIFT;
+    bool link = lane < 63u && whole && whole_n && rid_n == rid && fl_n == fl && shift >= 1u && shift <= PAIR_MAX_SHIFT;
+    if (BY_ID) link = link && __shfl_down( live ? job : 0xFFFFFFFEu, 1 ) == job + 1u;
     const uint64_t links = __ballot( link );
     const uint32_t run = lane ? (uint32_t)__clzll( (long long)~(links << (64u - lane)) ) : 0u;
     const bool lower = link && !(run & 1u);
@@ -166,11 +177,15 @@
                               const uint32_t* job_list, const uint32_t* job_count, hipStream_t s, const NarrowJobs* narrow = nullptr);
 nvbio_status launch_ungapped_e2e31(const uint32_t rbits, const int mode, const bool by_quality, const BatchDev& b, const SchemeDev& sc, const int32_t P,
                                    const int32_t G, int32_t* scores, uint2* sinks, uint8_t* need_dp, const JobLists& out, const uint32_t third_mask,
-                                   const NarrowRule nr, hipStream_t s);
+                                   const NarrowRule nr, hipStream_t s, const bool first_list = false);
+nvbio_status launch_route_placed_e2e31(const BatchDev& b, const uint2* anchor_records, const SchemeDev& sc, const int32_t P, const int32_t G,
+                                       int32_t* scores, uint2* sinks, uint8_t* need_dp, const JobLists& out, const uint32_t third_mask,
+                                       const NarrowRule nr, const bool settle_only, uint8_t* marks, hipStream_t s);
 nvbio_status launch_gap_chance_e2e31(const uint32_t rbits, const bool with_second, const BatchDev& b, const SchemeDev& sc, const int32_t P, const int32_t G,
                                      const GapLadder lad, int32_t* scores, uint2* sinks, uint8_t* need_dp, const JobLists& out, hipStream_t s);
 nvbio_status launch_gap_pairs(const BatchDev& b, uint32_t* partner, hipStream_t s);
-nvbio_status launch_pk(const int type, const uint32_t rbits, const BatchDev& b, const SchemeDev& sc, int32_t* scores, uint2* sinks, hipStream_t s, uint8_t* routes);
+nvbio_status launch_pk(const int type, const uint32_t rbits, const BatchDev& b, const SchemeDev& sc, int32_t* scores, uint2* sinks, hipStream_t s, uint8_t* routes,
+                       const uint2* anchor_records = nullptr);
 
 using ReadBits31 = Values<2, 4>;
 
diff --git a/nvbio-gpl_amd/csrc/band31_stage.hip b/nvbio-gpl_amd/csrc/band31_stage.hip
--- a/nvbio-gpl_amd/csrc/band31_stage.hip
+++ b/nvbio-gpl_amd/csrc/band31_stage.hip
@@ -85,14 +85,15 @@
     const uint32_t n_r = (REDO && classes) ? *l.count( JOB_REDO ) : 0u;
     for (uint32_t i = blockIdx.x * blockDim.x + threadIdx.x; i < n; i += gridDim.x * blockDim.x)
     {
-        if (i < n_dp) routes[l.dp[i]] = 1u;
-        if (i < n_b)  routes[l.class_b[i]] = 3u;
-        if (i < n_a)  routes[l.class_a[i]] = 2u;
+        if (i < n_dp) routes[l.dp[i]] |= 1u;
+        if (i < n_b)  routes[l.class_b[i]] |= 3u;
+        if (i < n_a)  routes[l.class_a[i]] |= 2u;
         if (i < n_r)  routes[l.redo[i]] |= 8u;
     }
 }
 
-nvbio_status launch_pk(const int type, const uint32_t rbits, const BatchDev& b, const SchemeDev& sc, int32_t* scores, uint2* sinks, hipStream_t s, uint8_t* routes)
+nvbio_status launch_pk(const int type, const uint32_t rbits, const BatchDev& b, const SchemeDev& sc, int32_t* scores, uint2* sinks, hipStream_t s, uint8_t* routes,
+                       const uint2* anchor_records)
 {
     const uint32_t pairs = (b.n + 1u) / 2u;
     int32_t P = 0; bool by_quality = false;
@@ -105,6 +106,8 @@
         const NarrowRule nr = narrow_rule( b.quals == nullptr && !(b.algo & (NVBIO_ALN_NO_NARROW_DP | NVBIO_ALN_RAGGED_READS)) && pk_binary16_ok( type, b, sc ),
                                            P, sc.pat_go, sc.pat_ge );
         const bool classes = nr.thr_b != 1;
+        const bool routed = anchor_records != nullptr && !(b.algo & (NVBIO_ALN_NO_ANCHOR_ROUTE | NVBIO_ALN_RAGGED_READS)) && b.quals == nullptr &&
+                            b.text_planes != nullptr;
         ScratchBlock aux;
         NVB_CHECK( aux.alloc_layout( "banded_job_list", s, "banded score: out of device memory for the job list", [&](ScratchLayout& c)
         {
@@ -117,13 +120,20 @@
             out.class_b = c.take<uint32_t>( classes ? b.n : 1u );
             out.class_a = c.take<uint32_t>( classes ? b.n : 1u );
             out.redo    = c.take<uint32_t>( classes ? b.n : 1u );
+            out.first   = routed ? c.take<uint32_t>( b.n ) : nullptr;
         } ) );
         const bool gapc = !by_quality && !(b.algo & NVBIO_ALN_NO_GAP_CHANCE);
         const uint32_t third_mask = gapc ? ((third ? 1u << 2 : 0u) | 1u << 4) : (third ? 1u << 2 : 0u);
         const bool fused = gapc && third && !(b.algo & (NVBIO_ALN_NO_SECOND_CHANCE | NVBIO_ALN_SPLIT_CHANCES));
         const GapLadder lad = gap_ladder( P, G, sc.pat_go, sc.pat_ge );
         NVB_HIP( hipMemsetAsync( out.counts, 0, JobLists::count_at( JOB_LIST_COUNT ) * sizeof(uint32_t), s ) );
-        NVB_CHECK( launch_ungapped_e2e31( rbits, 0, by_quality, b, sc, P, G, scores, sinks, need_dp, out, third_mask, nr, s ) );
+        if (routed)
+        {
+            if (routes) NVB_HIP( hipMemsetAsync( routes, 0, b.n, s ) );
+            NVB_CHECK( launch_route_placed_e2e31( b, anchor_records, sc, P, G, scores, sinks, need_dp, out, third_mask, nr,
+                                                  (b.algo & NVBIO_ALN_ANCHOR_ROUTE_SETTLED_ONLY) != 0, routes, s ) );
+        }
+        NVB_CHECK( launch_ungapped_e2e31( rbits, 0, by_quality, b, sc, P, G, scores, sinks, need_dp, out, third_mask, nr, s, routed ) );
         if (!fused)     NVB_CHECK( launch_ungapped_e2e31( rbits, 1, false, b, sc, P, G, scores, sinks, need_dp, out, 0u, nr, s ) );
         if (gapc)       NVB_CHECK( launch_gap_chance_e2e31( rbits, fused, b, sc, P, G, lad, scores, sinks, need_dp, out, s ) );
         else if (third) NVB_CHECK( launch_ungapped_e2e31( rbits, 2, false, b, sc, P, G, scores, sinks, need_dp, out, 0u, nr, s ) );
@@ -140,7 +150,7 @@
         if (routes)
         {
             const dim3 rgrid( (b.n + 255u) / 256u < 4096u ? (b.n + 255u) / 256u : 4096u ), block( 256 );
-            NVB_HIP( hipMemsetAsync( routes, 0, b.n, s ) );
+            if (!routed) NVB_HIP( hipMemsetAsync( routes, 0, b.n, s ) );
             NVB_CHECK( NVB_LAUNCH( job_routes_kernel<false>, rgrid, block, s, out, b.n, classes, routes ) );
             NVB_CHECK( NVB_LAUNCH( job_routes_kernel<true>,  rgrid, block, s, out, b.n, classes, routes ) );
         }
diff --git a/nvbio-gpl_amd/csrc/band31_ungapped_inl.h b/nvbio-gpl_amd/csrc/band31_ungapped_inl.h
--- a/nvbio-gpl_amd/csrc/band31_ungapped_inl.h
+++ b/nvbio-gpl_amd/csrc/band31_ungapped_inl.h
@@ -26,6 +26,64 @@
         return (((pl[k] ^ tl) | (ph[k] ^ th)) & pm[k]) | pn[k];
     }
 };
+
+__device__ __forceinline__ uint32_t first_pass_cap(const int32_t P, const int32_t G, const int32_t gap_open)
+{
+    const int64_t floor_u = 3 * (int64_t)(G < gap_open ? G : gap_open) - P;
+    return P > 0 ? (uint32_t)((-floor_u - 1) / (int64_t)P) : 0xFFFFFFFEu;
+}
+
+__device__ __forceinline__ bool second_chance_applies(const uint32_t algo, const bool settled, const int64_t U, const int32_t P, const int32_t G,
+                                                      const uint32_t M, const uint32_t N)
+{
+    return !settled && (int64_t)G - P < U && 2 * (int64_t)G < U && N >= M + 30u && !(algo & NVBIO_ALN_NO_SECOND_CHANCE);
+}
+__device__ __forceinline__ int32_t second_chance_gmax(const int32_t gap_open, const int32_t gap_ext, const int64_t U)
+{
+    int32_t gmax = 0;
+    while (gmax < 5 && (int64_t)gap_open + (int64_t)gmax * gap_ext >= U) ++gmax;
+    return gmax;
+}
+struct ThirdReach { int32_t gmax0, gmax1; bool two11, applies; };
+__device__ __forceinline__ ThirdReach third_chance_reach(const bool settled, const int64_t U, const int32_t P, const uint32_t M, const uint32_t N,
+                                                         const int32_t gap_open, const int32_t gap_ext)
+{
+    const int64_t go = gap_open, ge = gap_ext;
+    ThirdReach t; t.gmax0 = 0; t.gmax1 = 0;
+    while (t.gmax0 < 5 && go + (int64_t)t.gmax0 * ge >= U) ++t.gmax0;
+    while (t.gmax1 < 5 && go + (int64_t)t.gmax1 * ge - P >= U) ++t.gmax1;
+    t.two11 = 2 * go >= U;
+    const bool beyond = t.gmax0 > 4 || t.gmax1 > 4 || go - 2 * (int64_t)P >= U || 2 * go + ge >= U || 2 * go - P >= U || 3 * go >= U || ge < go;
+    t.applies = !settled && N >= M + 30u && !beyond && t.gmax0 >= 1 && (t.gmax1 >= 1 || t.two11);
+    return t;
+}
+
+template <bool NARROW>
+__device__ __forceinline__ uint32_t
+first_pass_tail(const uint32_t algo, const int32_t P, const int32_t G, const int32_t gap_open, const int32_t gap_ext,
+                int32_t* __restrict__ scores, uint2* __restrict__ sinks, const uint32_t job, const uint32_t M, const uint32_t N,
+                const int64_t U, const uint32_t best_d, const NarrowRule nr)
+{
+    const bool settled = U > (int64_t)G;
+    auto stash = [&]() { scores[job] = (int32_t)U; sinks[job] = make_uint2( M + best_d, M ); };
+    if (second_chance_applies( algo, settled, U, P, G, M, N ))
+    {
+        const int32_t gmax = second_chance_gmax( gap_open, gap_ext, U );
+        if (gmax >= 1 && gmax <= 4) { stash(); return 3u; }
+    }
+    if (third_chance_reach( settled, U, P, M, N, gap_open, gap_ext ).applies)
+    {
+        stash();
+        return 2u;
+    }
+    if (settled) { stash(); return 0u; }
+    if (NARROW && N >= M + 30u)
+    {
+        const uint32_t cls = narrow_class( nr, U, best_d, gap_ext );
+        if (cls) { stash(); return 1u | (cls << 8); }
+    }
+    return 1u;
+}
 
 template <int RBITS, int MODE, bool QUAL>
 __device__ __forceinline__ uint32_t
@@ -75,8 +133,7 @@
     }
     else
     {
-        const int64_t floor_u = 3 * (int64_t)(G < gap_open ? G : gap_open) - P;
-        const uint32_t cap = P > 0 ? (uint32_t)((-floor_u - 1) / (int64_t)P) : 0xFFFFFFFEu;
+        const uint32_t cap = first_pass_cap( P, G, gap_open );
         const uint32_t cap_x = (!QUAL && nr.cnt_max > cap && N >= M + 30u) ? nr.cnt_max : cap;
         uint32_t cnt_d[QUAL ? 31 : 1];
         #pragma unroll
@@ -137,19 +194,12 @@
             U = -(int64_t)best_w;
         }
     }
+    if (MODE == 0) return first_pass_tail<!QUAL>( b.algo, P, G, gap_open, gap_ext, scores, sinks, job, M, N, U, best_d, nr );
     bool settled = U > (int64_t)G;
-    auto stash = [&]() { scores[job] = (int32_t)U; sinks[job] = make_uint2( M + best_d, M ); };
-    const bool second_applies = !settled && (int64_t)G - P < U && 2 * (int64_t)G < U && N >= M + 30u && !(b.algo & NVBIO_ALN_NO_SECOND_CHANCE);
-    if (MODE == 0 && second_applies)
-    {
-        int32_t gmax = 0;
-        while (gmax < 5 && (int64_t)gap_open + (int64_t)gmax * gap_ext >= U) ++gmax;
-        if (gmax >= 1 && gmax <= 4) { stash(); return 3u; }
-    }
+    const bool second_applies = second_chance_applies( b.algo, settled, U, P, G, M, N );
     if (MODE == 1 && second_applies)
     {
-        int32_t gmax = 0;
-        while (gmax < 5 && (int64_t)gap_open + (int64_t)gmax * gap_ext >= U) ++gmax;
+        const int32_t gmax = second_chance_gmax( gap_open, gap_ext, U );
         if (gmax >= 1 && gmax <= 4)
         {
             #pragma unroll
@@ -196,18 +246,9 @@
             settled = !gapped;
         }
     }
-    const int64_t go = gap_open, ge = gap_ext;
-    int32_t gmax0 = 0, gmax1 = 0;
-    while (gmax0 < 5 && go + (int64_t)gmax0 * ge >= U) ++gmax0;
-    while (gmax1 < 5 && go + (int64_t)gmax1 * ge - P >= U) ++gmax1;
-    const bool two11  = 2 * go >= U;
-    const bool beyond = gmax0 > 4 || gmax1 > 4 || go - 2 * (int64_t)P >= U || 2 * go + ge >= U || 2 * go - P >= U || 3 * go >= U || ge < go;
-    const bool third_applies = !settled && N >= M + 30u && !beyond && gmax0 >= 1 && (gmax1 >= 1 || two11);
-    if (MODE == 0 && third_applies)
-    {
-        stash();
-        return 2u;
-    }
+    const ThirdReach tr = third_chance_reach( settled, U, P, M, N, gap_open, gap_ext );
+    const int32_t gmax0 = tr.gmax0, gmax1 = tr.gmax1;
+    const bool two11 = tr.two11, third_applies = tr.applies;
     if (MODE != 0 && third_applies)
     {
         #pragma unroll
@@ -325,11 +366,6 @@
         scores[job] = (int32_t)U; sinks[job] = make_uint2( M + best_d, M );
         return 0u;
     }
-    if (MODE == 0 && !QUAL && N >= M + 30u)
-    {
-        const uint32_t cls = narrow_class( nr, U, best_d, gap_ext );
-        if (cls) { stash(); return 1u | (cls << 8); }
-    }
     return 1u;
 }
 
diff --git a/nvbio-gpl_amd/csrc/bitplanes.h b/nvbio-gpl_amd/csrc/bitplanes.h
--- a/nvbio-gpl_amd/csrc/bitplanes.h
+++ b/nvbio-gpl_amd/csrc/bitplanes.h
@@ -194,4 +194,20 @@
     return ((((lo ^ tlo) | (hi ^ thi)) & mask) == 0u) && ((lw.u >> s) & 1u);
 }
 
-}
+__device__ __forceinline__ void load_locus_words_from(const void* __restrict__ lines, const uint32_t base, const uint32_t xs, const uint32_t x, LocusWords& out)
+{
+    load_locus_words( lines, base, xs, out );
+    const uint32_t line = base >> 7, off = x - (line << 7);
+    out.u = ((const uint32_t*)lines)[(size_t)line * 32u + 6u * (off >> 6) + 4u + ((off >> 5) & 1u)];
+}
+
+__device__ __forceinline__ uint32_t locus_mismatches(const LocusWords& lw, const uint32_t xs, const uint32_t xu, const uint32_t len, const uint32_t tlo, const uint32_t thi, bool& u)
+{
+    const uint32_t s = xs & 31u;
+    const uint32_t lo = __builtin_amdgcn_alignbit( lw.lo1, lw.lo0, s ), hi = __builtin_amdgcn_alignbit( lw.hi1, lw.hi0, s );
+    const uint32_t mask = len >= 32u ? 0xFFFFFFFFu : (1u << len) - 1u;
+    u = ((lw.u >> (xu & 31u)) & 1u) != 0u;
+    return ((lo ^ tlo) | (hi ^ thi)) & mask;
+}
+
+}
diff --git a/nvbio-gpl_amd/csrc/fm_canon_inl.h b/nvbio-gpl_amd/csrc/fm_canon_inl.h
--- a/nvbio-gpl_amd/csrc/fm_canon_inl.h
+++ b/nvbio-gpl_amd/csrc/fm_canon_inl.h
@@ -268,11 +268,13 @@
 
 enum : uint32_t { LS_SEED = 1u, LS_OK = 2u, LS_ASKED = 4u, LS_USABLE = 8u, LS_STRAND = 16u,
                   LS_SETTLED = 32u,
-                  LS_BEGIN = 256u };
-template <int BITS, bool COUNT, bool WIDE, bool RAGGED, typename Geom, typename Entry, typename Resolve>
+                  LS_BEGIN = 256u,
+                  LS_XOK = 128u,
+                  LS_MM = 4096u };
+template <int BITS, bool COUNT, bool WIDE, bool RAGGED, bool REC, typename Geom, typename Entry, typename Resolve>
 __device__ __forceinline__ void fm_seed_locus_loop(const DevIndex& f, const StringSetDev& q, const SeedTiles& tl, const uint32_t read_len, const void* __restrict__ locus,
                                                    unsigned long long* __restrict__ sectors_out, unsigned int* __restrict__ routes, const uint32_t tile0,
-                                                   const uint32_t lane, const uint32_t lr, const uint32_t j, const bool lane_ok,
+                                                   const uint32_t lane, const uint32_t lr, const uint32_t j, const bool lane_ok, const bool rec,
                                                    const Geom& seed_geom, const Entry& entry_of, const Resolve& resolve_tile)
 {
     const uint32_t n_waves = gridDim.x * 4u;
@@ -280,8 +282,10 @@
     const uint32_t anchor = lane - j;
     const bool     first = j == 0u;
     const uint32_t u_pfw = j * q.interval;
+    const uint32_t tail = (REC && rec) ? read_len - ((q.spr - 1u) * q.interval + len) : 0u;
     const uint4 none = make_uint4( 1u, 0u, 0u, 0u );
     auto qo_of = [&](const uint64_t V) -> uint32_t { return (uint32_t)(V >> (2u * (len - k) + k)) & 1u; };
+    auto tail_fits = [&](const uint32_t x, const uint32_t strand) -> bool { return strand ? x >= tail : (uint64_t)x + len + tail <= n; };
     auto pfw_of  = [&](const uint32_t v) -> uint32_t { return RAGGED ? v : u_pfw; };
     auto rlen_of = [&](const uint32_t v) -> uint32_t { return RAGGED ? v : read_len; };
     auto add = [&](unsigned int* word, const bool on) {
@@ -297,14 +301,36 @@
     {
         const uint64_t t4 = (uint64_t)tile0 + (uint64_t)step * n_waves;
         if (step >= 4u && t4 - 4ull * n_waves >= tl.n_tiles) break;
-        uint32_t settled = 0;
+        uint32_t settled = 0, mm2 = 3u;
         if (l_fl & LS_ASKED)
         {
             const uint32_t strand = (l_fl / LS_STRAND) & 1u;
             const uint32_t vl = (uint32_t)lV, vh = (uint32_t)(lV >> 32);
             uint32_t plo = squeeze2( vl ) | (squeeze2( vh ) << 16), phi = squeeze2( vl >> 1 ) | (squeeze2( vh >> 1 ) << 16);
-            if (strand) { plo = ~(__brev( plo ) >> (32u - len)); phi = ~(__brev( phi ) >> (32u - len)); }
-            if (locus_answers( LW, l_x, len, plo, phi )) settled = 1u + strand;
+            if (!REC)
+            {
+                if (strand) { plo = ~(__brev( plo ) >> (32u - len)); phi = ~(__brev( phi ) >> (32u - len)); }
+                if (locus_answers( LW, l_x, len, plo, phi )) settled = 1u + strand;
+            }
+            else
+            {
+                const bool     last = u_pfw == (q.spr - 1u) * q.interval;
+                const uint32_t ext = (last && tail_fits( l_x, strand )) ? tail : 0u, clen = len + ext, xs = strand ? l_x - ext : l_x;
+                if (strand) { plo = ~(__brev( plo ) >> (32u - clen)); phi = ~(__brev( phi ) >> (32u - clen)); }
+                bool uq;
+                const uint32_t mm = locus_mismatches( LW, xs, l_x, clen, plo, phi, uq );
+                const uint32_t wmask = len >= 32u ? 0xFFFFFFFFu : (1u << len) - 1u;
+                if (((strand ? mm >> ext : mm) & wmask) == 0u && uq) settled = 1u + strand;
+                if (rec)
+                {
+                    const uint32_t head = q.interval >= 32u ? 0xFFFFFFFFu : (1u << q.interval) - 1u;
+                    uint32_t part = head;
+                    if (strand) part = __brev( part ) >> (32u - len);
+                    if (last) part = 0xFFFFFFFFu;
+                    const uint32_t c = (uint32_t)__popc( mm & part );
+                    mm2 = (c < 3u && (!last || (ext == tail && (l_fl & LS_XOK)))) ? c : 3u;
+                }
+            }
         }
         if (COUNT && routes)
         {
@@ -340,7 +366,16 @@
             if (lane == 0 && c) atomicAdd( sectors_out, (unsigned long long)c );
         }
         uint64_t nV = 0; uint32_t n_fl = w_fl;
-        if (w_fl & LS_SEED) n_fl |= seed_bits_from_words<BITS>( W, (w_fl / LS_BEGIN) & 15u, len, false, false, nV ) ? LS_OK : 0u;
+        if (REC && tail)
+        {
+            if (w_fl & LS_SEED)
+            {
+                bool xok;
+                n_fl |= seed_bits_from_words_ext( W, (w_fl / LS_BEGIN) & 15u, len, tail, nV, xok ) ? LS_OK : 0u;
+                n_fl |= xok ? LS_XOK : 0u;
+            }
+        }
+        else if (w_fl & LS_SEED) n_fl |= seed_bits_from_words<BITS>( W, (w_fl / LS_BEGIN) & 15u, len, false, false, nV ) ? (REC ? LS_OK | LS_XOK : LS_OK) : 0u;
         const uint32_t n_pfw = w_pfw, n_rlen = w_rlen;
         const bool c_ok = (c_fl & LS_OK) != 0u;
         const bool is_one   = c_ok && ce.y >= DTAB_MARK && ce.x < DTAB_MARK;
@@ -357,25 +392,27 @@
         if (first ? (n_fl & LS_OK) != 0u : ((l_fl & LS_OK) && !settled)) { uint32_t qo; got = entry_of( first ? nV : lV, qo ); }
         const uint4 fe = first ? make_uint4( LW.lo0, LW.lo1, LW.hi0, LW.hi1 ) : got;
         LocusWords nLW = { ae.x, ae.y, ae.z, ae.w, 0 };
-        if (ask) load_locus_words( locus, base, x, nLW );
+        if (!REC) { if (ask) load_locus_words( locus, base, x, nLW ); }
+        else if (ask)
+            load_locus_words_from( locus, base, (r_strand && u_pfw == (q.spr - 1u) * q.interval && tail_fits( x, r_strand )) ? x - tail : x, x, nLW );
         {
             const uint64_t rid4 = t4 * tl.rpt + lr;
             uint32_t w_begin = 0;
             bool ws = t4 < tl.n_tiles && lane_ok && rid4 < tl.reads;
             if (RAGGED) { if (ws) ws = seed_geom( (uint32_t)rid4, w_begin, w_pfw, w_rlen ); }
             else if (ws) w_begin = (q.offsets ? q.offsets[rid4] : (uint32_t)rid4 * q.stride) + u_pfw;
-            if (ws) W = load_seed_words<BITS>( q.symbols, w_begin, len );
+            if (ws) W = load_seed_words<BITS>( q.symbols, w_begin, REC ? len + tail : len );
             w_fl = ws ? LS_SEED | ((w_begin & 15u) * LS_BEGIN) : 0u;
         }
         if (step >= 4u)
         {
             const uint32_t tile = (uint32_t)(t4 - 4ull * n_waves), rid = tile * tl.rpt + lr;
             resolve_tile( tile, rid, (c_fl & LS_SEED) != 0u, cV, ce, c_ok, qo_of( cV ), pfw_of( c_pfw ), rlen_of( c_rlen ), is_one, is_group, is_heavy,
-                          q0, q1, q2, q3, (c_fl / LS_SETTLED) & 3u, (uint32_t)cV );
-        }
-        cV = settled ? (uint64_t)l_x : lV; ce = fe; c_fl = l_fl | (settled * LS_SETTLED); c_pfw = l_pfw; c_rlen = l_rlen;
+                          q0, q1, q2, q3, (c_fl / LS_SETTLED) & 3u, (uint32_t)cV, c_fl );
+        }
+        cV = settled ? (uint64_t)l_x : lV; ce = fe; c_fl = l_fl | (settled * LS_SETTLED) | (REC ? mm2 * LS_MM : 0u); c_pfw = l_pfw; c_rlen = l_rlen;
         lV = aV; l_pfw = a_pfw; l_rlen = a_rlen; l_x = x; LW = nLW;
-        l_fl = (a_fl & (LS_SEED | LS_OK)) | (ask ? LS_ASKED : 0u) | (usable ? LS_USABLE : 0u) | (r_strand ? LS_STRAND : 0u);
+        l_fl = (a_fl & (LS_SEED | LS_OK | (REC ? LS_XOK : 0u))) | (ask ? LS_ASKED : 0u) | (usable ? LS_USABLE : 0u) | (r_strand ? LS_STRAND : 0u);
         aV = nV; ae = got; a_fl = n_fl; a_pfw = n_pfw; a_rlen = n_rlen;
     }
 }
@@ -387,8 +424,9 @@
                     uint64_t* __restrict__ tile_keys, uint32_t* __restrict__ tile_counts, uint2* __restrict__ res_ranges,
                     uint32_t* __restrict__ res_ids, const uint32_t res_cap, unsigned int* __restrict__ counts, unsigned long long* __restrict__ sectors_out,
                     uint32_t* __restrict__ tile_defer, uint32_t* __restrict__ defer_counts, const void* __restrict__ locus, unsigned int* __restrict__ routes,
-                    unsigned int* __restrict__ paths)
-{
+                    unsigned int* __restrict__ paths, uint2* __restrict__ anchor_records)
+{
+    constexpr bool REC = BITS == 4 && WIDE && DEFER && LOCUS && !RAGGED && !COUNT;
     const uint32_t lane = threadIdx.x & 63u;
     const uint32_t inline_max = resolve_opts & 15u;
     constexpr bool FAST_FORM = BITS == 4 && WIDE && (COUNT || DEFER);
@@ -410,7 +448,7 @@
         return !ragged || p_fw + len <= rlen;
     };
     auto entry_of = [&](const uint64_t V, uint32_t& qo) -> uint4 {
-        const uint64_t key = V >> (2u * r);
+        const uint64_t key = REC ? (V >> (2u * r)) & ((1ull << (2u * k)) - 1ull) : V >> (2u * r);
         qo = (uint32_t)(key >> k) & 1u;
         const uint64_t idx = canon_index( qo ? canon_revcomp( key, k ) : key, k );
         if (WIDE)
@@ -425,8 +463,10 @@
 
     auto resolve_tile = [&](const uint32_t tile, const uint32_t rid, const bool valid, const uint64_t V, const uint4 e, const bool e_valid, const uint32_t qo,
                             const uint32_t c_pfw, const uint32_t c_rlen, const bool is_one, const bool is_group, const bool is_heavy,
-                            const uint4 q0, const uint4 q1, const uint4 q2, const uint4 q3, const uint32_t settled, const uint32_t settled_x)
-    {
+                            const uint4 q0, const uint4 q1, const uint4 q2, const uint4 q3, const uint32_t settled, const uint32_t settled_x,
+                            const uint32_t fl)
+    {
+        uint32_t rec_d = 0;
         const uint32_t m = e.y - DTAB_MARK;
         const uint32_t rest = (uint32_t)V & rmask;
         const uint32_t want = qo ? (~rest & rmask) : rest;
@@ -466,6 +506,7 @@
                 const uint32_t p = s ? c_rlen - c_pfw - len : c_pfw;
                 const uint64_t diag = (uint64_t)v + 1024u - p;
                 const uint64_t key = ((uint64_t)rid << 34) | ((uint64_t)s << 33) | diag;
+                if (REC) rec_d = (uint32_t)diag;
                 const uint64_t below = (1ull << lane) - 1ull;
                 const uint64_t m0 = __ballot( has && s == 0u ), m1 = __ballot( has && s != 0u );
                 const uint64_t prev_mask = (s ? m1 : m0) & below;
@@ -508,6 +549,11 @@
             hits[0] = settled == 1u; hits[1] = settled == 2u;
             pos[0][0] = pos[1][0] = settled_x;
         }
+        if (REC)
+        {
+            const bool rs = (fl & LS_STRAND) != 0u;
+            rec_d = (rs ? pos[1][0] : pos[0][0]) + 1024u - (rs ? c_rlen - c_pfw - len : c_pfw);
+        }
         uint32_t tile_fill = 0;
         uint32_t defer_fill = 0;
         #pragma unroll
@@ -581,6 +627,21 @@
         }
         if (lane == 0) { tile_counts[tile] = tile_fill; if (DEFER) defer_counts[tile] = defer_fill; }
         }
+        if (REC && anchor_records)
+        {
+            const bool     head = j == 0u, usable = (fl & LS_USABLE) != 0u;
+            const uint32_t mm2 = (fl / LS_MM) & 3u;
+            const uint64_t bc = __ballot( head ? usable : settled != 0u );
+            const uint64_t b0 = __ballot( !head && (mm2 & 1u) ), b1 = __ballot( !head && (mm2 & 2u) );
+            if (head && (fl & LS_SEED))
+            {
+                const uint32_t lm = (1u << q.spr) - 1u;
+                const uint32_t y = ANCHOR_REC_VALID | ((fl & LS_STRAND) ? ANCHOR_REC_STRAND : 0u) | (len > q.interval ? ANCHOR_REC_APART2 : 0u) |
+                                   ((uint32_t)(bc >> lane) & lm) | (((uint32_t)(b0 >> lane) & lm) << ANCHOR_REC_LANES) |
+                                   (((uint32_t)(b1 >> lane) & lm) << (2u * ANCHOR_REC_LANES));
+                anchor_records[rid] = usable ? make_uint2( rec_d, y ) : make_uint2( 0u, 0u );
+            }
+        }
         if (COUNT)
         {
             uint32_t tot = valid ? sectors : 0u;
@@ -595,7 +656,8 @@
     if constexpr (LOCUS)
     {
         tile = (uint32_t)__builtin_amdgcn_readfirstlane( (int)tile );
-        fm_seed_locus_loop<BITS,COUNT,WIDE,RAGGED>( f, q, tl, read_len, locus, sectors_out, routes, tile, lane, lr, j, lane_ok, seed_geom, entry_of, resolve_tile );
+        fm_seed_locus_loop<BITS,COUNT,WIDE,RAGGED,REC>( f, q, tl, read_len, locus, sectors_out, routes, tile, lane, lr, j, lane_ok, REC && anchor_records != nullptr,
+                                                       seed_geom, entry_of, resolve_tile );
         return;
     }
     SeedWords W = { 0, 0, 0, 0, 0 }; uint32_t w_begin = 0, w_pfw = 0, w_rlen = 0; bool w_valid = false;
@@ -648,7 +710,7 @@
             if (w_valid) w_valid = seed_geom( rid2, w_begin, w_pfw, w_rlen );
             if (w_valid) W = load_seed_words<BITS>( q.symbols, w_begin, len );
         }
-        resolve_tile( tile, rid, valid, V, e, e_valid, qo, c_pfw, c_rlen, is_one, is_group, is_heavy, q0, q1, q2, q3, 0u, 0u );
+        resolve_tile( tile, rid, valid, V, e, e_valid, qo, c_pfw, c_rlen, is_one, is_group, is_heavy, q0, q1, q2, q3, 0u, 0u, 0u );
         V = Vn; e = en; e_valid = en_valid; qo = qon; c_pfw = n_pfw; c_rlen = n_rlen; c_seed = n_seed;
     }
 }
diff --git a/nvbio-gpl_amd/csrc/fm_index.hip b/nvbio-gpl_amd/csrc/fm_index.hip
--- a/nvbio-gpl_amd/csrc/fm_index.hip
+++ b/nvbio-gpl_amd/csrc/fm_index.hip
@@ -2,6 +2,7 @@
 #include "fm_seed_device.h"
 #include "seed_hits_device.h"
 #include "bitplanes.h"
+#include "anchor_record.h"
 #include <hipcub/hipcub.hpp>
 #include <new>
 #include <stdlib.h>
@@ -1644,14 +1645,23 @@
                                                 uint32_t residual_capacity, uint32_t* counts_dev, void* temp_dev, uint64_t temp_bytes,
                                                 void* stream)
 {
-    return nvbio_fm_match_seed_diagonals_both_tiled( index, seeds, flags, read_len, keys_dev, residual_ranges_dev, residual_ids_dev, residual_capacity,
-                                                     counts_dev, nullptr, temp_dev, temp_bytes, stream );
+    return nvbio_fm_match_seed_diagonals_both_anchored( index, seeds, flags, read_len, keys_dev, residual_ranges_dev, residual_ids_dev, residual_capacity,
+                                                        counts_dev, nullptr, nullptr, temp_dev, temp_bytes, stream );
 }
 
 nvbio_status nvbio_fm_match_seed_diagonals_both_tiled(nvbio_fm_index_t index, const nvbio_string_set* seeds, uint32_t flags, uint32_t read_len,
                                                       uint64_t* keys_dev, nvbio_uint2* residual_ranges_dev, uint32_t* residual_ids_dev,
                                                       uint32_t residual_capacity, uint32_t* counts_dev, uint32_t* tile_offsets_dev,
                                                       void* temp_dev, uint64_t temp_bytes, void* stream)
+{
+    return nvbio_fm_match_seed_diagonals_both_anchored( index, seeds, flags, read_len, keys_dev, residual_ranges_dev, residual_ids_dev, residual_capacity,
+                                                        counts_dev, tile_offsets_dev, nullptr, temp_dev, temp_bytes, stream );
+}
+
+nvbio_status nvbio_fm_match_seed_diagonals_both_anchored(nvbio_fm_index_t index, const nvbio_string_set* seeds, uint32_t flags, uint32_t read_len,
+                                                         uint64_t* keys_dev, nvbio_uint2* residual_ranges_dev, uint32_t* residual_ids_dev,
+                                                         uint32_t residual_capacity, uint32_t* counts_dev, uint32_t* tile_offsets_dev,
+                                                         nvbio_uint2* anchor_records_dev, void* temp_dev, uint64_t temp_bytes, void* stream)
 {
     NVB_REQUIRE( index != nullptr, "index is NULL" );
     FMIndexImpl* idx = (FMIndexImpl*)index;
@@ -1697,6 +1707,10 @@
     uint32_t inline_max = (flags >> 8) & 15u;
     inline_max = inline_max < 1u ? 1u : (inline_max > CTAB_INLINE ? CTAB_INLINE : inline_max);
     const uint32_t resolve_opts = inline_max | (((flags & NVBIO_FM_NO_FAST_RESOLVE) || !(flags & NVBIO_FM_DEFER_HEAVY)) ? SEED_RESOLVE_GENERAL : 0u);
+    const bool rec = anchor_records_dev != nullptr && seeds->symbol_bits == 4 && idx->cwide && defer && use_locus && q.intervals == nullptr &&
+                     read_len - (q.spr - 1u) * q.interval <= 32u && q.interval <= q.fixed_len && q.fixed_len <= 2u * q.interval &&
+                     q.spr <= ANCHOR_REC_LANES;
+    if (anchor_records_dev && !rec) NVB_HIP( hipMemsetAsync( anchor_records_dev, 0, (size_t)L.tl.reads * sizeof(uint2), s ) );
     NVB_CHECK( with_value( Values<2, 4>(), seeds->symbol_bits, [&](auto BITS)
     {
         const auto launch = [&](auto CNT, auto W, auto D, auto LC)
@@ -1707,7 +1721,7 @@
                                    (uint2*)residual_ranges_dev, residual_ids_dev, residual_capacity, (unsigned int*)counts_dev,
                                    CNT ? (unsigned long long*)(counts_dev + 4) : (unsigned long long*)nullptr, tile_defer, defer_counts,
                                    (const void*)(LC ? idx->locus : nullptr), routes ? (unsigned int*)counts_dev + 6 : (unsigned int*)nullptr,
-                                   paths ? (unsigned int*)counts_dev + 10 : (unsigned int*)nullptr );
+                                   paths ? (unsigned int*)counts_dev + 10 : (unsigned int*)nullptr, rec ? (uint2*)anchor_records_dev : (uint2*)nullptr );
             };
             if constexpr (LC) { if (q.intervals != nullptr) return form( std::true_type() ); }
             return form( std::false_type() );
diff --git a/nvbio-gpl_amd/csrc/fm_seed_device.h b/nvbio-gpl_amd/csrc/fm_seed_device.h
--- a/nvbio-gpl_amd/csrc/fm_seed_device.h
+++ b/nvbio-gpl_amd/csrc/fm_seed_device.h
@@ -59,6 +59,23 @@
     return W;
 }
 
+__device__ __forceinline__ bool seed_bits_from_words_ext(const SeedWords& W, const uint32_t begin, const uint32_t len, const uint32_t ext, uint64_t& V, bool& clean_ext)
+{
+    const uint32_t sh = (begin & 7u) * 4u, all = len + ext;
+    const uint64_t A = ((uint64_t)W.w0 << 32) | W.w1, B = ((uint64_t)W.w2 << 32) | W.w3, C = (uint64_t)W.w4 << 32;
+    const uint64_t X = sh ? (A << sh) | (B >> (64u - sh)) : A;
+    const uint64_t Y = sh ? (B << sh) | (C >> (64u - sh)) : B;
+    auto bad = [&](const uint32_t l) -> bool {
+        const uint64_t mx = l >= 16u ? ~0ull : ~0ull << (64u - 4u * l);
+        const uint64_t my = l <= 16u ? 0ull : (l >= 32u ? ~0ull : ~0ull << (64u - 4u * (l - 16u)));
+        return (((X & mx) | (Y & my)) & 0xCCCCCCCCCCCCCCCCull) != 0ull;
+    };
+    const bool clean = !bad( len );
+    clean_ext = !bad( all );
+    V = reverse_symbols( ((squeeze_nibbles( X ) << 32) | squeeze_nibbles( Y )) >> (64u - 2u * all), all );
+    return clean;
+}
+
 template <int BITS>
 __device__ __forceinline__ bool seed_bits_from_words(const SeedWords& W, const uint32_t begin, const uint32_t len, const bool fwd, const bool comp, uint64_t& V)
 {
diff --git a/nvbio-gpl_amd/csrc/gotoh_banded.hip b/nvbio-gpl_amd/csrc/gotoh_banded.hip
--- a/nvbio-gpl_amd/csrc/gotoh_banded.hip
+++ b/nvbio-gpl_amd/csrc/gotoh_banded.hip
@@ -168,13 +168,13 @@
 
 template <int BAND>
 static nvbio_status launch_score(int type, const BatchDev& b, const SchemeDev& sc, uint32_t rbits, uint32_t tbits,
-                                 int32_t* scores, uint2* sinks, hipStream_t s, uint8_t* routes)
+                                 int32_t* scores, uint2* sinks, hipStream_t s, uint8_t* routes, const uint2* anchor_records)
 {
     return with_value( AlnTypes(), type, [&](auto TYPE)
     {
         if (BAND == 31 && plain_gotoh( sc ) && packed_ok( TYPE, sc, b.max_read_len ) && !(b.algo & NVBIO_ALN_NO_PACKED_DP) &&
             tbits == 2 && (rbits == 4 || rbits == 2))
-            return launch_pk( TYPE, rbits, b, sc, scores, sinks, s, routes );
+            return launch_pk( TYPE, rbits, b, sc, scores, sinks, s, routes, anchor_records );
         const dim3 grid( (b.n + 127u) / 128u ), block( 128 );
         return with_bits( BitsAll(), rbits, tbits, [&](auto P)
         {
@@ -257,14 +257,16 @@
 }
 
 static nvbio_status banded_score(int device, uint32_t band, int type, const SchemeDev sc, const BatchDev& b, const nvbio_alignment_batch* batch,
-                                 int32_t* scores_dev, nvbio_uint2* sinks_dev, void* stream, uint8_t* routes_dev = nullptr)
+                                 int32_t* scores_dev, nvbio_uint2* sinks_dev, void* stream, uint8_t* routes_dev = nullptr,
+                                 const nvbio_uint2* anchor_records_dev = nullptr)
 {
     DeviceGuard g( device ); if (!g.ok) return NVBIO_ERR_NO_DEVICE;
     hipStream_t s = (hipStream_t)stream;
     if (routes_dev) NVB_HIP( hipMemsetAsync( routes_dev, 1, b.n, s ) );
     return with_value( Bands(), band, [&](auto BAND)
     {
-        return launch_score<BAND>( type, b, sc, batch->read_bits, batch->text_bits, scores_dev, (uint2*)sinks_dev, s, routes_dev );
+        return launch_score<BAND>( type, b, sc, batch->read_bits, batch->text_bits, scores_dev, (uint2*)sinks_dev, s, routes_dev,
+                                   (const uint2*)anchor_records_dev );
     }, [] { return NVBIO_ERR_UNSUPPORTED; } );
 }
 
@@ -278,6 +280,19 @@
     if (b.n == 0) return NVBIO_OK;
     NVB_REQUIRE( scores_dev && sinks_dev && routes_dev, "NULL output pointer" );
     return banded_score( device, band, type, scheme_dev( scheme ), b, batch, scores_dev, sinks_dev, stream, routes_dev );
+}
+
+extern "C" nvbio_status nvbio_banded_gotoh_score_anchored(int device, uint32_t band, nvbio_alignment_type type,
+                                                          const nvbio_gotoh_scheme* scheme, const nvbio_alignment_batch* batch,
+                                                          const nvbio_uint2* anchor_records_dev, int32_t* scores_dev, nvbio_uint2* sinks_dev,
+                                                          uint8_t* routes_dev, void* stream)
+{
+    NVB_REQUIRE( scheme != nullptr, "scheme is NULL" );
+    BatchDev b; NVB_CHECK( make_batch( batch, &b ) );
+    NVB_CHECK( check_band( band, NVBIO_ERR_UNSUPPORTED ) );
+    if (b.n == 0) return NVBIO_OK;
+    NVB_REQUIRE( scores_dev && sinks_dev, "NULL output pointer" );
+    return banded_score( device, band, type, scheme_dev( scheme ), b, batch, scores_dev, sinks_dev, stream, routes_dev, anchor_records_dev );
 }
 
 extern "C" nvbio_status nvbio_banded_gotoh_score(int device, uint32_t band, nvbio_alignment_type type,
diff --git a/nvbio-gpl_amd/pipeline.py b/nvbio-gpl_amd/pipeline.py
--- a/nvbio-gpl_amd/pipeline.py
+++ b/nvbio-gpl_amd/pipeline.py
@@ -5,7 +5,7 @@
 import numpy as np
 
 from .abi import bind
-from . import (_MIRRORS, HOST_HEADER_PATH, ALN_RAGGED_READS, FM_COMPLEMENT, FM_NO_FAST_RESOLVE, FM_NO_SEED_LOCUS, FM_SCAN_FORWARD, LOCAL, MAX_SEED_OFFSET, READ_COMPLEMENT, READ_REVERSE, SCORE_MIN, SEMI_GLOBAL, AlignmentBatch,
+from . import (_MIRRORS, HOST_HEADER_PATH, ALN_NO_ANCHOR_ROUTE, ALN_RAGGED_READS, FM_COMPLEMENT, FM_NO_FAST_RESOLVE, FM_NO_SEED_LOCUS, FM_SCAN_FORWARD, LOCAL, MAX_SEED_OFFSET, READ_COMPLEMENT, READ_REVERSE, SCORE_MIN, SEMI_GLOBAL, AlignmentBatch,
                BatchedBandedAlignmentScore, FMIndexFilter, GotohAligner, GotohScheme, HitQueues, PackedStringSet, RaggedSeedLayout, SeedHitsParams,
                best_approx_init_ragged, read_queue_begin_ragged, score_reduce_effort, score_reduce_effort_ragged, score_stream_flatten, score_stream_output,
                seed_hits_loc, seed_hits_map, seed_hits_map_ragged, seed_hits_select, SEED_NO_FAST_RESOLVE, SEED_NO_LOCUS)
@@ -95,6 +95,11 @@
     return dict(S_int=S_int, spr=spr, ragged=ragged, intervals=intervals, min_scores=min_scores, qs=qs, read_off=read_off)
 
 
+def _wants_anchor_records(reads, params, geo):
+    return bool(not geo["ragged"] and reads.quals is None and params.band == 31 and params.aln_type == SEMI_GLOBAL and params.scheme.c.match == 0
+                and not ((params.algo_flags or 0) & ALN_NO_ANCHOR_ROUTE))
+
+
 def seed_pass_begin(fmi, reads, params, slot=0, timers=None, stream=None, after=None):
     import torch
     if stream is not None:
@@ -115,7 +120,8 @@
     af = params.algo_flags or 0
     fmi.match_seed_diagonals_both(geo["qs"], reads.read_len, b, inline_hits=min(4, params.max_seed_hits or 4), defer_heavy=params.defer_heavy,
                                   grid_blocks=int(getattr(params, "seed_grid_blocks", 0) or 0),
-                                  flags=(FM_NO_SEED_LOCUS if af & SEED_NO_LOCUS else 0) | (FM_NO_FAST_RESOLVE if af & SEED_NO_FAST_RESOLVE else 0))
+                                  flags=(FM_NO_SEED_LOCUS if af & SEED_NO_LOCUS else 0) | (FM_NO_FAST_RESOLVE if af & SEED_NO_FAST_RESOLVE else 0),
+                                  anchor_records=_wants_anchor_records(reads, params, geo))
     if ev_t is not None:
         ev_t.record()
     if "host" not in b:
@@ -158,6 +164,7 @@
     ext_flags = (params.algo_flags or 0) | (ALN_RAGGED_READS if ragged else 0)
     text_planes = fmi.text_planes_of(genome2, genome_len)
     aligner = GotohAligner(params.aln_type, params.scheme)
+    anchor_records = None
     top = None
     finish = None
 
@@ -170,7 +177,8 @@
         tock(e)
         e = tick("extend" + tag)
         batch = AlignmentBatch(reads.reads4, 4, read_off, genome2, 2, wb, we, quals=reads.quals, read_id=rid,
-                               flags=flags, device=dev, max_read_len=M, algo_flags=ext_flags or None, text_planes=text_planes)
+                               flags=flags, device=dev, max_read_len=M, algo_flags=ext_flags or None, text_planes=text_planes,
+                               anchor_records=anchor_records)
         scores, sinks = BatchedBandedAlignmentScore(params.band, aligner).enact(batch)
         tock(e)
         if finish is not None:
@@ -218,6 +226,7 @@
             pre = seed_pass_begin(fmi, reads, params, 0, timers)
         assert pre["reads"] is reads
         b = pre["b"]
+        anchor_records = b.get("anchor_records") if _wants_anchor_records(reads, params, geo) else None
         pre["ev"].synchronize()
         FinishStatus.of(dev).check()
         n_keys, n_rf, n_rr = int(b["host"][0]), int(b["host"][1]), int(b["host"][2])
```

Result: slower. 2.062 billion (-11.9%).
